# bacon205/Multimodal_eeg_fmri

Measured on AMD Instinct MI355X. Metric: pairs_per_sec_per_node, higher is better.
Workload: dtype bf16

## Files before the change

### include/mmeeg_hip.h

```cpp
#ifndef MMEEG_HIP_H
#define MMEEG_HIP_H

#include <stdint.h>

#ifdef __cplusplus
extern "C" {
#endif

typedef struct ihipStream_t* hipStream_t;

#define MM_ABI_VERSION 5

const char* mm_last_error(void);
int mm_abi_version(void);

int mm_pack_nct_bf16(const float* x, void* y, int B, int C, int T, int Cp, hipStream_t stream);
int mm_unpack_ntc_f32(const void* g, float* dx, int B, int C, int T, int Cp, hipStream_t stream);
int mm_prep_conv_weight(const float* w, void* w_fwd, void* w_dgrad, int Cout, int Cin, int k,
                        int Cinp, int Coutp, hipStream_t stream);

int mm_conv1d_fwd(const void* x, const void* w, int B, int T, int Cin, int Cout, int taps, int pad,
                  const float* scale, const float* shift, int act, const float* residual,
                  const float* pe, int pool, float* stats, float* out_f32, void* out_bf16,
                  void* out_pre, float drop_p, uint32_t drop_seed, const uint32_t* seed_epoch,
// ... 108 lines not shown
int mm_bn_act_bwd_apply_bcast(const float* y, const float* out4, const float* dout_rows, float scale, const float* sums,
                              void* dy, int R, int S, int N, int act, float drop_p, uint32_t seed,
                              const uint32_t* seed_epoch, int train, int sums_nrep, hipStream_t stream);

int mm_pooled_head_bwd_rows(const float* dout, const void* z_pre_bf16, const float* W, void* dz_bf16, float* rows_out,
                            void* dx_bf16, int B, int L, int D, int N, int act, float drop_p, uint32_t seed,
                            float emit_drop_p, uint32_t emit_seed, const uint32_t* seed_epoch, hipStream_t stream);

int mm_attn_fwd(const void* qkv, void* out, float* lse, int B, int L, int H, int head_dim,
                float scale, float drop_p, uint32_t seed, const uint32_t* seed_epoch,
                const float* attn_mask, int attn_mask_per_head, hipStream_t stream);
int mm_attn_bwd(const void* qkv, const void* out, const void* dout, const float* lse, void* dqkv,
                float* delta_ws, int B, int L, int H, int head_dim, float scale, float drop_p,
                uint32_t seed, const uint32_t* seed_epoch, const float* attn_mask, int attn_mask_per_head,
                hipStream_t stream);
int mm_attn_fwd_hd(const void* qkv, void* out, float* lse, int B, int L, int H, int head_dim,
                   float scale, float drop_p, uint32_t seed, const uint32_t* seed_epoch,
                   const float* attn_mask, int attn_mask_per_head, hipStream_t stream);
int mm_attn_bwd_hd(const void* qkv, const void* out, const void* dout, const float* lse, void* dqkv,
                   float* delta_ws, int B, int L, int H, int head_dim, float scale, float drop_p,
                   uint32_t seed, const uint32_t* seed_epoch, const float* attn_mask, int attn_mask_per_head,
                   hipStream_t stream);

int mm_colsum(const void* a_bf16, const float* a_f32, float* out, int M, int N, hipStream_t stream);
int mm_meanpool_fwd(const float* x, float* out_f32, void* out_bf16, int B, int L, int D, hipStream_t stream);
int mm_meanpool_bwd(const float* g, float* dx, int B, int L, int D, hipStream_t stream);
int mm_stage_inputs(const float* eeg, void* eeg_packed_bf16, float* eeg_copy, int B, int C, int T, int Cp,
                    float* fmri_dst, const float* fmri_src, int64_t fmri_n, hipStream_t stream);
int mm_act_bwd(const float* g_f32, const void* g_bf16, const void* z, void* out, int64_t n, int act,
               float drop_p, uint32_t seed, const uint32_t* seed_epoch, hipStream_t stream);

int mm_pack_volume_bf16(const float* x, void* y, int64_t nvox, int Cp, hipStream_t stream);
int mm_conv3d_fwd(const void* x, const void* w, int B, int D, int H, int W, int Cin, int Cout,
                  const float* shift, float* stats, float* out_f32, void* out_bf16, hipStream_t stream);
int mm_conv3d_wgrad(const void* dy, const void* x, float* dw, float* dbias, int B, int D, int H, int W,
                    int Cin, int Cout, int Cin_real, int64_t sn, int64_t sc, int64_t stap, int nrep,
                    int64_t rep_stride, int slot_mode, hipStream_t stream);
int mm_conv3d_wgrad_slots(int B, int D, int H, int W, int Cin, int Cout, int* slots_host, hipStream_t stream);
int mm_pool3d_bn_act_fwd(const void* y, const float* out4, void* out_bf16, void* ysel, void* arg, int B, int D,
                         int H, int W, int N, int act, float drop_p, uint32_t seed, const uint32_t* seed_epoch,
                         hipStream_t stream);
int mm_pool3d_bn_act_bwd_reduce(const void* ysel, const float* out4, const void* dout_bf16, float* sums_out,
                                int B, int D, int H, int W, int N, int act, float drop_p, uint32_t seed,
                                const uint32_t* seed_epoch, hipStream_t stream);
int mm_pool3d_bn_act_bwd_apply(const void* y, const void* arg, const float* out4, const void* dout_bf16,
                               const float* sums, void* dy, int B, int D, int H, int W, int N, int act,
                               float drop_p, uint32_t seed, const uint32_t* seed_epoch, int train, int sums_nrep,
                               hipStream_t stream);

int mm_conv3d_l1(int mode, const float* x, const void* wimg, const float* bias, const float* out4,
                 const void* dout, const float* sums, float* stats, void* out, float* dw_tapmajor,
                 float* dbias, int B, int D, int H, int W, int train, float drop_p, uint32_t seed,
                 const uint32_t* seed_epoch, hipStream_t stream);
int mm_conv3d_l1_fwd_winners(const float* x, const void* wimg, const float* bias, const float* out4, void* out,
                             void* arg, int B, int D, int H, int W, int train, float drop_p, uint32_t seed,
                             const uint32_t* seed_epoch, hipStream_t stream);
int mm_conv3d_l1_gram(const float* x, const void* wimg, const float* bias, float* gram, float* stats, int B, int D,
                      int H, int W, hipStream_t stream);
int mm_conv3d_l1_bwd(const float* x, const void* wimg, const float* bias, const float* out4, const void* dout,
                     float* sums_out, float* a1, const float* gram, float* dw, float* dbias, int B, int D,
                     int H, int W, int train, float drop_p, uint32_t seed, const uint32_t* seed_epoch,
                     hipStream_t stream);

int mm_small_linear_fwd(const float* x, const float* W, const float* bias, const float* scale,
                        const float* shift, float* y, float* pre, int B, int K, int N, int act,
                        float drop_p, uint32_t seed, const uint32_t* seed_epoch, hipStream_t stream);
int mm_small_linear_bwd(const float* dy, const float* x, const float* W, float* dx, float* dW, float* db,
                        int B, int K, int N, hipStream_t stream);
int mm_act_f32(const float* z, float* y, int64_t n, int act, float drop_p, uint32_t seed, const uint32_t* seed_epoch, hipStream_t stream);
int mm_act_bwd_f32(const float* g, const float* z, float* out, int64_t n, int act, float drop_p,
                   uint32_t seed, const uint32_t* seed_epoch, hipStream_t stream);
int mm_colstats(const float* x, float* stats, int B, int N, hipStream_t stream);
int mm_proj_heads_fwd(const float* x_e, const float* W_e, const float* b_e, const float* g_e, const float* be_e,
                      int K_e, const float* x_f, const float* W_f, const float* b_f, const float* g_f,
                      const float* be_f, int K_f, float* z1, float* hn, float* stat, float* z, float* nrm, int B,
                      int N, float eps, float drop_p, uint32_t seed_e, uint32_t seed_f,
                      const uint32_t* seed_epoch, hipStream_t stream);
int mm_proj_heads_bwd(const float* dz, const float* z, const float* nrm, const float* hn, const float* z1,
                      const float* stat, const float* x_e, const float* W_e, const float* g_e, int K_e,
                      const float* x_f, const float* W_f, const float* g_f, int K_f, float* dx_e, float* dW_e,
                      float* db_e, float* dg_e, float* dbe_e, float* dx_f, float* dW_f, float* db_f, float* dg_f,
                      float* dbe_f, int B, int N, float drop_p, uint32_t seed_e, uint32_t seed_f,
                      const uint32_t* seed_epoch, hipStream_t stream);
int mm_clip_loss_own_rows(const float* z_all, const float* logit_scale, float* scal4, float* dz_local, float* ws,
                          int B, int Bg, int N, int row0, hipStream_t stream);
int mm_clip_loss_ws_floats(int B, int Bg, int* floats_host, hipStream_t stream);
int mm_clip_loss_own_rows_grouped(const float* z_all, const int* gid_all, const float* logit_scale, float* scal4,
                                  float* dz_local, float* ws, int B, int Bg, int N, int row0, hipStream_t stream);
int mm_clip_loss_grouped_ws_floats(int B, int Bg, int* floats_host, hipStream_t stream);

#define MM_RETRIEVAL_KMAX 16
#define MM_RETRIEVAL_NMAX (1 << 20)
int mm_retrieval(const float* Q, const float* G, const int* pos, int* ranks, int* topk_idx, float* topk_score,
                 float* ws, int Nq, int Ng, int D, int k, hipStream_t stream);
int mm_retrieval_ws_floats(int Nq, int Ng, int D, int k, int* floats_host, hipStream_t stream);
int mm_retrieval_grouped(const float* Q, const float* G, const int* qgid, const int* ggid, int* ranks, float* ws,
                         int Nq, int Ng, int D, hipStream_t stream);
int mm_retrieval_grouped_ws_floats(int Nq, int Ng, int D, int* floats_host, hipStream_t stream);

typedef struct {
    float* w[3]; float* b[3]; float* gamma[3]; float* beta[3]; float* run_mean[3]; float* run_var[3];
    void* batches_tracked[3];
    float* W; float* B; float* Gamma; float* Beta; float* Run_mean; float* Run_var;
    int cin; int k[3]; int cinp; int reserved;
} mm_power_merge_t;
int mm_power_merge(const void* desc_host, int mode, hipStream_t stream);

int mm_softmax2_concat(const float* a, const float* c, const float* pa, const float* pc, float* out, int B,
                       int Ha, int Hc, hipStream_t stream);
int mm_learned_fusion(const float* f0, const float* f1, const float* f2, const float* dyn,
                      const float* logits, const float* temperature, float* fused, float* weights, int B,
                      int H, int M, hipStream_t stream);
int mm_attn_1xk(const float* p0, const float* p1, const float* p2, const float* p3, int K, const float* dctx,
                float* ctx, float* attw, float* dp0, float* dp1, float* dp2, float* dp3, int B, int E,
                int nhead, float drop_p, uint32_t seed, const uint32_t* seed_epoch, int backward,
                hipStream_t stream);
int mm_add_f32(const float* a, const float* b, float* out, int64_t n, hipStream_t stream);
int mm_attn_1x2(const float* proj_e, const float* proj_f, float* ctx, float* attw, int B, int E, int nhead,
                hipStream_t stream);
int mm_attn_1x2_train(const float* proj_e, const float* proj_f, const float* dctx, float* ctx, float* attw,
                      float* dproj_e, float* dproj_f, int B, int E, int nhead, float drop_p, uint32_t seed,
                      const uint32_t* seed_epoch, int backward, hipStream_t stream);
int mm_learned_fusion_bwd(const float* f0, const float* f1, const float* f2, const float* dyn,
                          const float* logits, const float* temperature, const float* dfused, float* df0,
                          float* df1, float* df2, float* ddyn, float* dlogits, float* dtemp, int B, int H,
                          int M, hipStream_t stream);
int mm_softmax2_concat_bwd(const float* dout, const float* a, const float* c, const float* pa,
                           const float* pc, float* da, float* dc, float* dpa, float* dpc, int B, int Ha,
                           int Hc, hipStream_t stream);
int mm_weighted_ce(const float* logits, const void* target_i64, const float* class_weight, float* loss_out,
                   float* dlogits, int B, int C, hipStream_t stream);
int mm_focal_loss(const float* logits, const void* target_i64, float* loss_out, float* per_sample,
                  float* dlogits, int B, int C, float alpha, float gamma, float scale, hipStream_t stream);
int mm_gate2_mix(const float* g, const float* erp, const float* pw, const float* conn, float* comb,
                 float* gate, int B, int H, float boost, hipStream_t stream);
int mm_gate2_mix_bwd(const float* dcomb, const float* g, const float* erp, const float* pw, float* derp,
                     float* dpw, float* dconn, float* dg, int B, int H, float boost, hipStream_t stream);
int mm_smoothed_ce(const float* logits, const void* target_i64, float* loss_out, float* dlogits, int B,
                   int C, float smoothing, hipStream_t stream);
int mm_stft_power(const float* x, void* out_bf16, float* out_f32, int B, int C, int T, int nfft, int hop,
                  int ch_off, int ch_total, hipStream_t stream);
#define MM_ZSCORE_WS_DOUBLES 64
int mm_sample_zscore_bf16(const float* x, void* out_bf16, double* ws, int B, int rows, int ch_valid, int ch_total,
                          float eps, hipStream_t stream);
int mm_sample_zscore_bwd(const float* x, const void* g_bf16, float* dx, int B, int rows, int ch_valid, int ch_total,
                         float eps, hipStream_t stream);
int mm_stft_power_bwd(const float* x, const float* g_power, float* dx, int B, int C, int T, int nfft, int hop,
                      int ch_off, int ch_total, hipStream_t stream);
int mm_mul_f32(const float* a, const float* b, float* out, int64_t n, hipStream_t stream);
int mm_linear_fwd_meanpool(const void* x, const void* w, int M, int K, const float* bias, const float* residual,
                           float* out_f32, float drop_p, uint32_t seed, const uint32_t* seed_epoch, float* pool_out,
                           int rows_per_group, hipStream_t stream);
int mm_linear_fwd_ln(const void* x, const void* w, int M, int K, const float* bias, const float* residual,
                     float* out_f32, float drop_p, uint32_t seed, const uint32_t* seed_epoch, const float* ln_gamma,
                     const float* ln_beta, float ln_eps, void* ln_out_bf16, float* ln_stat, hipStream_t stream);
int mm_pooled_head_fwd(const float* pooled, const float* pooled_acc, const float* W, const float* bias, float* out, void* z_pre_bf16,
                       void* pooled_bf16, int B, int D, int N, int act, float drop_p, uint32_t seed,
                       const uint32_t* seed_epoch, hipStream_t stream);
int mm_pooled_head_bwd(const float* dout, const void* z_pre_bf16, const float* W, void* dz_bf16, float* dx,
                       void* dx_bf16, int B, int L, int D, int N, int act, float drop_p, uint32_t seed,
                       float emit_drop_p, uint32_t emit_seed, const uint32_t* seed_epoch, hipStream_t stream);
int mm_drop_path(const float* x, float* out, int64_t B, int64_t inner, float drop_p, uint32_t seed,
                 const uint32_t* seed_epoch, hipStream_t stream);
int mm_meanpool_bf16(const void* x, float* out, int R, int S, int N, hipStream_t stream);

#define MM_OPT_STATE_FLOATS 1032
int mm_sumsq(const float* g, float* state, int64_t n, hipStream_t stream);
int mm_adamw_clip(float* p, float* g, float* m, float* v, float* state, int64_t n, float beta1,
                  float beta2, float eps, float weight_decay, float max_norm, float grad_scale,
                  int zero_grad, uint32_t* seed_epoch, hipStream_t stream);

int mm_xai_interp(const float* x, const float* base, int base_rows, float* out, int n_steps, int s0, int steps,
// ... 36 lines not shown
```

### multimodal_eeg_fmri_amd/autograd.py

```python
from __future__ import annotations

import os
from typing import Dict, List, Optional

import torch

from . import _hip
from . import ops
from .ops import ACT, AREPL, REPL, WREP, _BF, _F32, _empty, _zeros


_BAG = {"cur": None}


def _reduce_into(dst, src, K, stride, offset=0, nrep=REPL):
    if dst is None:
        return
    if nrep not in (1, REPL):
        raise ValueError("_reduce_into: nrep is 1 (fp32 vector) or REPL (accumulator workspace)")
    bag = _BAG["cur"]
    ptr = src.data_ptr() + (8 if nrep == REPL else 4) * offset
    if bag is not None:
        bag.defer(ptr, dst, K, AREPL if nrep == REPL else 1, stride, keep=src)
    elif nrep == REPL:
# ... 617 lines not shown
    end = ops.kernel_timer.bracket(f"conv3d_dgrad_c{N}")
    _hip.call("mm_conv3d_fwd", dy, wd, B, D, H, W, N, cinp, None, None, None, dx)
    if end is not None:
        end.record()
    return dx


def conv3d_l1_bwd(bag: GradBag, s: dict, dout: torch.Tensor):
    conv, bn, x = s["conv"], s["bn"], s["x"]
    B, _, D, H, W = x.shape
    train = 1 if s.get("train", True) else 0
    sums = _zeros((REPL, 2, 32), x)
    dw = bag.target(conv.weight)
    if dw is None:
        _hip.call("mm_conv3d_l1", 2, x, s["wimg"], conv.bias, s["out4"], dout, None, sums, None, None, None,
                  B, D, H, W, train, float(s["drop_p"]), int(s["seed"]), ops.EP())
    else:
        a1 = _zeros((REPL, 27, 32), x)
        _hip.call("mm_conv3d_l1_bwd", x, s["wimg"], conv.bias, s["out4"], dout, sums, a1, s.get("gramc") if train else None,
                  dw, bag.target(conv.bias), B, D, H, W, train, float(s["drop_p"]), int(s["seed"]), ops.EP())
    _bn_param_grads(bag, bn, sums, 32, nrep=REPL)


def volume_encoder_bwd(bag: GradBag, sv: dict, dout: torch.Tensor):
    last = sv["convs"][2]
    d = pooled_head_bwd(bag, sv["head"], dout, rows_only=not last["pool"])
    g = conv3d_bn_act_bwd(bag, last, d)
    g = conv3d_bn_act_bwd(bag, sv["convs"][1], g)
    if sv["convs"][0].get("l1"):
        conv3d_l1_bwd(bag, sv["convs"][0], g)
        return None
    need_dx = bool(sv.get("need_dx"))
    dxp = conv3d_bn_act_bwd(bag, sv["convs"][0], g, need_dx=need_dx)
    if not need_dx:
        return None
    Bx, C, D, H, W = sv["x_shape"]
    return dxp[..., :C].permute(0, 4, 1, 2, 3).float().contiguous()


class VolumeEncoderFn(_ModuleFn):

    @staticmethod
    def run(m, x):
        return VolumeEncoderFn.apply(m, x, *_module_params(m))

    @staticmethod
    def forward(ctx, m, x, *params):
        ctx.need_dx = bool(x.requires_grad)
        out, saved = ops._vol_forward_impl(m, x.float(), m.training, True, save=True, need_dx=ctx.need_dx)
        ctx.saved, ctx.params = saved, params
        return out

    @staticmethod
    def backward(ctx, dout):
        bag = GradBag()
        with deferred(bag, dout.device):
            dx = volume_encoder_bwd(bag, ctx.saved, dout)
        return _ModuleFn._finish(ctx, bag, ctx.params, dx)


def proj_head_bwd(bag: GradBag, s: dict, da: torch.Tensor, need_dx=True):
    lin, ln = s["seq"][0], s["seq"][1]
    B, N = da.shape
    K = lin.weight.shape[1]
    dhn = _empty((B, N), _F32, da)
    _hip.call("mm_act_bwd_f32", da, s["hn"], dhn, B * N, ACT["gelu"], float(s["p"]), int(s["seed"]), ops.EP())
    dz1 = _empty((B, N), _F32, da)
    dgb = _zeros((REPL, 2, N), da)
    _hip.call("mm_layernorm_bwd", None, dhn, s["z1"], s["stat"], ln.weight, None, dz1, None, dgb, B, N, 0.0, 0, None)
    _ln_param_grads(bag, ln, dgb, N)
    dx = _empty((B, K), _F32, da) if need_dx else None
    _hip.call("mm_small_linear_bwd", dz1, s["x"], lin.weight, dx, bag.target(lin.weight), bag.target(lin.bias), B, K, N)
    return dx


def contrastive_embed_bwd(bag: GradBag, s: dict, dz: torch.Tensor, need=(True, True)):
    B, N = s["B"], s["N"]
    br = s["bridge"]
    (le, lne), (lf, lnf) = br.eeg_proj[:2], br.fmri_proj[:2]
    xe, xf = s["xe"], s["xf"]
    dxe = _empty(xe.shape, _F32, dz) if need[0] else None
    dxf = _empty(xf.shape, _F32, dz) if need[1] else None
    t = bag.target
    _hip.call("mm_proj_heads_bwd", dz.contiguous(), s["z"], s["nrm"], s["hn"], s["z1"], s["stat"],
              xe, le.weight, lne.weight, xe.shape[1], xf, lf.weight, lnf.weight, xf.shape[1],
              dxe, t(le.weight), t(le.bias), t(lne.weight), t(lne.bias),
              dxf, t(lf.weight), t(lf.bias), t(lnf.weight), t(lnf.bias),
              B, N, float(s["p"]), int(s["seeds"][0]), int(s["seeds"][1]), ops.EP())
    return dxe, dxf


class ContrastiveEmbedFn(torch.autograd.Function):
    @staticmethod
    def run(bridge, eeg, fmri):
        ps = list(bridge.eeg_proj.parameters()) + list(bridge.fmri_proj.parameters())
        return ContrastiveEmbedFn.apply(bridge, eeg, fmri, *ps)

    @staticmethod
    def forward(ctx, bridge, eeg, fmri, *params):
        z, saved = ops.contrastive_embed_impl(bridge, eeg, fmri, bridge.training)
        ctx.saved, ctx.params = saved, params
        ctx.need = (eeg.requires_grad, fmri.requires_grad)
        return z

    @staticmethod
    def backward(ctx, dz):
        bag = GradBag()
        with deferred(bag, dz.device):
            dxe, dxf = contrastive_embed_bwd(bag, ctx.saved, dz.contiguous(), ctx.need)
        return (None, dxe, dxf) + tuple(bag.result(p) for p in ctx.params)


class ClipLossFn(torch.autograd.Function):

    @staticmethod
    def forward(ctx, z, logit_scale, group, gid=None):
        from . import dp
        z = z.contiguous().float()
        B, N2 = z.shape
        rank = dp.rank(group)
        z_all = dp.gather_embeddings(z, group)
        need_grad = z.requires_grad or logit_scale.requires_grad
        scal = _empty((4,), _F32, z)
        dz = _empty((B, N2), _F32, z) if need_grad else None
        ls = logit_scale.detach().reshape(1).float().contiguous()
        gid_all = None if gid is None else dp.gather_embeddings(gid.view(B, 1), group).view(-1)
        ops.clip_loss_own_rows(z_all, gid_all, ls, scal, dz, B, rank * B)
        if need_grad:
            ctx.save_for_backward(dz, scal)
        return scal[0].clone(), scal[1].clone(), scal[2].clone()

    @staticmethod
    def backward(ctx, g_loss, g_a, g_b):
        dz, scal = ctx.saved_tensors
        return dz * g_loss, (scal[3] * g_loss).reshape(()), None, None
```

### multimodal_eeg_fmri_amd/bridge_trainer.py

```python
from __future__ import annotations

import os
from typing import Dict, Optional

import torch
import torch.nn as nn

from . import _hip, dp, ops
from .autograd import GradBag, contrastive_embed_bwd, deferred, erp_encoder_bwd, power_encoder_bwd, volume_encoder_bwd
from .bridge_checkpoint import TrainerCheckpointMixin
from .bridge_utils import EEGfMRIContrastiveBridge, retrieval_metrics
from .enhanced_models_v4 import EnhancedERPEncoder
from .fmri_utils import fMRIVolumeEncoder3D
from .optim import FlatBucket


class BridgeTrainer(TrainerCheckpointMixin, nn.Module):
    def __init__(self, eeg_channels: int = 64, hidden_dim: int = 128, fmri_dim: int = 64,
                 bridge_dim: int = 128, dropout: float = 0.3, lr: float = 1e-4,
                 weight_decay: float = 1e-4, grad_clip: float = 1.0, betas=(0.9, 0.999),
                 eps: float = 1e-8, group=None, device="cuda", mode: str = "graph", eeg_encoder: Optional[nn.Module] = None,
                 num_heads: int = 4, num_layers: int = 2):
        super().__init__()
        self.eeg_encoder = (EnhancedERPEncoder(eeg_channels, hidden_dim, num_layers, num_heads, dropout)
# ... 50 lines not shown
        assert off == self.bucket.n
        self.fmri_lo = self.groups[-1][2]
        self._works = []
        self.capture_mode = None
        self.bucket.state[2] = lr
        self._scal = torch.zeros(4, device=device)
        ops.weights_changed()

    @property
    def _side(self):
        if self._side_stream is None:
            self._side_stream = torch.cuda.Stream()
        return self._side_stream

    @property
    def world(self):
        import torch.distributed as dist
        return dist.get_world_size(self.group) if self.group is not None else 1

    def set_lr(self, lr: float):
        self.lr = lr
        self.bucket.state[2] = lr

    def forward(self, eeg: torch.Tensor, fmri: torch.Tensor, groups: Optional[torch.Tensor] = None):
        gid = ops.group_ids(groups, eeg.shape[0], eeg.device, "BridgeTrainer")
        if not self.two_streams:
            return self.head(self.eeg_encoder(eeg), self.fmri_encoder(fmri), self.group, gid)
        main = torch.cuda.current_stream()
        self._side.wait_stream(main)
        with torch.cuda.stream(self._side):
            ff = self.fmri_encoder(fmri)
        fe = self.eeg_encoder(eeg)
        main.wait_stream(self._side)
        ff.record_stream(main)
        return self.head(fe, ff, self.group, gid)

    def train_step(self, eeg: torch.Tensor, fmri: torch.Tensor, groups: Optional[torch.Tensor] = None) -> Dict[str, torch.Tensor]:
        ops.check_volume_shape(fmri.shape)
        gid = ops.group_ids(groups, eeg.shape[0], None if self.mode == "graph" else eeg.device, "train_step")
        if self.mode == "autograd":
            return self._step_autograd(eeg, fmri, gid)
        if self.mode == "manual":
            with torch.no_grad():
                return self._step_manual(eeg, fmri, gid)
        return self._step_graph(eeg, fmri, gid)

    def _step_autograd(self, eeg, fmri, gid=None):
        b = self.bucket
        b.zero_grad()
        loss, acc_e, acc_f = self.forward(eeg, fmri, gid)
        loss.backward()
        b.absorb_autograd_grads()
        self._seg_optimizer()
        return {"loss": loss.detach(), "top1_e2f": acc_e, "top1_f2e": acc_f}

    STAMP_NAMES = ("step start", "weights prepared", "EEG fwd done", "fMRI fwd start", "fMRI fwd done",
                   "heads fwd done", "loss done", "heads bwd done", "EEG bwd done", "fMRI bwd start",
                   "fMRI bwd done", "grad reductions done", "AdamW done", "side stream done")

    def _stamp(self, i):
        if self.stamps is not None:
            _hip.call("mm_debug_stamp", self.stamps, i)

    def _seg_forward(self, eeg, fmri, xb=None):
        self._stamp(0)
        if self._weight_list is not None:
            ops.arena.begin(eeg.device, clear=self._arena_need, defer_zero=True)
            ops.weights.prepare_all(self._weight_list, zero=ops.arena.zero_range())
        else:
            ops.arena.begin(eeg.device, clear=self._arena_need)
        self._stamp(1)
        main = torch.cuda.current_stream()
        self._side.wait_stream(main)
        self._fmri_longer = self._fmri_is_longer(fmri)

        def fmri_branch():
            with torch.cuda.stream(self._side):
                self._stamp(3)
                out = ops._vol_forward_impl(self.fmri_encoder, fmri, True, True)
                self._stamp(4)
            return out
        if self._fmri_longer:
            ff, sv_f = fmri_branch()
        fe, sv_e = self._eeg_forward(eeg, xb)
        self._stamp(2)
        if not self._fmri_longer:
            ff, sv_f = fmri_branch()
        main.wait_stream(self._side)
        z, sv_h = ops.contrastive_embed_impl(self.head.bridge, fe, ff, True)
        self._stamp(5)
        return z, (sv_e, sv_f, sv_h)

    @staticmethod
    def _fmri_is_longer(fmri) -> bool:
        env = os.environ.get("MM_FMRI_LONGER")
        if env is not None:
            return env == "1"
        return fmri[0].numel() >= 4 * 32 ** 3

    def _eeg_forward(self, eeg, xb):
        enc = self.eeg_encoder
        if self._eeg_kind == "erp":
            return ops._erp_forward_impl(enc, eeg, True, True, xb=xb)
        if self._eeg_kind == "power":
            return ops._power_forward_impl(enc, xb if xb is not None else ops.pack_nct(eeg), True, False)
        spec = ops.stft_front_end(eeg, enc.n_ffts, enc.hop, enc.normalize)
        return ops._power_forward_impl(enc.encoder, spec, True, False)

    def _seg_loss(self, z_all, scal, dz, gid_all=None):
        ls = self.head.logit_scale.detach().reshape(1)
        ops.clip_loss_own_rows(z_all, gid_all, ls, scal, dz, dz.shape[0], dp.rank(self.group) * dz.shape[0])
        self._stamp(6)

    def _reduce_group(self, ready: str):
        for name, rdy, lo, hi in self.groups:
            if rdy == ready and hi > lo:
                self._works.append(dp.allreduce_sum_(self.bucket.g[lo:hi], self.group, async_op=True))

    def _seg_backward(self, saved, dz, scal, reduce: bool = False):
        sv_e, sv_f, sv_h = saved
        self._works = []
        bag = GradBag()
        with deferred(bag, dz.device):
            bag.defer(scal.data_ptr() + 12, self.head.logit_scale._mm_grad.view(1), 1, 1, 1, keep=scal)
            dfe, dff = contrastive_embed_bwd(bag, sv_h, dz)
            self._stamp(7)
            main = torch.cuda.current_stream()
            self._side.wait_stream(main)
            hand = not getattr(self, "_fmri_longer", False)
            handed = []

            def split():
                if not hand:
                    return
                ev = torch.cuda.Event()
                handed.append((bag.hand_over(), ev))
                ev.record()
            def split_convs():
                split()
                bag.defer_conv_wgrads = False
            handed_convs = int(os.environ.get("MM_CONV_WGRADS_HANDED", "1")) if hand else 0
            bag.defer_conv_wgrads = handed_convs >= 2

            def conv3_done():
                bag.defer_conv_wgrads = handed_convs >= 1

            def fmri_branch():
                with torch.cuda.stream(self._side):
                    self._stamp(9)
                    bag_f = GradBag()
                    with deferred(bag_f, dz.device):
                        volume_encoder_bwd(bag_f, sv_f, dff)
                    self._stamp(10)
                    if reduce and hand:
                        self._reduce_group("fmri")
                    for i, (hb, ev) in enumerate(handed):
                        self._side.wait_event(ev)
                        hb.flush(dz.device)
                        if reduce:
                            self._reduce_group(f"handed{i}")
                    self._stamp(13)
                return bag_f
            if not hand:
                bag_f = fmri_branch()
            finish = None
            if self._eeg_kind == "erp":
                erp_encoder_bwd(bag, sv_e, dfe, after_blocks=split, after_conv2=split_convs, after_conv3=conv3_done)
            else:
                _, finish = power_encoder_bwd(bag, sv_e, dfe)
            bag.flush(dz.device)
            if finish is not None:
                finish()
            self._stamp(8)
            if hand:
                bag_f = fmri_branch()
            if reduce:
                if not hand:
                    self._reduce_group("handed0")
                    self._reduce_group("handed1")
                self._reduce_group("main")
                if not hand:
                    with torch.cuda.stream(self._side):
                        self._reduce_group("fmri")
            main.wait_stream(self._side)
        self._stamp(11)
        self._bags = getattr(self, "_bags", [])[-12:] + [bag, bag_f] + [hb for hb, _ in handed]

    def _seg_optimizer(self, reduced: bool = False):
        if reduced:
            for w in self._works:
                dp.wait(w)
            self._works = []
        else:
            dp.allreduce_sum_(self.bucket.g, self.group)
        self._seg_adamw()

    def _seg_adamw(self):
        b = self.bucket
        _hip.call("mm_sumsq", b.g, b.state, b.n)
        _hip.call("mm_adamw_clip", b.p, b.g, b.m, b.v, b.state, b.n, self.betas[0], self.betas[1],
                  self.eps, self.weight_decay, self.grad_clip, 1.0 / self.world, 1, ops.EP())
        ops.weights_changed()
        if self._arena_need is None:
            self._arena_need = (ops.arena.high * 5 // 4 + 4095) // 4096 * 4096
        ops.arena.end()
        self._stamp(12)

    def _step_manual(self, eeg, fmri, gid=None):
        recording = self._weight_list is None
        if recording:
            ops.weights.start_recording()
        try:
            return self._step_manual_body(eeg, fmri, gid)
        finally:
            if recording:
                self._weight_list = ops.weights.stop_recording()

    def _step_manual_body(self, eeg, fmri, gid=None):
        gid_all = None if gid is None else dp.gather_embeddings(gid.view(-1, 1), self.group).view(-1)
        z, saved = self._seg_forward(eeg, fmri)
        z_all = dp.gather_embeddings(z, self.group)
        scal, dz = self._scal, ops._empty(tuple(z.shape), torch.float32, z)
        self._seg_loss(z_all, scal, dz, gid_all)
        early = dp.active(self.group)
        self._seg_backward(saved, dz, scal, reduce=early)
        self._seg_optimizer(reduced=early)
        return {"loss": scal[0], "top1_e2f": scal[1], "top1_f2e": scal[2]}

    def _capture(self, eeg, fmri, gid=None):
        dev = eeg.device
        world = self.world
        c = {"epoch": torch.zeros(1, dtype=torch.int32, device=dev)}
        stft = self._eeg_kind == "stft"
        Bx, Cx, Tx = eeg.shape
        n_e = eeg.numel() * 4 if stft else Bx * Tx * ops.cpad(Cx) * 2
        n_f = fmri.numel() * 4
        c["grouped"] = gid is not None
        c["in"] = torch.empty(n_e + n_f + (Bx * 4 if c["grouped"] else 0), dtype=torch.uint8, device=dev)
        c["fmri"] = c["in"][n_e:n_e + n_f].view(torch.float32).view(fmri.shape)
        c["fmri"].copy_(fmri)
        c["gid"] = c["gid_all"] = None
        if c["grouped"]:
            c["gid"] = c["in"][n_e + n_f:].view(torch.int32)
            c["gid"].copy_(gid)
        if stft:
            c["eeg"], c["xb"] = c["in"][:n_e].view(torch.float32).view(eeg.shape), None
            c["eeg"].copy_(eeg)
        else:
            c["eeg"] = eeg.clone()
            c["xb"] = c["in"][:n_e].view(torch.bfloat16).view(Bx, Tx, ops.cpad(Cx))
            _hip.call("mm_pack_nct_bf16", c["eeg"], c["xb"], Bx, Cx, Tx, c["xb"].shape[2])
        ops.set_seed_epoch(c["epoch"])
        b = self.bucket
        snap = [t.clone() for t in (b.p, b.m, b.v, b.state)]
        bufs = [t for t in self.buffers() if t is not None]
        snap_bufs = [t.clone() for t in bufs]
        side = torch.cuda.Stream()
        side.wait_stream(torch.cuda.current_stream())
        with torch.cuda.stream(side), torch.no_grad():
            for _ in range(2):
                self._step_manual(c["eeg"], c["fmri"], c["gid"])
        torch.cuda.current_stream().wait_stream(side)
        torch.cuda.synchronize()
        with torch.no_grad():
            for t, sv in zip((b.p, b.m, b.v, b.state), snap):
                t.copy_(sv)
            for t, sv in zip(bufs, snap_bufs):
                t.copy_(sv)
        ops.weights_changed()
        c["pool"] = torch.cuda.graph_pool_handle()
        graphs = []

        dist_alive = torch.distributed.is_available() and torch.distributed.is_initialized()

        def record(fn, mode=None):
            mode = mode or ("thread_local" if dist_alive else "global")
            g = torch.cuda.CUDAGraph()
            with torch.cuda.graph(g, pool=c["pool"], capture_error_mode=mode), torch.no_grad():
                fn()
            graphs.append(g)

        B = eeg.shape[0]
        N2 = 2 * self.head.bridge.bridge_dim
        c["scal"] = self._scal
        import os
        dist_step = not (world == 1 and not (self.force_segments and self.group is not None))
        c["gid_gather"] = c["grouped"] and dist_step and dp.active(self.group)
        if c["grouped"]:
            c["gid_all"] = torch.empty(world * B, dtype=torch.int32, device=dev) if c["gid_gather"] else c["gid"]
        if not dist_step:
            def whole():
                z, saved = self._seg_forward(c["eeg"], c["fmri"], xb=c["xb"])
                c["z"] = z
                c["dz"] = ops._empty(tuple(z.shape), torch.float32, z)
                self._seg_loss(z, c["scal"], c["dz"], c["gid_all"])
                self._seg_backward(saved, c["dz"], c["scal"])
                self._grad_probe()
                self._seg_adamw()
            record(whole)
            self.capture_mode = "one graph"
        elif dp.CAPTURABLE and os.environ.get("MM_DP_CAPTURE", "1") != "0" and self._capture_with_collectives(c, record, graphs, B, N2, world, dev):
            self.capture_mode = "one graph + captured RCCL collectives"
        else:
            self.capture_mode = "3 segments + 2 eager collectives"
            def seg1():
                c["z"], c["saved"] = self._seg_forward(c["eeg"], c["fmri"], xb=c["xb"])
                c["dz"] = ops._empty((B, N2), torch.float32, c["z"])
            record(seg1)
            c["z_all"] = torch.empty(world * B, N2, device=dev)

            def seg2():
                self._seg_loss(c["z_all"], c["scal"], c["dz"], c["gid_all"])
                self._seg_backward(c["saved"], c["dz"], c["scal"])
            record(seg2)

            def seg3():
                self._grad_probe()
                self._seg_adamw()
            record(seg3)
        c["graphs"] = graphs
        self._cap = c

    def _grad_probe(self):
        probe = getattr(self, "grad_probe", None)
        if probe is not None:
            probe.copy_(self.bucket.g)

    def _capture_with_collectives(self, c, record, graphs, B, N2, world, dev) -> bool:
        c["z_all"] = torch.empty(world * B, N2, device=dev)
        dp.all_gather_into(c["z_all"], torch.zeros(B, N2, device=dev), self.group)
        dp.wait(dp.allreduce_sum_(torch.zeros(8, device=dev), self.group, async_op=True))
        torch.cuda.synchronize()

        def whole_dp():
            self._gather_group_ids(c)
            z, saved = self._seg_forward(c["eeg"], c["fmri"], xb=c["xb"])
            c["z"] = z
            c["dz"] = ops._empty((B, N2), torch.float32, z)
            dp.all_gather_into(c["z_all"], z, self.group)
            self._seg_loss(c["z_all"], c["scal"], c["dz"], c["gid_all"])
            self._seg_backward(saved, c["dz"], c["scal"], reduce=True)
            for w in self._works:
                dp.wait(w)
            self._works = []
            self._grad_probe()
            self._seg_adamw()
        issued0 = dp.issued
        err = None
        try:
            record(whole_dp, mode="thread_local")
        except Exception as e:
            err = f"{type(e).__name__}: {e}"
            e.__traceback__ = None
            del e
        verdict = dp.agree_on_capture(err is None, dp.issued - issued0, self.group)
        if verdict == "captured":
            return True
        import gc
        import warnings
        warnings.warn(f"collectives not captured into the step's hipGraph on every rank (this rank: "
                      f"{'captured' if err is None else err}; group verdict {verdict}); "
                      "all ranks use three graph segments around two eager collectives")
        if err is None:
            graphs.pop()
        c.pop("z", None), c.pop("dz", None)
        gc.collect()
        torch.cuda.synchronize()
        c["pool"] = torch.cuda.graph_pool_handle()
        self._works = []
        if verdict == "segments-after-abort":
            dp.check_communicator(self.group, dev)
        ops.arena.end()
        ops.weights_changed()
        return False

    def _gather_group_ids(self, c):
        if not c["gid_gather"]:
            return
# ... 299 lines not shown
```

### multimodal_eeg_fmri_amd/csrc/heads.hip

```cpp
#include "common.h"

namespace {

__global__ void small_linear_fwd_kernel(const float* __restrict__ x, const float* __restrict__ W,
                                        const float* __restrict__ bias, const float* __restrict__ scale,
                                        const float* __restrict__ shift, float* __restrict__ y,
                                        float* __restrict__ pre, int B, int K, int N, int act,
                                        uint32_t thresh, uint32_t seed, float inv_keep, const uint32_t* epoch) {
    seed = mm_eff_seed(seed, epoch);
    extern __shared__ float xs[];
    const int b = blockIdx.x;
    for (int k = threadIdx.x; k < K; k += blockDim.x) xs[k] = x[(size_t)b * K + k];
    __syncthreads();
    const int lane = threadIdx.x & 63, wave = threadIdx.x >> 6, nw = blockDim.x >> 6;
    for (int n = blockIdx.y * nw + wave; n < N; n += gridDim.y * nw) {
        float s = 0.f;
        for (int k = lane; k < K; k += 64) s += xs[k] * W[(size_t)n * K + k];
        s = wave_sum(s);
        if (lane == 0) {
            s += bias ? bias[n] : 0.f;
            if (scale) s = s * scale[n] + shift[n];
            const size_t idx = (size_t)b * N + n;
            if (pre) pre[idx] = s;
            s = apply_act(s, act);
// ... 5 lines not shown

__global__ void small_linear_dx_kernel(const float* __restrict__ dy, const float* __restrict__ W,
                                       float* __restrict__ dx, int B, int K, int N) {
    extern __shared__ float ds[];
    const int b = blockIdx.x;
    for (int n = threadIdx.x; n < N; n += blockDim.x) ds[n] = dy[(size_t)b * N + n];
    __syncthreads();
    for (int k = threadIdx.x; k < K; k += blockDim.x) {
        float s = 0.f;
        for (int n = 0; n < N; ++n) s += ds[n] * W[(size_t)n * K + k];
        dx[(size_t)b * K + k] = s;
    }
}

__global__ void small_linear_dw_kernel(const float* __restrict__ dy, const float* __restrict__ x,
                                       float* __restrict__ dW, float* __restrict__ db, int B, int K, int N) {
    const int n = blockIdx.x;
    for (int k = threadIdx.x; k < K; k += blockDim.x) {
        float s = 0.f;
        for (int b = 0; b < B; ++b) s += dy[(size_t)b * N + n] * x[(size_t)b * K + k];
        dW[(size_t)n * K + k] += s;
    }
    if (db && threadIdx.x == 0) {
        float s = 0.f;
        for (int b = 0; b < B; ++b) s += dy[(size_t)b * N + n];
        db[n] += s;
    }
}

__global__ void act_f32_kernel(const float* __restrict__ z, float* __restrict__ y, size_t n, int act,
                               uint32_t thresh, uint32_t seed, float inv_keep, const uint32_t* epoch) {
    seed = mm_eff_seed(seed, epoch);
    for (size_t i = (size_t)blockIdx.x * blockDim.x + threadIdx.x; i < n; i += (size_t)gridDim.x * blockDim.x) {
        float v = apply_act(z[i], act);
        if (thresh) v *= dropout_scale(seed, (uint32_t)i, thresh, inv_keep);
        y[i] = v;
    }
}
__global__ void act_bwd_f32_kernel(const float* __restrict__ g, const float* __restrict__ z, float* __restrict__ out,
                                   size_t n, int act, uint32_t thresh, uint32_t seed, float inv_keep,
                                   const uint32_t* epoch) {
    seed = mm_eff_seed(seed, epoch);
    for (size_t i = (size_t)blockIdx.x * blockDim.x + threadIdx.x; i < n; i += (size_t)gridDim.x * blockDim.x) {
        float v = g[i];
        if (thresh) v *= dropout_scale(seed, (uint32_t)i, thresh, inv_keep);
        if (z) v *= act_grad(z[i], act);
        out[i] = v;
    }
}

__global__ void colstats_kernel(const float* __restrict__ x, float* __restrict__ stats, int B, int N) {
    const int n = blockIdx.x * blockDim.x + threadIdx.x;
    if (n >= N) return;
    float s = 0.f, q = 0.f;
    for (int b = 0; b < B; ++b) { const float v = x[(size_t)b * N + n]; s += v; q += v * v; }
    mm_acc_t* acc = reinterpret_cast<mm_acc_t*>(stats);
    acc[n] = acc_encode<MM_ACC_STAT>(s);
    acc[N + n] = acc_encode<MM_ACC_STAT>(q);
}


struct HeadSide {
    const float* x; const float* W; const float* bias; const float* gamma; const float* beta;
    float* dx; float* dW; float* dbias; float* dgamma; float* dbeta;
    int K; uint32_t seed;
};
struct HeadsArgs {
    HeadSide s[2];
    float* z1; float* hn; float* stat;
    float* z; float* nrm;
    const float* dz;
    int B, N; float eps; uint32_t thresh; float inv_keep; const uint32_t* epoch;
};
constexpr int HEAD_MAXK = 1024, HEAD_MAXN = 256;

__device__ __forceinline__ float block_sum256(float v, float* red ) {
    v = wave_sum(v);
    __syncthreads();
    if ((threadIdx.x & 63) == 0) red[threadIdx.x >> 6] = v;
    __syncthreads();
    return (red[0] + red[1]) + (red[2] + red[3]);
}

__global__ __launch_bounds__(256) void proj_heads_fwd_kernel(HeadsArgs a) {
    __shared__ float xs[HEAD_MAXK], v[HEAD_MAXN], red[4];
    const int b = blockIdx.x, m = blockIdx.y, tid = threadIdx.x, lane = tid & 63, wave = tid >> 6;
    const HeadSide s = a.s[m];
    const int N = a.N, K = s.K;
    for (int k = tid; k < K; k += 256) xs[k] = s.x[(size_t)b * K + k];
    __syncthreads();
    const int T = N <= 64 ? 4 : (N <= 128 ? 2 : 1);
    {
        const int n = tid / T, part = tid % T;
        float acc = 0.f;
        if (n < N) {
            const float* wr = s.W + (size_t)n * K;
            if ((K & 3) == 0) {
#pragma unroll 8
                for (int k = part * 4; k < K; k += 4 * T) {
                    const float4 w4 = *reinterpret_cast<const float4*>(wr + k);
                    acc += w4.x * xs[k] + w4.y * xs[k + 1] + w4.z * xs[k + 2] + w4.w * xs[k + 3];
                }
            } else {
                for (int k = part; k < K; k += T) acc += wr[k] * xs[k];
            }
        }
        if (T >= 2) acc += __shfl_xor(acc, 1, 64);
        if (T >= 4) acc += __shfl_xor(acc, 2, 64);
        if (n < N && part == 0) v[n] = acc + (s.bias ? s.bias[n] : 0.f);
    }
    (void)lane; (void)wave;
    __syncthreads();
    const bool on = tid < N;
    const float x1 = on ? v[tid] : 0.f;
    const float mean = block_sum256(x1, red) / N;
    const float dlt = on ? x1 - mean : 0.f;
    const float rstd = rsqrtf(block_sum256(dlt * dlt, red) / N + a.eps);
    float act = 0.f, hn = 0.f;
    const size_t o = ((size_t)m * a.B + b) * N + tid;
    if (on) {
        hn = dlt * rstd * s.gamma[tid] + s.beta[tid];
        act = gelu_erf(hn);
        if (a.thresh) act *= dropout_scale(mm_eff_seed(s.seed, a.epoch), (uint32_t)(b * N + tid), a.thresh, a.inv_keep);
        if (a.z1) { a.z1[o] = x1; a.hn[o] = hn; }
    }
    const float nr = fmaxf(sqrtf(block_sum256(act * act, red)), 1e-12f);
    if (on) a.z[(size_t)b * 2 * N + m * N + tid] = act / nr;
    if (tid == 0) {
        a.nrm[m * a.B + b] = nr;
        if (a.stat) { a.stat[((size_t)m * a.B + b) * 2] = mean; a.stat[((size_t)m * a.B + b) * 2 + 1] = rstd; }
    }
}

constexpr int HB_RC = 32;
template <int NE>
__global__ __launch_bounds__(1024) void proj_heads_bwd_kernel(HeadsArgs a) {
    __shared__ float d1[HB_RC][HEAD_MAXN];
    __shared__ float px[1024];
    const int j = blockIdx.x, m = blockIdx.y, tid = threadIdx.x, lane = tid & 63, wave = tid >> 6;
    const HeadSide s = a.s[m];
    const int N = a.N, K = s.K, B = a.B, G = gridDim.x;
    const int NK = N * K, S = (NK + G - 1) / G;
    const uint32_t seed = mm_eff_seed(s.seed, a.epoch);
    float ag[NE], ab[NE], gam[NE];
#pragma unroll
    for (int e = 0; e < NE; ++e) {
        ag[e] = 0.f; ab[e] = 0.f;
        gam[e] = lane + 64 * e < N ? s.gamma[lane + 64 * e] : 0.f;
    }
    for (int b0 = 0; b0 < B; b0 += HB_RC) {
        const int nb = B - b0 < HB_RC ? B - b0 : HB_RC;
        __syncthreads();
        float dzv[2][NE], zv[2][NE], hnv[2][NE], z1v[2][NE], mean[2], rstd[2], nr[2];
#pragma unroll
        for (int q = 0; q < 2; ++q) {
            const int r = wave + 16 * q;
            const bool row_on = r < nb;
            const int b = row_on ? b0 + r : b0;
            const size_t o = ((size_t)m * B + b) * N, oz = (size_t)b * 2 * N + m * N;
            mean[q] = a.stat[((size_t)m * B + b) * 2]; rstd[q] = a.stat[((size_t)m * B + b) * 2 + 1];
            nr[q] = a.nrm[m * B + b];
#pragma unroll
            for (int e = 0; e < NE; ++e) {
                const int n = lane + 64 * e;
                const bool on = row_on && n < N;
                dzv[q][e] = on ? a.dz[oz + n] : 0.f;
                zv[q][e] = on ? a.z[oz + n] : 0.f;
                hnv[q][e] = on ? a.hn[o + n] : 0.f;
                z1v[q][e] = on ? a.z1[o + n] : 0.f;
            }
        }
#pragma unroll
        for (int q = 0; q < 2; ++q) {
            const int r = wave + 16 * q;
            if (r >= nb) continue;
            const int b = b0 + r;
            float dot = 0.f;
#pragma unroll
            for (int e = 0; e < NE; ++e) dot += dzv[q][e] * zv[q][e];
            dot = wave_sum(dot);
            float gd[NE], xh[NE], s1 = 0.f, s2 = 0.f;
#pragma unroll
            for (int e = 0; e < NE; ++e) {
                const int n = lane + 64 * e;
                gd[e] = 0.f; xh[e] = 0.f;
                if (n < N) {
                    float g = (dzv[q][e] - zv[q][e] * dot) / nr[q];
                    if (a.thresh) g *= dropout_scale(seed, (uint32_t)(b * N + n), a.thresh, a.inv_keep);
                    const float dh = g * gelu_erf_grad(hnv[q][e]);
                    xh[e] = (z1v[q][e] - mean[q]) * rstd[q];
                    gd[e] = dh * gam[e];
                    ag[e] += dh * xh[e];
                    ab[e] += dh;
                }
                s1 += gd[e]; s2 += gd[e] * xh[e];
            }
            const float m1 = wave_sum(s1) / N, m2 = wave_sum(s2) / N;
#pragma unroll
            for (int e = 0; e < NE; ++e) {
                const int n = lane + 64 * e;
                if (n < N) d1[r][n] = rstd[q] * (gd[e] - m1 - xh[e] * m2);
            }
        }
        __syncthreads();
        if (s.dx) {
            const int nparts = 1024 / K > 0 ? 1024 / K : 1;
            for (int b = j; b < b0 + nb; b += G) {
                if (b < b0) continue;
                const int k = tid % K, part = tid / K;
                if (part < nparts) {
                    float acc = 0.f;
#pragma unroll 4
                    for (int n = part; n < N; n += nparts) acc += d1[b - b0][n] * s.W[(size_t)n * K + k];
                    px[part * K + k] = acc;
                }
                __syncthreads();
                if (tid < K) {
                    float acc = 0.f;
                    for (int q = 0; q < nparts; ++q) acc += px[q * K + tid];
                    s.dx[(size_t)b * K + tid] = acc;
                }
                __syncthreads();
            }
        }
        if (s.dW) {
            const int hi = (j + 1) * S < NK ? (j + 1) * S : NK;
            for (int i = j * S + tid; i < hi; i += 1024) {
                const int n = i / K, k = i % K;
                const float* xc = s.x + (size_t)b0 * K + k;
                float acc = 0.f;
#pragma unroll 8
                for (int r = 0; r < nb; ++r) acc += d1[r][n] * xc[(size_t)r * K];
                s.dW[i] += acc;
            }
        }
        if (j == 0 && s.dbias && tid < N) {
            float acc = 0.f;
            for (int r = 0; r < nb; ++r) acc += d1[r][tid];
            s.dbias[tid] += acc;
        }
    }
    if (j == 0 && (s.dgamma || s.dbeta)) {
        __syncthreads();
        float (*pg)[2][HEAD_MAXN] = reinterpret_cast<float (*)[2][HEAD_MAXN]>(&d1[0][0]);
#pragma unroll
        for (int e = 0; e < NE; ++e) {
            const int n = lane + 64 * e;
            if (n < N) { pg[wave][0][n] = ag[e]; pg[wave][1][n] = ab[e]; }
        }
        __syncthreads();
        if (tid < 2 * N) {
            const int which = tid / N, n = tid % N;
            float acc = 0.f;
            for (int w = 0; w < 16; ++w) acc += pg[w][which][n];
            float* dst = which ? s.dbeta : s.dgamma;
            if (dst) dst[n] += acc;
        }
    }
}

struct ClipShared {
    float *qe, *qf, *cr, *cc, *red;
};
__device__ __forceinline__ ClipShared clip_shared(float* sm, int N, int Bg) {
    ClipShared s;
    s.qe = sm; s.qf = sm + N; s.cr = s.qf + N; s.cc = s.cr + Bg; s.red = s.cc + Bg;
    return s;
}
__device__ __forceinline__ void clip_cosines(const float* __restrict__ z_all, int r, int Bg, int N, const ClipShared& sh,
                                             float& mxr, float& mxc) {
    const int LD = 2 * N, tid = threadIdx.x, lane = tid & 63, wave = tid >> 6;
    for (int n = tid; n < N; n += 256) { sh.qe[n] = z_all[(size_t)r * LD + n]; sh.qf[n] = z_all[(size_t)r * LD + N + n]; }
    __syncthreads();
    float a_mx = -INFINITY, c_mx = -INFINITY;
    const int sub = tid & 7, n32 = N & ~31;
    for (int j = tid >> 3; j < Bg; j += 32) {
        float a = 0.f, c = 0.f;
        const float* re = z_all + (size_t)j * LD;
        const float* rf = re + N;
        for (int n = sub * 4; n < n32; n += 32) {
            const float4 vf = *reinterpret_cast<const float4*>(rf + n);
            const float4 ve = *reinterpret_cast<const float4*>(re + n);
            a += sh.qe[n] * vf.x + sh.qe[n + 1] * vf.y + sh.qe[n + 2] * vf.z + sh.qe[n + 3] * vf.w;
            c += sh.qf[n] * ve.x + sh.qf[n + 1] * ve.y + sh.qf[n + 2] * ve.z + sh.qf[n + 3] * ve.w;
        }
        for (int n = n32 + sub; n < N; n += 8) { a += sh.qe[n] * rf[n]; c += sh.qf[n] * re[n]; }
#pragma unroll
        for (int o = 4; o > 0; o >>= 1) { a += __shfl_xor(a, o, 64); c += __shfl_xor(c, o, 64); }
        if (sub == 0) { sh.cr[j] = a; sh.cc[j] = c; }
        a_mx = fmaxf(a_mx, a); c_mx = fmaxf(c_mx, c);
    }
    a_mx = wave_max(a_mx); c_mx = wave_max(c_mx);
    if (lane == 0) { sh.red[wave] = a_mx; sh.red[4 + wave] = c_mx; }
    __syncthreads();
    mxr = fmaxf(fmaxf(sh.red[0], sh.red[1]), fmaxf(sh.red[2], sh.red[3]));
    mxc = fmaxf(fmaxf(sh.red[4], sh.red[5]), fmaxf(sh.red[6], sh.red[7]));
    __syncthreads();
}
__device__ __forceinline__ void clip_sum2(float& a, float& c, float* red) {
    const int lane = threadIdx.x & 63, wave = threadIdx.x >> 6;
    a = wave_sum(a); c = wave_sum(c);
    if (lane == 0) { red[wave] = a; red[4 + wave] = c; }
    __syncthreads();
    a = (red[0] + red[1]) + (red[2] + red[3]);
    c = (red[4] + red[5]) + (red[6] + red[7]);
    __syncthreads();
}
__device__ __forceinline__ void clip_max2(float& a, float& c, float* red) {
    const int lane = threadIdx.x & 63, wave = threadIdx.x >> 6;
    a = wave_max(a); c = wave_max(c);
    if (lane == 0) { red[wave] = a; red[4 + wave] = c; }
    __syncthreads();
    a = fmaxf(fmaxf(red[0], red[1]), fmaxf(red[2], red[3]));
    c = fmaxf(fmaxf(red[4], red[5]), fmaxf(red[6], red[7]));
    __syncthreads();
}

template <bool GROUPED>
__global__ __launch_bounds__(256) void clip_lse_kernel(const float* __restrict__ z_all, const float* __restrict__ logit_scale,
                                                       float* __restrict__ ws, int Bg, int N, const int* __restrict__ gid) {
    extern __shared__ float sm[];
    const ClipShared sh = clip_shared(sm, N, Bg);
    const int r = blockIdx.x, tid = threadIdx.x;
    const float s = __expf(logit_scale[0]);
    int gr = 0;
    if constexpr (GROUPED) gr = gid[r];
    float mxr, mxc;
    clip_cosines(z_all, r, Bg, N, sh, mxr, mxc);
    float pmr = -INFINITY, pmc = -INFINITY;
    if constexpr (GROUPED) {
        for (int j = tid; j < Bg; j += 256)
            if (gid[j] == gr) { pmr = fmaxf(pmr, sh.cr[j]); pmc = fmaxf(pmc, sh.cc[j]); }
        clip_max2(pmr, pmc, sh.red);
    }
    float se = 0.f, sf = 0.f, ee = 0.f, ef = 0.f;
    float qe = 0.f, qf = 0.f, qee = 0.f, qef = 0.f;
    for (int j = tid; j < Bg; j += 256) {
        const float a = sh.cr[j], c = sh.cc[j];
        const float pa = __expf(s * (a - mxr)), pc = __expf(s * (c - mxc));
        se += pa; sf += pc; ee += pa * a; ef += pc * c;
        if constexpr (GROUPED) {
            if (gid[j] == gr) {
                const float qa = __expf(s * (a - pmr)), qc = __expf(s * (c - pmc));
                qe += qa; qf += qc; qee += qa * a; qef += qc * c;
            }
        }
    }
    clip_sum2(se, sf, sh.red);
    clip_sum2(ee, ef, sh.red);
    if constexpr (GROUPED) {
        clip_sum2(qe, qf, sh.red);
        clip_sum2(qee, qef, sh.red);
    }
    if (tid == 0) {
        if constexpr (GROUPED) {
            const float lse_r = s * mxr + __logf(se), lse_c = s * mxc + __logf(sf);
            const float lsp_r = s * pmr + __logf(qe), lsp_c = s * pmc + __logf(qf);
            ws[r] = lse_r;
            ws[Bg + r] = lse_c;
            ws[2 * Bg + r] = 0.5f * ((lse_r - lsp_r) + (lse_c - lsp_c));
            ws[3 * Bg + r] = pmr >= mxr ? 1.f : 0.f;
            ws[4 * Bg + r] = pmc >= mxc ? 1.f : 0.f;
            ws[5 * Bg + r] = s * 0.5f * ((ee / se - qee / qe) + (ef / sf - qef / qf));
            ws[6 * Bg + r] = lsp_r;
            ws[7 * Bg + r] = lsp_c;
        } else {
            const float diag = sh.cr[r];
            const float lse_r = s * mxr + __logf(se), lse_c = s * mxc + __logf(sf);
            ws[r] = lse_r;
            ws[Bg + r] = lse_c;
            ws[2 * Bg + r] = 0.5f * ((lse_r - s * diag) + (lse_c - s * sh.cc[r]));
            ws[3 * Bg + r] = diag >= mxr ? 1.f : 0.f;
            ws[4 * Bg + r] = sh.cc[r] >= mxc ? 1.f : 0.f;
            ws[5 * Bg + r] = s * 0.5f * ((ee / se - diag) + (ef / sf - sh.cc[r]));
        }
    }
}

template <bool GROUPED>
__global__ __launch_bounds__(256) void clip_rows_kernel(const float* __restrict__ z_all, const float* __restrict__ logit_scale,
                                                        const float* __restrict__ ws, float* __restrict__ scal,
                                                        float* __restrict__ dz, int B, int Bg, int N, int row0,
                                                        const int* __restrict__ gid) {
    extern __shared__ float sm[];
    const ClipShared sh = clip_shared(sm, N, Bg);
    const int i = blockIdx.x, gi = row0 + i, tid = threadIdx.x, LD = 2 * N;
    const float s = __expf(logit_scale[0]);
    const float invB = 1.f / (float)B;
    if (i == 0 && tid < 64) {
        float acc[4] = {0.f, 0.f, 0.f, 0.f};
        for (int r0 = 0; r0 < B; r0 += 64) {
            float v[4];
#pragma unroll
            for (int q = 0; q < 4; ++q) v[q] = (r0 + tid < B) ? ws[(size_t)(2 + q) * Bg + row0 + r0 + tid] : 0.f;
#pragma unroll
            for (int q = 0; q < 4; ++q) acc[q] += wave_sum(v[q]);
        }
        if (tid < 4) scal[tid] = (tid == 0 ? acc[0] : tid == 1 ? acc[1] : tid == 2 ? acc[2] : acc[3]) * invB;
    }
    if (!dz) return;
    float mxr, mxc;
    clip_cosines(z_all, gi, Bg, N, sh, mxr, mxc);
    const float lse_rg = ws[gi], lse_cg = ws[Bg + gi];
    float lsp_rg = 0.f, lsp_cg = 0.f;
    int gg = 0;
    if constexpr (GROUPED) { lsp_rg = ws[6 * Bg + gi]; lsp_cg = ws[7 * Bg + gi]; gg = gid[gi]; }
    const float k = 0.5f * invB * s;
    for (int j = tid; j < Bg; j += 256) {
        const float a = s * sh.cr[j], c = s * sh.cc[j];
        float ga = __expf(a - lse_rg) + __expf(a - ws[Bg + j]);
        float gc = __expf(c - ws[j]) + __expf(c - lse_cg);
        if constexpr (GROUPED) {
            if (gid[j] == gg) {
                ga -= __expf(a - lsp_rg) + __expf(a - ws[7 * Bg + j]);
                gc -= __expf(c - ws[6 * Bg + j]) + __expf(c - lsp_cg);
            }
        } else {
            if (j == gi) { ga -= 2.f; gc -= 2.f; }
        }
        sh.cr[j] = k * ga; sh.cc[j] = k * gc;
    }
    __syncthreads();
    float* orow = dz + (size_t)i * LD;
    for (int n = tid; n < 2 * N; n += 256) {
        const bool first = n < N;
        const float* g = first ? sh.cr : sh.cc;
        const float* col = z_all + (first ? N + n : n - N);
        float acc = 0.f;
        int j = 0;
        for (; j + 8 <= Bg; j += 8) {
            float v[8];
#pragma unroll
            for (int q = 0; q < 8; ++q) v[q] = col[(size_t)(j + q) * LD];
#pragma unroll
            for (int q = 0; q < 8; ++q) acc += g[j + q] * v[q];
        }
        for (; j < Bg; ++j) acc += g[j] * col[(size_t)j * LD];
        orow[n] = acc;
    }
}

constexpr int SUMSQ_SLOTS = 1024;

__global__ void sumsq_kernel(const float* __restrict__ g, float* __restrict__ state, size_t n) {
    float s = 0.f;
    for (size_t i = (size_t)blockIdx.x * blockDim.x + threadIdx.x; i < n; i += (size_t)gridDim.x * blockDim.x) s += g[i] * g[i];
    s = wave_sum(s);
    __shared__ float red[4];
    if ((threadIdx.x & 63) == 0) red[threadIdx.x >> 6] = s;
    __syncthreads();
    if (threadIdx.x == 0) state[8 + blockIdx.x] = (red[0] + red[1]) + (red[2] + red[3]);
    if (blockIdx.x == 0)
        for (int i = gridDim.x + threadIdx.x; i < SUMSQ_SLOTS; i += blockDim.x) state[8 + i] = 0.f;
}

__device__ inline float sumsq_total(const float* __restrict__ state) {
    __shared__ float tot[4];
    const int t = threadIdx.x;
    float s = (state[8 + t] + state[8 + 256 + t]) + (state[8 + 512 + t] + state[8 + 768 + t]);
    s = wave_sum(s);
    if ((t & 63) == 0) tot[t >> 6] = s;
    __syncthreads();
    return (tot[0] + tot[1]) + (tot[2] + tot[3]);
}

__global__ void adamw_kernel(float* __restrict__ p, float* __restrict__ g, float* __restrict__ m,
                             float* __restrict__ v, const float* __restrict__ state, size_t n, float beta1,
                             float beta2, float eps, float wd, float max_norm, float grad_scale, int zero_grad) {
    const float step = state[0] + 1.f;
    const float lr = state[2];
    const float gn = sqrtf(sumsq_total(state)) * grad_scale;
    const float clip = (max_norm > 0.f) ? fminf(1.f, max_norm / (gn + 1e-6f)) : 1.f;
    const float gs = grad_scale * clip;
    const float bc1 = 1.f - powf(beta1, step), bc2 = 1.f - powf(beta2, step);
    const float step_size = lr / bc1, inv_sqrt_bc2 = rsqrtf(bc2);
    for (size_t i = (size_t)blockIdx.x * blockDim.x + threadIdx.x; i < n; i += (size_t)gridDim.x * blockDim.x) {
        const float gi = g[i] * gs;
        float pi = p[i] * (1.f - lr * wd);
        const float mi = beta1 * m[i] + (1.f - beta1) * gi;
        const float vi = beta2 * v[i] + (1.f - beta2) * gi * gi;
        pi -= step_size * mi / (sqrtf(vi) * inv_sqrt_bc2 + eps);
        p[i] = pi; m[i] = mi; v[i] = vi;
        if (zero_grad) g[i] = 0.f;
    }
}

__global__ void adamw_finish_kernel(float* __restrict__ state, float max_norm, float grad_scale, uint32_t* epoch) {
    const float ss = sumsq_total(state);
    if (threadIdx.x != 0) return;
    if (epoch) epoch[0] += 1;
    const float gn = sqrtf(ss) * grad_scale;
    state[3] = (max_norm > 0.f) ? fminf(1.f, max_norm / (gn + 1e-6f)) : 1.f;
    state[4] = gn;
    state[0] += 1.f;
    state[1] = ss;
}


struct PowerMergeArgs {
    float* w[3]; float* b[3]; float* gamma[3]; float* beta[3]; float* run_mean[3]; float* run_var[3];
    long long* tracked[3];
    float* W; float* B; float* Gamma; float* Beta; float* Run_mean; float* Run_var;
    int cin, k[3], cinp, reserved;
};

template <int MODE>
__global__ void power_merge_kernel(PowerMergeArgs a) {
    const size_t per_o = (size_t)a.cin * 7, total = 192 * per_o;
    const size_t gid = (size_t)blockIdx.x * blockDim.x + threadIdx.x;
    if (gid < 192) {
        const int i = (int)gid / 64, j = (int)gid % 64;
        if (MODE == 0 || MODE == 3) {
            a.B[gid] = a.b[i][j]; a.Gamma[gid] = a.gamma[i][j]; a.Beta[gid] = a.beta[i][j];
            a.Run_mean[gid] = a.run_mean[i][j]; a.Run_var[gid] = a.run_var[i][j];
        } else if (MODE == 1) {
            a.run_mean[i][j] = a.Run_mean[gid]; a.run_var[i][j] = a.Run_var[gid];
            if (j == 0 && a.tracked[i]) a.tracked[i][0] += 1;
        } else {
            if (a.b[i] && a.B) a.b[i][j] += a.B[gid];
            if (a.gamma[i] && a.Gamma) a.gamma[i][j] += a.Gamma[gid];
            if (a.beta[i] && a.Beta) a.beta[i][j] += a.Beta[gid];
        }
// ... 694 lines not shown
    const int F = nfft / 2 + 1;
    float* tw_c = sm;
    float* tw_s = tw_c + nfft;
    float* win = tw_s + nfft;
    float* fr = win + nfft;
    float* cr = fr + 8 * nfft;
    float* ci = cr + 8 * F;
    float* acc = ci + 8 * F;
    const int b = blockIdx.y, c = blockIdx.x, tid = threadIdx.x;
    for (int n = tid; n < nfft; n += 256) {
        float s, co;
        __sincosf(6.283185307179586f * (float)n / (float)nfft, &s, &co);
        tw_c[n] = co; tw_s[n] = s;
        win[n] = 0.5f - 0.5f * __cosf(6.283185307179586f * (float)n / (float)nfft);
    }
    for (int t = tid; t < T; t += 256) acc[t] = 0.f;
    const float* xr = x + ((size_t)b * C + c) * T;
    __syncthreads();
    for (int f0 = 0; f0 < frames; f0 += 8) {
        for (int i = tid; i < 8 * nfft; i += 256) {
            const int fi = i / nfft, n = i % nfft, frame = f0 + fi;
            float v = 0.f;
            if (frame < frames) {
                int t = frame * hop + n - nfft / 2;
                if (t < 0) t = -t;
                if (t >= T) t = 2 * (T - 1) - t;
                v = xr[t] * win[n];
            }
            fr[i] = v;
        }
        __syncthreads();
        for (int i = tid; i < 8 * F; i += 256) {
            const int fi = i / F, f = i % F, frame = f0 + fi;
            float re = 0.f, im = 0.f;
            if (frame < frames) {
                const float* fv = fr + fi * nfft;
                for (int n = 0; n < nfft; ++n) {
                    const int k = (f * n) & (nfft - 1);
                    re += fv[n] * tw_c[k];
                    im -= fv[n] * tw_s[k];
                }
                const float g2 = 2.f * gP[((size_t)b * frames + frame) * ch_total + ch_off + (size_t)c * F + f];
                re *= g2; im *= g2;
            }
            cr[i] = re; ci[i] = im;
        }
        __syncthreads();
        for (int i = tid; i < 8 * nfft; i += 256) {
            const int fi = i / nfft, n = i % nfft;
            float dv = 0.f;
            const float *pr = cr + fi * F, *pi = ci + fi * F;
            for (int f = 0; f < F; ++f) {
                const int k = (f * n) & (nfft - 1);
                dv += pr[f] * tw_c[k] - pi[f] * tw_s[k];
            }
            fr[i] = dv * win[n];
        }
        __syncthreads();
        for (int t0 = tid; t0 < T; t0 += 256) {
            float a = acc[t0];
            for (int fi = 0; fi < 8; ++fi) {
                const int frame = f0 + fi;
                if (frame >= frames) break;
                const int base = nfft / 2 - frame * hop;
                int n = t0 + base;
                if (n >= 0 && n < nfft) a += fr[fi * nfft + n];
                n = -t0 + base;
                if (t0 > 0 && n >= 0 && n < nfft) a += fr[fi * nfft + n];
                n = 2 * (T - 1) - t0 + base;
                if (t0 < T - 1 && n >= 0 && n < nfft) a += fr[fi * nfft + n];
            }
            acc[t0] = a;
        }
        __syncthreads();
    }
    float* dr = dx + ((size_t)b * C + c) * T;
    for (int t = tid; t < T; t += 256) dr[t] += acc[t];
}

__global__ void mul_f32_kernel(const float* __restrict__ a, const float* __restrict__ b, float* __restrict__ o, size_t n) {
    for (size_t i = (size_t)blockIdx.x * blockDim.x + threadIdx.x; i < n; i += (size_t)gridDim.x * blockDim.x) o[i] = a[i] * b[i];
}

__global__ __launch_bounds__(256) void pooled_head_fwd_kernel(const float* __restrict__ pooled, const mm_acc_t* __restrict__ pooled_acc,
                                                             const float* __restrict__ W,
                                                             const float* __restrict__ bias, float* __restrict__ out,
                                                             bf16* __restrict__ z_pre, bf16* __restrict__ pooled_bf16,
                                                             int D, int N, int act, uint32_t thresh, float inv_keep,
                                                             uint32_t seed, const uint32_t* __restrict__ epoch) {
    __shared__ float xs[1024];
    const int b = blockIdx.x;
    for (int k = threadIdx.x; k < D; k += 256) {
        const float v = pooled ? pooled[(size_t)b * D + k] : acc_val<MM_ACC_GRAD>(pooled_acc[(size_t)b * D + k]);
        xs[k] = v;
        if (pooled_bf16) pooled_bf16[(size_t)b * D + k] = (bf16)v;
    }
    __syncthreads();
    seed = mm_eff_seed(seed, epoch);
    for (int n = threadIdx.x; n < N; n += 256) {
        const float* wr = W + (size_t)n * D;
        float acc[4] = {0.f, 0.f, 0.f, 0.f};
        int k = 0;
        for (; k + 64 <= D; k += 64) {
            float4 w4[16];
#pragma unroll
            for (int q = 0; q < 16; ++q) w4[q] = *reinterpret_cast<const float4*>(wr + k + q * 4);
#pragma unroll
            for (int q = 0; q < 16; ++q)
                acc[q & 3] += w4[q].x * xs[k + q * 4] + w4[q].y * xs[k + q * 4 + 1] + w4[q].z * xs[k + q * 4 + 2] +
                              w4[q].w * xs[k + q * 4 + 3];
        }
        for (; k < D; k += 16) {
            float4 w4[4];
#pragma unroll
            for (int q = 0; q < 4; ++q) w4[q] = *reinterpret_cast<const float4*>(wr + k + q * 4);
#pragma unroll
            for (int q = 0; q < 4; ++q)
                acc[q] += w4[q].x * xs[k + q * 4] + w4[q].y * xs[k + q * 4 + 1] + w4[q].z * xs[k + q * 4 + 2] +
                          w4[q].w * xs[k + q * 4 + 3];
        }
        const float z = (acc[0] + acc[1]) + (acc[2] + acc[3]) + (bias ? bias[n] : 0.f);
        const size_t idx = (size_t)b * N + n;
        if (z_pre) z_pre[idx] = (bf16)z;
        float v = apply_act(z, act);
        if (thresh) v *= dropout_scale(seed, (uint32_t)idx, thresh, inv_keep);
        out[idx] = v;
    }
}

__global__ __launch_bounds__(256) void pooled_head_bwd_kernel(const float* __restrict__ dout, const bf16* __restrict__ z_pre,
                                                             const float* __restrict__ W, bf16* __restrict__ dz_bf16,
                                                             float* __restrict__ dx, bf16* __restrict__ dx_bf16, int L, int D,
                                                             int N, int rows_per_wg, int act, uint32_t thresh, float inv_keep,
                                                             uint32_t seed, uint32_t thresh2, float inv_keep2, uint32_t seed2,
                                                             const uint32_t* __restrict__ epoch, float* __restrict__ rows_out) {
    __shared__ float dz[1024];
    __shared__ __attribute__((aligned(16))) float dp[1024];
    const int b = blockIdx.x, l0 = blockIdx.y * rows_per_wg;
    seed = mm_eff_seed(seed, epoch);
    seed2 = mm_eff_seed(seed2, epoch);
    for (int n = threadIdx.x; n < N; n += 256) {
        const size_t idx = (size_t)b * N + n;
        float g = dout[idx] * act_grad((float)z_pre[idx], act);
        if (thresh) g *= dropout_scale(seed, (uint32_t)idx, thresh, inv_keep);
        dz[n] = g;
        if (blockIdx.y == 0 && dz_bf16) dz_bf16[idx] = (bf16)g;
    }
    __syncthreads();
    const float invL = 1.f / (float)L;
    for (int k = threadIdx.x; k < D; k += 256) {
        float acc[4] = {0.f, 0.f, 0.f, 0.f};
        int n = 0;
        for (; n + 16 <= N; n += 16) {
            float w[16];
#pragma unroll
            for (int q = 0; q < 16; ++q) w[q] = W[(size_t)(n + q) * D + k];
#pragma unroll
            for (int q = 0; q < 16; ++q) acc[q & 3] += dz[n + q] * w[q];
        }
        for (; n < N; n += 4) {
#pragma unroll
            for (int q = 0; q < 4; ++q) acc[q] += dz[n + q] * W[(size_t)(n + q) * D + k];
        }
        dp[k] = ((acc[0] + acc[1]) + (acc[2] + acc[3])) * invL;
        if (rows_out && blockIdx.y == 0) rows_out[(size_t)b * D + k] = dp[k];
    }
    __syncthreads();
    const int vec = D / 4;
    const int lend = min(L, l0 + rows_per_wg);
    for (int i = threadIdx.x; i < (lend - l0) * vec; i += 256) {
        const int l = l0 + i / vec, k4 = (i % vec) * 4;
        const float4 v = *reinterpret_cast<const float4*>(dp + k4);
        const size_t base = ((size_t)b * L + l) * D + k4;
        if (dx) *reinterpret_cast<float4*>(dx + base) = v;
        if (dx_bf16) {
            const float vs[4] = {v.x, v.y, v.z, v.w};
            bf16x4 o;
#pragma unroll
            for (int c = 0; c < 4; ++c)
                o[c] = (bf16)(thresh2 ? vs[c] * dropout_scale(seed2, (uint32_t)(base + c), thresh2, inv_keep2) : vs[c]);
            *reinterpret_cast<bf16x4*>(dx_bf16 + base) = o;
        }
    }
}

__global__ void drop_path_kernel(const float* __restrict__ x, float* __restrict__ o, size_t n, size_t inner,
                                 uint32_t thresh, float inv_keep, uint32_t base, const uint32_t* __restrict__ epoch) {
    const uint32_t seed = mm_eff_seed(base, epoch);
    for (size_t i = (size_t)blockIdx.x * blockDim.x + threadIdx.x; i < n; i += (size_t)gridDim.x * blockDim.x)
        o[i] = x[i] * dropout_scale(seed, (uint32_t)(i / inner), thresh, inv_keep);
}

__global__ void meanpool_bf16_kernel(const bf16* __restrict__ x, float* __restrict__ out, int S, int N) {
    const int r = blockIdx.x;
    for (int n = threadIdx.x; n < N; n += blockDim.x) {
        float s = 0.f;
        for (int t = 0; t < S; ++t) s += (float)x[((size_t)r * S + t) * N + n];
        out[(size_t)r * N + n] = s / (float)S;
    }
}

inline uint32_t thresh_h(float p) { return p > 0.f ? (uint32_t)((double)p * 4294967296.0) : 0u; }
inline int grid_h(size_t n, int cap = 2048) { size_t g = (n + 255) / 256; return (int)(g < (size_t)cap ? (g ? g : 1) : cap); }

}

extern "C" {

int mm_small_linear_fwd(const float* x, const float* W, const float* bias, const float* scale, const float* shift,
                        float* y, float* pre, int B, int K, int N, int act, float drop_p, uint32_t seed,
                        const uint32_t* seed_epoch, hipStream_t st) {
    MM_REQUIRE(x && W && y && B > 0 && K > 0 && N > 0, "small_linear_fwd: null/invalid");
    MM_REQUIRE((scale == nullptr) == (shift == nullptr), "small_linear_fwd: scale/shift come in pairs");
    MM_REQUIRE((size_t)K * 4 <= 64 * 1024, "small_linear_fwd: K=%d too large", K);
    const int gy = ceil_div(N, 4) < 64 ? ceil_div(N, 4) : 64;
    hipLaunchKernelGGL(small_linear_fwd_kernel, dim3(B, gy), dim3(256), K * sizeof(float), st, x, W, bias, scale, shift,
                       y, pre, B, K, N, act, thresh_h(drop_p), seed, drop_p > 0.f ? 1.f / (1.f - drop_p) : 1.f, seed_epoch);
    return mm_check_launch("small_linear_fwd");
}

int mm_small_linear_bwd(const float* dy, const float* x, const float* W, float* dx, float* dW, float* db, int B, int K,
                        int N, hipStream_t st) {
    MM_REQUIRE(dy && x && W && B > 0 && K > 0 && N > 0, "small_linear_bwd: null/invalid");
    MM_REQUIRE((size_t)N * 4 <= 64 * 1024, "small_linear_bwd: N=%d too large", N);
    if (dx) hipLaunchKernelGGL(small_linear_dx_kernel, dim3(B), dim3(256), N * sizeof(float), st, dy, W, dx, B, K, N);
    if (dW) hipLaunchKernelGGL(small_linear_dw_kernel, dim3(N), dim3(128), 0, st, dy, x, dW, db, B, K, N);
    return mm_check_launch("small_linear_bwd");
}

int mm_act_f32(const float* z, float* y, int64_t n, int act, float drop_p, uint32_t seed, const uint32_t* seed_epoch,
               hipStream_t st) {
    MM_REQUIRE(z && y && n > 0, "act_f32: null");
    hipLaunchKernelGGL(act_f32_kernel, dim3(grid_h((size_t)n)), dim3(256), 0, st, z, y, (size_t)n, act, thresh_h(drop_p),
                       seed, drop_p > 0.f ? 1.f / (1.f - drop_p) : 1.f, seed_epoch);
    return mm_check_launch("act_f32");
}

int mm_act_bwd_f32(const float* g, const float* z, float* out, int64_t n, int act, float drop_p, uint32_t seed,
                   const uint32_t* seed_epoch, hipStream_t st) {
    MM_REQUIRE(g && out && n > 0, "act_bwd_f32: null");
    hipLaunchKernelGGL(act_bwd_f32_kernel, dim3(grid_h((size_t)n)), dim3(256), 0, st, g, z, out, (size_t)n, act,
                       thresh_h(drop_p), seed, drop_p > 0.f ? 1.f / (1.f - drop_p) : 1.f, seed_epoch);
    return mm_check_launch("act_bwd_f32");
}

int mm_colstats(const float* x, float* stats, int B, int N, hipStream_t st) {
    MM_REQUIRE(x && stats && B > 0 && N > 0, "colstats: null");
    hipLaunchKernelGGL(colstats_kernel, dim3(ceil_div(N, 64)), dim3(64), 0, st, x, stats, B, N);
    return mm_check_launch("colstats");
}

int mm_proj_heads_fwd(const float* x_e, const float* W_e, const float* b_e, const float* g_e, const float* be_e, int K_e,
                      const float* x_f, const float* W_f, const float* b_f, const float* g_f, const float* be_f, int K_f,
                      float* z1, float* hn, float* stat, float* z, float* nrm, int B, int N, float eps, float drop_p,
                      uint32_t seed_e, uint32_t seed_f, const uint32_t* seed_epoch, hipStream_t st) {
    MM_REQUIRE(x_e && W_e && g_e && be_e && x_f && W_f && g_f && be_f && z && nrm, "proj_heads_fwd: null");
    MM_REQUIRE((!z1 && !hn && !stat) || (z1 && hn && stat), "proj_heads_fwd: z1/hn/stat go together");
    MM_REQUIRE(B > 0 && N > 0 && N <= HEAD_MAXN && K_e > 0 && K_e <= HEAD_MAXK && K_f > 0 && K_f <= HEAD_MAXK,
               "proj_heads_fwd: B=%d N=%d K=%d/%d", B, N, K_e, K_f);
    HeadsArgs a{};
    a.s[0].x = x_e; a.s[0].W = W_e; a.s[0].bias = b_e; a.s[0].gamma = g_e; a.s[0].beta = be_e; a.s[0].K = K_e; a.s[0].seed = seed_e;
    a.s[1].x = x_f; a.s[1].W = W_f; a.s[1].bias = b_f; a.s[1].gamma = g_f; a.s[1].beta = be_f; a.s[1].K = K_f; a.s[1].seed = seed_f;
    a.z1 = z1; a.hn = hn; a.stat = stat; a.z = z; a.nrm = nrm; a.B = B; a.N = N; a.eps = eps;
    a.thresh = thresh_h(drop_p); a.inv_keep = drop_p > 0.f ? 1.f / (1.f - drop_p) : 1.f; a.epoch = seed_epoch;
    hipLaunchKernelGGL(proj_heads_fwd_kernel, dim3(B, 2), dim3(256), 0, st, a);
    return mm_check_launch("proj_heads_fwd");
}

int mm_proj_heads_bwd(const float* dz, const float* z, const float* nrm, const float* hn, const float* z1,
                      const float* stat, const float* x_e, const float* W_e, const float* g_e, int K_e,
                      const float* x_f, const float* W_f, const float* g_f, int K_f, float* dx_e, float* dW_e,
                      float* db_e, float* dg_e, float* dbe_e, float* dx_f, float* dW_f, float* db_f, float* dg_f,
                      float* dbe_f, int B, int N, float drop_p, uint32_t seed_e, uint32_t seed_f,
                      const uint32_t* seed_epoch, hipStream_t st) {
    MM_REQUIRE(dz && z && nrm && hn && z1 && stat && x_e && W_e && g_e && x_f && W_f && g_f, "proj_heads_bwd: null");
    MM_REQUIRE(B > 0 && N > 0 && N <= HEAD_MAXN && K_e > 0 && K_e <= HEAD_MAXK && K_f > 0 && K_f <= HEAD_MAXK,
               "proj_heads_bwd: B=%d N=%d K=%d/%d", B, N, K_e, K_f);
    HeadsArgs a{};
    a.s[0].x = x_e; a.s[0].W = W_e; a.s[0].gamma = g_e; a.s[0].K = K_e; a.s[0].seed = seed_e;
    a.s[0].dx = dx_e; a.s[0].dW = dW_e; a.s[0].dbias = db_e; a.s[0].dgamma = dg_e; a.s[0].dbeta = dbe_e;
    a.s[1].x = x_f; a.s[1].W = W_f; a.s[1].gamma = g_f; a.s[1].K = K_f; a.s[1].seed = seed_f;
    a.s[1].dx = dx_f; a.s[1].dW = dW_f; a.s[1].dbias = db_f; a.s[1].dgamma = dg_f; a.s[1].dbeta = dbe_f;
    a.z1 = const_cast<float*>(z1); a.hn = const_cast<float*>(hn); a.stat = const_cast<float*>(stat);
    a.z = const_cast<float*>(z); a.nrm = const_cast<float*>(nrm); a.dz = dz; a.B = B; a.N = N;
    a.thresh = thresh_h(drop_p); a.inv_keep = drop_p > 0.f ? 1.f / (1.f - drop_p) : 1.f; a.epoch = seed_epoch;
    switch (ceil_div(N, 64)) {
        case 1: hipLaunchKernelGGL(proj_heads_bwd_kernel<1>, dim3(B, 2), dim3(1024), 0, st, a); break;
        case 2: hipLaunchKernelGGL(proj_heads_bwd_kernel<2>, dim3(B, 2), dim3(1024), 0, st, a); break;
        case 3: hipLaunchKernelGGL(proj_heads_bwd_kernel<3>, dim3(B, 2), dim3(1024), 0, st, a); break;
        default: hipLaunchKernelGGL(proj_heads_bwd_kernel<4>, dim3(B, 2), dim3(1024), 0, st, a); break;
    }
    return mm_check_launch("proj_heads_bwd");
}

static int clip_ws_rows(bool grouped) { return grouped ? 8 : 6; }

static int clip_loss_launch(const char* who, const float* z_all, const int* gid, const float* logit_scale, float* scal4,
                            float* dz_local, float* ws, int B, int Bg, int N, int row0, hipStream_t st) {
    MM_REQUIRE(B > 0 && Bg >= B && row0 >= 0 && row0 + B <= Bg && N > 0, "%s: B=%d Bg=%d row0=%d", who, B, Bg, row0);
    MM_REQUIRE(N % 4 == 0, "%s: N=%d must be a multiple of 4 (16-byte row loads)", who, N);
    const size_t lds = (size_t)(2 * N + 2 * Bg + 32) * sizeof(float);
    MM_REQUIRE(lds <= 64 * 1024, "%s: N/Bg too large for LDS", who);
    const auto lse = gid ? clip_lse_kernel<true> : clip_lse_kernel<false>;
    const auto rows = gid ? clip_rows_kernel<true> : clip_rows_kernel<false>;
    hipLaunchKernelGGL(lse, dim3(Bg), dim3(256), lds, st, z_all, logit_scale, ws, Bg, N, gid);
    char what[64];
    snprintf(what, sizeof what, "%s(lse)", who);
    int rc = mm_check_launch(what);
    if (rc) return rc;
    hipLaunchKernelGGL(rows, dim3(B), dim3(256), lds, st, z_all, logit_scale, ws, scal4, dz_local, B, Bg, N, row0, gid);
    snprintf(what, sizeof what, "%s(rows)", who);
    return mm_check_launch(what);
}

int mm_clip_loss_ws_floats(int B, int Bg, int* floats_host, hipStream_t) {
    MM_REQUIRE(floats_host && B > 0 && Bg >= B, "clip_loss_ws_floats: bad args");
    *floats_host = clip_ws_rows(false) * Bg;
    return 0;
}

int mm_clip_loss_own_rows(const float* z_all, const float* logit_scale, float* scal4, float* dz_local, float* ws, int B,
                          int Bg, int N, int row0, hipStream_t st) {
    MM_REQUIRE(z_all && logit_scale && scal4 && ws, "clip_loss_own_rows: null");
    return clip_loss_launch("clip_loss_own_rows", z_all, nullptr, logit_scale, scal4, dz_local, ws, B, Bg, N, row0, st);
}

int mm_clip_loss_grouped_ws_floats(int B, int Bg, int* floats_host, hipStream_t) {
    MM_REQUIRE(floats_host && B > 0 && Bg >= B, "clip_loss_grouped_ws_floats: bad args");
    *floats_host = clip_ws_rows(true) * Bg;
    return 0;
}

int mm_clip_loss_own_rows_grouped(const float* z_all, const int* gid_all, const float* logit_scale, float* scal4, float* dz_local,
                                  float* ws, int B, int Bg, int N, int row0, hipStream_t st) {
    MM_REQUIRE(z_all && gid_all && logit_scale && scal4 && ws, "clip_loss_own_rows_grouped: null");
    return clip_loss_launch("clip_loss_own_rows_grouped", z_all, gid_all, logit_scale, scal4, dz_local, ws, B, Bg, N, row0, st);
}

int mm_sumsq(const float* g, float* state, int64_t n, hipStream_t st) {
    MM_REQUIRE(g && state && n > 0, "sumsq: null");
    hipLaunchKernelGGL(sumsq_kernel, dim3(grid_h((size_t)n, 1024)), dim3(256), 0, st, g, state, (size_t)n);
    return mm_check_launch("sumsq");
}

int mm_adamw_clip(float* p, float* g, float* m, float* v, float* state, int64_t n, float beta1, float beta2,
                  float eps, float weight_decay, float max_norm, float grad_scale, int zero_grad, uint32_t* seed_epoch,
                  hipStream_t st) {
    MM_REQUIRE(p && g && m && v && state && n > 0, "adamw_clip: null");
    hipLaunchKernelGGL(adamw_kernel, dim3(grid_h((size_t)n)), dim3(256), 0, st, p, g, m, v, state, (size_t)n, beta1,
                       beta2, eps, weight_decay, max_norm, grad_scale, zero_grad);
    hipLaunchKernelGGL(adamw_finish_kernel, dim3(1), dim3(256), 0, st, state, max_norm, grad_scale, seed_epoch);
    return mm_check_launch("adamw_clip");
}

int mm_power_merge(const void* desc_host, int mode, hipStream_t st) {
    MM_REQUIRE(desc_host && mode >= 0 && mode <= 3, "power_merge: null / mode");
    const PowerMergeArgs a = *static_cast<const PowerMergeArgs*>(desc_host);
    MM_REQUIRE(a.cin > 0, "power_merge: cin");
    for (int i = 0; i < 3; ++i) MM_REQUIRE(a.k[i] == 3 || a.k[i] == 5 || a.k[i] == 7, "power_merge: kernel sizes must be 3, 5 or 7");
    if (mode == 0 || mode == 3) {
        for (int i = 0; i < 3; ++i)
            MM_REQUIRE(a.w[i] && a.b[i] && a.gamma[i] && a.beta[i] && a.run_mean[i] && a.run_var[i], "power_merge(0): null part");
        MM_REQUIRE(a.W && a.B && a.Gamma && a.Beta && a.Run_mean && a.Run_var, "power_merge(0): null merged tensor");
        MM_REQUIRE(mode == 0 || (a.cinp >= a.cin && a.cinp % 16 == 0), "power_merge(3): cinp=%d", a.cinp);
    } else if (mode == 1) {
        for (int i = 0; i < 3; ++i) MM_REQUIRE(a.run_mean[i] && a.run_var[i], "power_merge(1): null part");
        MM_REQUIRE(a.Run_mean && a.Run_var, "power_merge(1): null merged statistics");
    }
    const size_t total = (size_t)192 * a.cin * 7;
    const int grid = mode == 1 ? 1 : grid_h(total, 2048);
    if (mode == 3) hipLaunchKernelGGL(power_merge_kernel<3>, dim3(grid), dim3(256), 0, st, a);
    else if (mode == 0) hipLaunchKernelGGL(power_merge_kernel<0>, dim3(grid), dim3(256), 0, st, a);
    else if (mode == 1) hipLaunchKernelGGL(power_merge_kernel<1>, dim3(grid), dim3(256), 0, st, a);
    else hipLaunchKernelGGL(power_merge_kernel<2>, dim3(grid), dim3(256), 0, st, a);
    return mm_check_launch("power_merge");
}

int mm_softmax2_concat(const float* a, const float* c, const float* pa, const float* pc, float* out, int B, int Ha,
                       int Hc, hipStream_t st) {
    MM_REQUIRE(a && c && pa && pc && out && B > 0 && Ha > 0 && Hc > 0, "softmax2_concat: null");
    hipLaunchKernelGGL(softmax2_concat_kernel, dim3(grid_h((size_t)B * (Ha + Hc))), dim3(256), 0, st, a, c, pa, pc, out, B, Ha, Hc);
    return mm_check_launch("softmax2_concat");
}

int mm_learned_fusion(const float* f0, const float* f1, const float* f2, const float* dyn, const float* logits,
                      const float* temperature, float* fused, float* weights, int B, int H, int M, hipStream_t st) {
    MM_REQUIRE(f0 && f1 && dyn && logits && temperature && fused && B > 0 && H > 0, "learned_fusion: null");
    MM_REQUIRE(M >= 2 && M <= 3 && (M == 2 || f2), "learned_fusion: M=%d (2 or 3)", M);
    hipLaunchKernelGGL(learned_fusion_kernel, dim3(ceil_div(B, 4)), dim3(256), 0, st, f0, f1, f2, dyn, logits,
                       temperature, fused, weights, B, H, M);
    return mm_check_launch("learned_fusion");
}

int mm_attn_1x2(const float* proj_e, const float* proj_f, float* ctx, float* attw, int B, int E, int nhead,
                hipStream_t st) {
    MM_REQUIRE(proj_e && proj_f && ctx && attw && B > 0 && nhead > 0 && nhead <= 16 && E % nhead == 0, "attn_1x2: bad args");
    hipLaunchKernelGGL(attn_1x2_fused_kernel, dim3(B), dim3(256), 0, st, proj_e, proj_f, nullptr, ctx, attw, nullptr, nullptr,
                       B, E, nhead, 0u, 0u, 1.f, nullptr, 0);
    return mm_check_launch("attn_1x2");
}

int mm_attn_1x2_train(const float* proj_e, const float* proj_f, const float* dctx, float* ctx, float* attw,
                      float* dproj_e, float* dproj_f, int B, int E, int nhead, float drop_p, uint32_t seed,
                      const uint32_t* seed_epoch, int backward, hipStream_t st) {
    MM_REQUIRE(proj_e && proj_f && B > 0 && nhead > 0 && nhead <= 16 && E % nhead == 0, "attn_1x2_train: bad args");
    MM_REQUIRE(backward ? (dctx && dproj_e && dproj_f) : (ctx != nullptr), "attn_1x2_train: outputs");
    hipLaunchKernelGGL(attn_1x2_fused_kernel, dim3(B), dim3(256), 0, st, proj_e, proj_f, dctx, ctx, attw, dproj_e,
                       dproj_f, B, E, nhead, thresh_h(drop_p), seed, drop_p > 0.f ? 1.f / (1.f - drop_p) : 1.f,
                       seed_epoch, backward);
    return mm_check_launch("attn_1x2_train");
}

int mm_learned_fusion_bwd(const float* f0, const float* f1, const float* f2, const float* dyn, const float* logits,
                          const float* temperature, const float* dfused, float* df0, float* df1, float* df2,
                          float* ddyn, float* dlogits, float* dtemp, int B, int H, int M, hipStream_t st) {
    MM_REQUIRE(f0 && f1 && dyn && logits && temperature && dfused && df0 && df1 && ddyn && dlogits && dtemp,
               "learned_fusion_bwd: null");
    MM_REQUIRE(M >= 2 && M <= 3 && (M == 2 || (f2 && df2)), "learned_fusion_bwd: M=%d", M);
    hipLaunchKernelGGL(learned_fusion_bwd_kernel, dim3(1), dim3(1024), 0, st, f0, f1, f2, dyn, logits,
                       temperature, dfused, df0, df1, df2, ddyn, dlogits, dtemp, B, H, M);
    return mm_check_launch("learned_fusion_bwd");
// ... 65 lines not shown
    }
    const size_t lds = (size_t)(3 * nfft + 8 * nfft) * sizeof(float);
    const int fblocks = ceil_div(frames, 8);
    const int gx = (long)B * C >= 1024 ? 1 : (fblocks < 8 ? fblocks : 8);
    hipLaunchKernelGGL(stft_power_kernel, dim3(gx, C, B), dim3(256), lds, st, x, (bf16*)out_bf16, out_f32,
                       C, T, nfft, hop, frames, ch_off, ch_total);
    return mm_check_launch("stft_power");
}

int mm_sample_zscore_bf16(const float* x, void* out_bf16, double* ws, int B, int rows, int ch_valid, int ch_total, float eps,
                          hipStream_t st) {
    MM_REQUIRE(x && out_bf16 && B > 0 && rows > 0 && ch_valid > 0 && ch_valid <= ch_total, "sample_zscore: null/invalid");
    const size_t n = (size_t)rows * ch_total;
    if (ws && ch_valid == ch_total && (n & 3) == 0 && n < (1ull << 31) && n >= (1u << 16)) {
        MM_REQUIRE(((uintptr_t)ws & 7) == 0, "sample_zscore: workspace alignment");
        hipLaunchKernelGGL(zscore_partial_kernel, dim3(ZS_CHUNKS, B), dim3(256), 0, st, x, ws, (unsigned)(n >> 2));
        hipLaunchKernelGGL(zscore_apply_kernel, dim3(ZS_CHUNKS, B), dim3(256), 0, st, x, (const double*)ws, (bf16*)out_bf16,
                           (unsigned)(n >> 2), (float)rows * (float)ch_valid, eps);
        return mm_check_launch("sample_zscore(chunked)");
    }
    hipLaunchKernelGGL(sample_zscore_kernel, dim3(B), dim3(1024), 0, st, x, (bf16*)out_bf16, rows, ch_valid, ch_total, eps);
    return mm_check_launch("sample_zscore");
}

int mm_stft_power_bwd(const float* x, const float* g_power, float* dx, int B, int C, int T, int nfft, int hop, int ch_off,
                      int ch_total, hipStream_t st) {
    MM_REQUIRE(x && g_power && dx && B > 0 && C > 0 && T > 0, "stft_power_bwd: null/invalid");
    MM_REQUIRE(nfft >= 8 && nfft <= 1024 && (nfft & (nfft - 1)) == 0 && hop > 0 && T > nfft / 2, "stft_power_bwd: nfft=%d hop=%d", nfft, hop);
    const int frames = T / hop + 1;
    const int F = nfft / 2 + 1;
    MM_REQUIRE(ch_off >= 0 && ch_off + C * F <= ch_total, "stft_power_bwd: channel window");
    const size_t lds = (size_t)(3 * nfft + 8 * nfft + 16 * F + T) * sizeof(float);
    if (lds > 160 * 1024) return mm_fail(MM_ERR_UNSUPPORTED, "stft_power_bwd: T=%d nfft=%d needs %zu bytes of LDS", T, nfft, lds);
    auto kern = stft_power_bwd_kernel;
    if (lds > 64 * 1024) (void)hipFuncSetAttribute(reinterpret_cast<const void*>(kern), hipFuncAttributeMaxDynamicSharedMemorySize, (int)lds);
    hipLaunchKernelGGL(kern, dim3(C, B), dim3(256), lds, st, x, g_power, dx, C, T, nfft, hop, frames, ch_off, ch_total);
    return mm_check_launch("stft_power_bwd");
}

int mm_sample_zscore_bwd(const float* x, const void* g_bf16, float* dx, int B, int rows, int ch_valid, int ch_total, float eps,
                         hipStream_t st) {
    MM_REQUIRE(x && g_bf16 && dx && B > 0 && rows > 0 && ch_valid > 0 && ch_valid <= ch_total, "sample_zscore_bwd: null/invalid");
    hipLaunchKernelGGL(sample_zscore_bwd_kernel, dim3(B), dim3(1024), 0, st, x, (const bf16*)g_bf16, dx, rows, ch_valid, ch_total, eps);
    return mm_check_launch("sample_zscore_bwd");
}

int mm_attn_1xk(const float* p0, const float* p1, const float* p2, const float* p3, int K, const float* dctx,
                float* ctx, float* attw, float* dp0, float* dp1, float* dp2, float* dp3, int B, int E, int nhead,
                float drop_p, uint32_t seed, const uint32_t* seed_epoch, int backward, hipStream_t st) {
    MM_REQUIRE(K >= 1 && K <= 4 && B > 0 && nhead > 0 && nhead <= 16 && E % nhead == 0, "attn_1xk: K=%d nhead=%d E=%d", K, nhead, E);
    Attn1xKArgs a{};
    const float* p[4] = {p0, p1, p2, p3};
    float* dp[4] = {dp0, dp1, dp2, dp3};
    for (int j = 0; j < K; ++j) {
        MM_REQUIRE(p[j] && (!backward || dp[j]), "attn_1xk: null token %d", j);
        a.p[j] = p[j]; a.dp[j] = dp[j];
    }
    MM_REQUIRE(backward ? dctx != nullptr : ctx != nullptr, "attn_1xk: outputs");
    a.dctx = dctx; a.ctx = ctx; a.attw = attw; a.B = B; a.E = E; a.nhead = nhead; a.K = K;
    a.thresh = thresh_h(drop_p); a.seed = seed; a.inv_keep = drop_p > 0.f ? 1.f / (1.f - drop_p) : 1.f;
    a.epoch = seed_epoch; a.backward = backward;
    hipLaunchKernelGGL(attn_1xk_kernel, dim3(B), dim3(256), 0, st, a);
    return mm_check_launch("attn_1xk");
}

int mm_add_f32(const float* a, const float* b, float* out, int64_t n, hipStream_t st) {
    MM_REQUIRE(a && b && out && n > 0, "add_f32: null");
    hipLaunchKernelGGL(add_f32_kernel, dim3(grid_h((size_t)n)), dim3(256), 0, st, a, b, out, (size_t)n);
    return mm_check_launch("add_f32");
}

int mm_mul_f32(const float* a, const float* b, float* out, int64_t n, hipStream_t st) {
    MM_REQUIRE(a && b && out && n > 0, "mul_f32: null");
    hipLaunchKernelGGL(mul_f32_kernel, dim3(grid_h((size_t)n)), dim3(256), 0, st, a, b, out, (size_t)n);
    return mm_check_launch("mul_f32");
}

int mm_pooled_head_fwd(const float* pooled, const float* pooled_acc, const float* W, const float* bias, float* out, void* z_pre_bf16,
                       void* pooled_bf16, int B, int D, int N, int act, float drop_p, uint32_t seed,
                       const uint32_t* seed_epoch, hipStream_t st) {
    MM_REQUIRE((pooled != nullptr) != (pooled_acc != nullptr) && W && out && B > 0, "pooled_head_fwd: null (exactly one of pooled / pooled_acc)");
    MM_REQUIRE(D > 0 && D <= 1024 && D % 16 == 0 && N > 0, "pooled_head_fwd: D=%d (multiple of 16, <= 1024)", D);
    MM_REQUIRE(drop_p >= 0.f && drop_p < 1.f, "pooled_head_fwd: drop_p");
    const uint32_t thresh = drop_p > 0.f ? (uint32_t)((double)drop_p * 4294967296.0) : 0u;
    hipLaunchKernelGGL(pooled_head_fwd_kernel, dim3(B), dim3(256), 0, st, pooled, reinterpret_cast<const mm_acc_t*>(pooled_acc), W, bias, out, (bf16*)z_pre_bf16,
                       (bf16*)pooled_bf16, D, N, act, thresh, drop_p > 0.f ? 1.f / (1.f - drop_p) : 1.f, seed, seed_epoch);
    return mm_check_launch("pooled_head_fwd");
}

static int pooled_head_bwd_common(const float* dout, const void* z_pre_bf16, const float* W, void* dz_bf16, float* dx,
                                  void* dx_bf16, float* rows_out, int B, int L, int D, int N, int act, float drop_p,
                                  uint32_t seed, float emit_drop_p, uint32_t emit_seed, const uint32_t* seed_epoch,
                                  hipStream_t st) {
    MM_REQUIRE(dout && z_pre_bf16 && W && (dx || dx_bf16) && B > 0 && L > 0, "pooled_head_bwd: null");
    MM_REQUIRE(D > 0 && D <= 1024 && D % 4 == 0 && N > 0 && N <= 1024 && N % 4 == 0, "pooled_head_bwd: D=%d N=%d", D, N);
    MM_REQUIRE(drop_p >= 0.f && drop_p < 1.f && emit_drop_p >= 0.f && emit_drop_p < 1.f, "pooled_head_bwd: drop_p");
    const int rows = 32;
    const uint32_t t1 = drop_p > 0.f ? (uint32_t)((double)drop_p * 4294967296.0) : 0u;
    const uint32_t t2 = emit_drop_p > 0.f ? (uint32_t)((double)emit_drop_p * 4294967296.0) : 0u;
    hipLaunchKernelGGL(pooled_head_bwd_kernel, dim3(B, (L + rows - 1) / rows), dim3(256), 0, st, dout, (const bf16*)z_pre_bf16, W,
                       (bf16*)dz_bf16, dx, (bf16*)dx_bf16, L, D, N, rows, act, t1, drop_p > 0.f ? 1.f / (1.f - drop_p) : 1.f, seed,
                       t2, emit_drop_p > 0.f ? 1.f / (1.f - emit_drop_p) : 1.f, emit_seed, seed_epoch, rows_out);
    return mm_check_launch("pooled_head_bwd");
}

int mm_pooled_head_bwd(const float* dout, const void* z_pre_bf16, const float* W, void* dz_bf16, float* dx, void* dx_bf16,
                       int B, int L, int D, int N, int act, float drop_p, uint32_t seed, float emit_drop_p,
                       uint32_t emit_seed, const uint32_t* seed_epoch, hipStream_t st) {
    return pooled_head_bwd_common(dout, z_pre_bf16, W, dz_bf16, dx, dx_bf16, nullptr, B, L, D, N, act, drop_p, seed, emit_drop_p,
                                  emit_seed, seed_epoch, st);
}

int mm_pooled_head_bwd_rows(const float* dout, const void* z_pre_bf16, const float* W, void* dz_bf16, float* rows_out,
                            void* dx_bf16, int B, int L, int D, int N, int act, float drop_p, uint32_t seed,
                            float emit_drop_p, uint32_t emit_seed, const uint32_t* seed_epoch, hipStream_t st) {
    MM_REQUIRE(rows_out && dx_bf16, "pooled_head_bwd_rows: null");
    return pooled_head_bwd_common(dout, z_pre_bf16, W, dz_bf16, nullptr, dx_bf16, rows_out, B, L, D, N, act, drop_p, seed,
                                  emit_drop_p, emit_seed, seed_epoch, st);
}

int mm_drop_path(const float* x, float* out, int64_t B, int64_t inner, float drop_p, uint32_t seed,
                 const uint32_t* seed_epoch, hipStream_t st) {
    MM_REQUIRE(x && out && B > 0 && inner > 0 && drop_p >= 0.f && drop_p < 1.f, "drop_path: bad args");
    const uint32_t thresh = (uint32_t)fminf(drop_p * 4294967296.f, 4294967295.f);
    hipLaunchKernelGGL(drop_path_kernel, dim3(grid_h((size_t)(B * inner))), dim3(256), 0, st, x, out, (size_t)(B * inner),
                       (size_t)inner, thresh, 1.f / (1.f - drop_p), seed, seed_epoch);
    return mm_check_launch("drop_path");
}

int mm_meanpool_bf16(const void* x, float* out, int R, int S, int N, hipStream_t st) {
    MM_REQUIRE(x && out && R > 0 && S > 0 && N > 0, "meanpool_bf16: null");
    hipLaunchKernelGGL(meanpool_bf16_kernel, dim3(R), dim3(128), 0, st, (const bf16*)x, out, S, N);
    return mm_check_launch("meanpool_bf16");
}

}
```

### multimodal_eeg_fmri_amd/ops.py

```python
from __future__ import annotations

import functools
import math
import os
import weakref
from typing import Dict, List, Optional

import torch

from . import _hip

ACT = {"none": 0, "gelu": 1, "relu": 2, "tanh": 3, "sigmoid": 4}
_BF = torch.bfloat16
_F32 = torch.float32


def _need_gpu(*tensors):
    for t in tensors:
        if t is not None and not t.is_cuda:
            raise _hip.HipLibraryError(
                "multimodal_eeg_fmri_amd runs on the MI355X HIP path only: got a CPU tensor "
                "(no CPU / eager-PyTorch fallback is provided)")
    _hip.load()

# ... 193 lines not shown
    def seed(self, w: torch.Tensor, wf: torch.Tensor, wd, cinp: int, coutp: int):
        self._store[id(w)] = ((w.data_ptr(), w._version, self._gen, tuple(w.shape)), wf, wd, cinp, coutp, weakref.ref(w))

    def get(self, w: torch.Tensor, need_dgrad: bool, key=None):
        owner = w if key is None else key
        if self._rec is not None and not getattr(owner, "_mm_transient", False):
            self._rec.append((owner, None if key is None else tuple(w.shape), bool(need_dgrad)))
        k = id(owner)
        ver = (owner.data_ptr(), owner._version, self._gen, tuple(w.shape))
        hit = self._store.get(k)
        if (hit is not None and hit[5]() is owner and hit[0] == ver
                and (hit[2] is not None or not need_dgrad)):
            return hit[1], hit[2], hit[3], hit[4]
        wd3 = self._as3d(w)
        cout, cin, k3 = wd3.shape
        cinp, coutp = cpad(cin), cpad(cout)
        wf = _empty((cout, k3, cinp), _BF, w)
        wd = _empty((cinp, k3, coutp), _BF, w) if need_dgrad else None
        _hip.call("mm_prep_conv_weight", wd3, wf, wd, cout, cin, k3, cinp, coutp if need_dgrad else 0)
        if len(self._store) > 4096:
            self._store = {i: e for i, e in self._store.items() if e[5]() is not None}
        self._store[k] = (ver, wf, wd, cinp, coutp, weakref.ref(owner))
        return wf, wd, cinp, coutp


weights = _WeightCache()


def weights_changed():
    weights.invalidate()


def pack_nct(x: torch.Tensor) -> torch.Tensor:
    B, C, T = x.shape
    cp = cpad(C)
    y = _empty((B, T, cp), _BF, x)
    _hip.call("mm_pack_nct_bf16", x.contiguous(), y, B, C, T, cp)
    return y


def igemm(x: torch.Tensor, wf: torch.Tensor, taps: int, pad: int, cout: int, *,
          scale=None, shift=None, act="none", residual=None, pe=None, pool=1, stats=None,
          out_f32=False, out_bf16=True, out_pre=False, drop_p=0.0, seed=0, gradz=None, gradz_act="none"):
    B, T, cin = x.shape
    res = {}
    of = _empty((B, T // pool, cout), _F32, x) if out_f32 else None
    ob = _empty((B, T // pool, cout), _BF, x) if out_bf16 else None
    op = _empty((B, T, cout), _BF, x) if out_pre else None
    args = (x, wf, B, T, cin, cout, taps, pad, scale, shift, ACT[act], residual, pe,
            pool, stats, of, ob, op, float(drop_p), int(seed), EP(), gradz, ACT[gradz_act])
    nsplit, ws_floats = _splitk_plan(B, T, cin, cout, taps)
    if nsplit > 1:
        _hip.call("mm_conv1d_fwd_splitk", *args, _empty((ws_floats,), _F32, x), nsplit)
    else:
        _hip.call("mm_conv1d_fwd", *args)
    res["f32"], res["bf16"], res["pre"] = of, ob, op
    return res


_SPLITK_PLANS: Dict[tuple, tuple] = {}


def _splitk_plan(B: int, T: int, cin: int, cout: int, taps: int):
    if taps == 1:
        return 1, 0
    key = (B, T, cin, cout, taps)
    plan = _SPLITK_PLANS.get(key)
    if plan is None:
        import ctypes
        n, ws = ctypes.c_int(0), ctypes.c_int64(0)
        _hip.call("mm_conv1d_fwd_splitk_plan", B, T, cin, cout, taps, ctypes.addressof(n), ctypes.addressof(ws))
        plan = _SPLITK_PLANS[key] = (n.value, ws.value)
    return plan


def clip_loss_ws_floats(B: int, Bg: int, grouped: bool = False) -> int:
    return _hip.host_int("mm_clip_loss_grouped_ws_floats" if grouped else "mm_clip_loss_ws_floats", B, Bg)


def clip_loss_grouped_ws_floats(B: int, Bg: int) -> int:
    return clip_loss_ws_floats(B, Bg, grouped=True)


def clip_loss_own_rows(z_all, gid_all, logit_scale1, scal, dz, B: int, row0: int):
    Bg, N2 = z_all.shape
    ws = _empty((clip_loss_ws_floats(B, Bg, gid_all is not None),), _F32, z_all)
    if gid_all is None:
        _hip.call("mm_clip_loss_own_rows", z_all, logit_scale1, scal, dz, ws, B, Bg, N2 // 2, row0)
    else:
        _hip.call("mm_clip_loss_own_rows_grouped", z_all, gid_all, logit_scale1, scal, dz, ws, B, Bg, N2 // 2, row0)


def group_ids(groups, n: int, device=None, who: str = "groups") -> Optional[torch.Tensor]:
    if groups is None:
        return None
    if not isinstance(groups, torch.Tensor):
        raise ValueError(f"{who}: group ids must be a torch.Tensor (got {type(groups).__name__})")
    if groups.dim() != 1 or groups.shape[0] != n:
        raise ValueError(f"{who}: group ids must have shape ({n},) (got {tuple(groups.shape)})")
    if groups.dtype.is_floating_point or groups.dtype.is_complex or groups.dtype == torch.bool:
        raise ValueError(f"{who}: group ids must be an integer tensor (got {groups.dtype})")
    if groups.is_cuda:
        if groups.dtype != torch.int32:
            raise ValueError(f"{who}: group ids on the device must be int32 (got {groups.dtype}); host tensors of any integer "
                             "dtype are converted")
        if device is not None and groups.device != torch.device(device):
            raise ValueError(f"{who}: group ids are on {groups.device}, the batch on {device}")
        return groups.contiguous()
    if n and groups.dtype != torch.int32:
        g64 = groups.long()
        if bool((g64 < -2 ** 31).any()) or bool((g64 >= 2 ** 31).any()):
            raise ValueError(f"{who}: group ids must fit in int32")
    g32 = groups.to(torch.int32).contiguous()
    return g32 if device is None else g32.to(device)


def linear_rows(x2d: torch.Tensor, weight: torch.Tensor, bias, *, act="none", residual=None,
                out_f32=False, out_bf16=True, out_pre=False, drop_p=0.0, seed=0, need_dgrad=False):
    M, K = x2d.shape
    wf, _, cinp, _ = weights.get(weight, need_dgrad)
    if cinp != K:
        raise _hip.HipLibraryError(f"linear: activation width {K} != padded weight width {cinp}")
    r = igemm(x2d.view(1, M, K), wf, 1, 0, weight.shape[0], shift=bias, act=act,
              residual=residual, out_f32=out_f32, out_bf16=out_bf16, out_pre=out_pre,
              drop_p=drop_p, seed=seed)
    return {k: (v.view(-1, v.shape[-1]) if v is not None else None) for k, v in r.items()}


def bn_fold_eval(bn, conv_bias) -> torch.Tensor:
    n = bn.num_features
    out4 = _empty((4, n), _F32, bn.weight)
    _hip.call("mm_bn_finalize", None, bn.weight, bn.bias, bn.running_mean, bn.running_var,
              conv_bias, out4, n, 1.0, 0.0, float(bn.eps), 1, None)
    return out4


def bn_finalize_train(bn, stats, count) -> torch.Tensor:
    n = bn.num_features
    out4 = _empty((4, n), _F32, bn.weight)
    mom = 0.1 if bn.momentum is None else float(bn.momentum)
    _hip.call("mm_bn_finalize", stats, bn.weight, bn.bias, bn.running_mean, bn.running_var,
              None, out4, n, float(count), mom, float(bn.eps), 0, bn.num_batches_tracked)
    return out4


def bn_fin_desc(bn, stats, count):
    import ctypes
    import struct
    n = bn.num_features
    out4 = _empty((4, n), _F32, bn.weight)
    mom = 0.1 if bn.momentum is None else float(bn.momentum)
    nb = bn.num_batches_tracked
    raw = struct.pack("<QQQQQQQfffi", stats.data_ptr(), bn.weight.data_ptr(), bn.bias.data_ptr(), bn.running_mean.data_ptr(),
                      bn.running_var.data_ptr(), out4.data_ptr(), nb.data_ptr() if nb is not None else 0,
                      float(count), mom, float(bn.eps), 0)
    buf = ctypes.create_string_buffer(raw, len(raw))
    return buf, out4


def layernorm(x2d: torch.Tensor, ln, want_stat: bool):
    M, D = x2d.shape
    out = _empty((M, D), _BF, x2d)
    stat = _empty((M, 2), _F32, x2d) if want_stat else None
    _hip.call("mm_layernorm_fwd", x2d, ln.weight, ln.bias, out, None, stat, M, D, float(ln.eps))
    return out, stat


def attn_effective_dropout(p: float) -> float:
    return round(256.0 * float(p)) / 256.0


def attention(qkv: torch.Tensor, nhead: int, want_lse: bool, drop_p: float = 0.0, seed: int = 0, mask=None):
    if 0.0 < float(drop_p) < 1.0 / 512.0:
# ... 106 lines not shown
    x2 = x.view(M, D)
    fuse_ln = D == 128 and M % 32 == 0
    h1, st1 = prenorm[:2] if prenorm is not None else layernorm(x2, blk.norm1, save)
    if prenorm is not None and len(prenorm) > 2:
        qkv = prenorm[2]
    else:
        qkv = linear_rows(h1, blk.self_attn.in_proj_weight, blk.self_attn.in_proj_bias,
                          need_dgrad=need_dgrad)["bf16"]
    pa = float(blk.self_attn.dropout) if training else 0.0
    sa = _next_seed() if pa > 0 else 0
    o, lse = attention(qkv.view(B, L, 3 * D), blk.nhead, save, pa, sa, mask)
    s1 = _next_seed() if p > 0 else 0
    f1 = None
    s2 = None
    if fuse_ln:
        wf, _, cinp, _ = weights.get(blk.self_attn.out_proj.weight, need_dgrad)
        x1 = _empty((M, D), _F32, x)
        h2 = _empty((M, D), _BF, x)
        st2 = _empty((M, 2), _F32, x) if save else None
        w1, _, c1, _ = weights.get(blk.linear1.weight, need_dgrad)
        n1 = blk.linear1.weight.shape[0]
        if c1 == 128 and n1 % 128 == 0 and M * n1 < (1 << 32) and not _NO_FFN1_FUSE:
            s2 = _next_seed() if p > 0 else 0
            g1 = _empty((M, n1), _BF, x)
            z1 = _empty((M, n1), _BF, x) if save else None
            _hip.call("mm_linear_fwd_ln_gemm2_act", o.view(M, D), wf, M, cinp, blk.self_attn.out_proj.bias, x2, x1, float(p),
                      int(s1), EP(), blk.norm2.weight, blk.norm2.bias, float(blk.norm2.eps), h2, st2, w1, blk.linear1.bias,
                      n1, g1, z1, ACT[blk._act], float(p), int(s2))
            f1 = {"bf16": g1, "pre": z1, "f32": None}
        else:
            _hip.call("mm_linear_fwd_ln", o.view(M, D), wf, M, cinp, blk.self_attn.out_proj.bias, x2, x1, float(p), int(s1),
                      EP(), blk.norm2.weight, blk.norm2.bias, float(blk.norm2.eps), h2, st2)
    else:
        x1 = linear_rows(o.view(M, D), blk.self_attn.out_proj.weight, blk.self_attn.out_proj.bias,
                         residual=x2, out_f32=True, out_bf16=False, drop_p=p, seed=s1,
                         need_dgrad=need_dgrad)["f32"]
        h2, st2 = layernorm(x1, blk.norm2, save)
    if f1 is None:
        s2 = _next_seed() if p > 0 else 0
        f1 = linear_rows(h2, blk.linear1.weight, blk.linear1.bias, act=blk._act, out_pre=save,
                         drop_p=p, seed=s2, need_dgrad=need_dgrad)
    s3 = _next_seed() if p > 0 else 0
    nxt = None
    if pool_out is not None:
        wf, _, cinp, _ = weights.get(blk.linear2.weight, need_dgrad)
        x2o = _empty((M, D), _F32, x)
        _hip.call("mm_linear_fwd_meanpool", f1["bf16"], wf, M, cinp, blk.linear2.bias, x1, x2o, float(p), int(s3),
                  EP(), pool_out, L)
    elif next_norm is not None and fuse_ln:
        wf, _, cinp, _ = weights.get(blk.linear2.weight, need_dgrad)
        x2o = _empty((M, D), _F32, x)
        hn = _empty((M, D), _BF, x)
        stn = _empty((M, 2), _F32, x) if save else None
        wq = None
        if next_blk is not None and not _NO_QKV_FUSE:
            wq, _, cq, _ = weights.get(next_blk.self_attn.in_proj_weight, need_dgrad)
            if cq != 128 or next_blk.self_attn.in_proj_weight.shape[0] % 128:
                wq = None
        if wq is not None:
            nq = next_blk.self_attn.in_proj_weight.shape[0]
            qn = _empty((M, nq), _BF, x)
            _hip.call("mm_linear_fwd_ln_gemm2", f1["bf16"], wf, M, cinp, blk.linear2.bias, x1, x2o, float(p), int(s3), EP(),
                      next_norm.weight, next_norm.bias, float(next_norm.eps), hn, stn, wq, next_blk.self_attn.in_proj_bias,
                      nq, qn)
            nxt = (hn, stn, qn)
        else:
            _hip.call("mm_linear_fwd_ln", f1["bf16"], wf, M, cinp, blk.linear2.bias, x1, x2o, float(p), int(s3), EP(),
                      next_norm.weight, next_norm.bias, float(next_norm.eps), hn, stn)
            nxt = (hn, stn)
    else:
        x2o = linear_rows(f1["bf16"], blk.linear2.weight, blk.linear2.bias, residual=x1, out_f32=True,
                          out_bf16=False, drop_p=p, seed=s3, need_dgrad=need_dgrad)["f32"]
    saved = None
    if save:
        saved = dict(x=x2, h1=h1, st1=st1, qkv=qkv, o=o, lse=lse, x1=x1, h2=h2, st2=st2,
                     z=f1["pre"], g=f1["bf16"], p=p, seeds=(s1, s2, s3), attn_drop=(pa, sa), B=B, L=L, blk=blk,
                     mask=mask)
    if next_norm is not None:
        return x2o.view(B, L, D), saved, nxt
    return x2o.view(B, L, D), saved


def pooled_head_fwd(x: torch.Tensor, lin, *, act="gelu", training=False, drop_p=0.0,
                    need_dgrad=False, save=None, pooled_f32=None):
    B, L, D = x.shape
    pooled_acc = pooled_f32 is not None
    save = training if save is None else save
    p = drop_p if training else 0.0
    seed = _next_seed() if p > 0 else 0
    if D % 16 == 0 and D <= 1024:
        if pooled_f32 is None:
            pooled_f32 = _empty((B, D), _F32, x)
            _hip.call("mm_meanpool_fwd", x, pooled_f32, None, B, L, D)
        N = lin.weight.shape[0]
        out = _empty((B, N), _F32, x)
        z = _empty((B, N), _BF, x) if save else None
        pooled = _empty((B, D), _BF, x) if save else None
        _hip.call("mm_pooled_head_fwd", None if pooled_acc else pooled_f32, pooled_f32 if pooled_acc else None,
                  lin.weight, lin.bias, out, z, pooled, B, D, N, ACT[act], float(p), int(seed), EP())
        saved = dict(pooled=pooled, z=z, seed=seed, drop_p=p, B=B, L=L, D=D, lin=lin, act=act, fused=True) if save else None
        return out, saved
    pooled = _empty((B, D), _BF, x)
    _hip.call("mm_meanpool_fwd", x, None, pooled, B, L, D)
    r = linear_rows(pooled, lin.weight, lin.bias, act=act, out_f32=True, out_bf16=False,
                    out_pre=save, drop_p=p, seed=seed, need_dgrad=need_dgrad)
    saved = dict(pooled=pooled, z=r["pre"], seed=seed, drop_p=p, B=B, L=L, D=D, lin=lin,
                 act=act) if save else None
    return r["f32"], saved


def pe_table(pos_encoder, L: int) -> torch.Tensor:
    pe = pos_encoder.pe
    if L > pe.shape[0]:
        raise ValueError(f"sequence length {L} exceeds PositionalEncoding max_len {pe.shape[0]}")
    return pe[:L, 0, :].contiguous()


def _encoder_tail_impl(m, h, training: bool, need_dgrad: bool, save: bool, prenorm=None, stages=None):
    blocks = []
    B, L, D = h.shape
    nblk = len(m.transformer_layers)
    pooled = _zeros((B, 2 * D), h) if nblk and L % 32 == 0 and D == 128 else None
    layers = list(m.transformer_layers)
    for i, blk in enumerate(layers):
        if i < nblk - 1:
            h, s, prenorm = transformer_block_fwd(h, blk, training, need_dgrad, save=save, prenorm=prenorm,
                                                  next_norm=layers[i + 1].norm1, next_blk=layers[i + 1])
        else:
            h, s = transformer_block_fwd(h, blk, training, need_dgrad, save=save, pool_out=pooled, prenorm=prenorm)
        blocks.append(s)
        if stages is not None:
            stages[f"block{i}"] = h.clone()
    out, s = pooled_head_fwd(h, m.output_proj[2], training=training, drop_p=m.drop_p, need_dgrad=need_dgrad,
                             save=save, pooled_f32=pooled)
    return out, blocks, s, h


def _erp_forward_impl(m, x: torch.Tensor, training: bool, need_dgrad: bool, save=None, xb=None, stages=None):
    cl = m.conv_layers
    save = training if save is None else save
    p = m.drop_p if training else 0.0
    if xb is None:
        xb = pack_nct(x)
    saved = []
    saved_in = []
    r, s = conv_bn_act(xb, cl[0], cl[1], training=training, drop_p=p, need_dgrad=need_dgrad, save=save)
    saved.append(s)
    saved_in.append(r["bf16"])
    r, s = conv_bn_act(r["bf16"], cl[4], cl[5], pool=2, training=training, drop_p=p,
                       drop_first=False, need_dgrad=need_dgrad, save=save)
    saved.append(s)
    saved_in.append(r["bf16"])
    L = r["bf16"].shape[1]
    r, s = conv_bn_act(r["bf16"], cl[9], cl[10], training=training, drop_p=p,
                       pe=pe_table(m.pos_encoder, L), pe_drop_p=(m.pos_encoder.dropout.p if training else 0.0),
                       want_f32=True, want_bf16=False, need_dgrad=need_dgrad, save=save,
                       next_norm=m.transformer_layers[0].norm1 if len(m.transformer_layers) else None)
    saved.append(s)
    if stages is not None:
        stages["conv1"], stages["conv2"] = saved_in[0].clone(), saved_in[1].clone()
        stages["pos"] = r["f32"].clone()
        if not save:
            wf3 = weights.get(cl[9].weight, need_dgrad)[0]
            o4 = bn_fold_eval(cl[10], cl[9].bias)
            stages["conv3"] = igemm(saved_in[1], wf3, cl[9].kernel_size[0], cl[9].padding[0], cl[9].out_channels,
                                    scale=o4[0], shift=o4[1], act="gelu", out_f32=True, out_bf16=False)["f32"]
    out, blocks, s, h = _encoder_tail_impl(m, r["f32"], training, need_dgrad, save, prenorm=r.get("prenorm"), stages=stages)
    return out, dict(convs=saved, blocks=blocks, head=s, x_shape=tuple(x.shape), tokens=h)


def erp_encoder_forward(m, x: torch.Tensor) -> torch.Tensor:
    _need_gpu(x)
    if m.training or _wants_grad(m, x):
        from .autograd import ErpEncoderFn
        return ErpEncoderFn.run(m, x)
    with torch.no_grad():
        return _erp_forward_impl(m, x.float(), False, False)[0]


def _wants_grad(m, x) -> bool:
    return torch.is_grad_enabled() and (x.requires_grad or any(p.requires_grad for p in m.parameters()))


def add_positional(x, pe, drop_p, training):
    _need_gpu(x)
    if x.dim() != 3:
        raise ValueError("PositionalEncoding: expected a 3-D input (batch, seq, d_model) or (seq, 1, d_model)")
    L = x.size(1) if x.size(1) != 1 else x.size(0)
    if L > pe.shape[0]:
        raise ValueError(f"sequence length {L} exceeds PositionalEncoding max_len {pe.shape[0]}")
    from .autograd import AddPositionalFn
    return AddPositionalFn.apply(x, pe, float(drop_p) if training else 0.0)


def add_positional_impl(x, pe, p: float, seed: int, backward: bool = False):
    shape = x.shape
    if x.size(1) != 1:
        B, L, D = shape
    else:
        L, B, D = shape[0], 1, shape[2]
    xf = x.float().contiguous()
    tab = None if backward else pe[:L, 0, :].contiguous()
    out = _empty(tuple(shape), _F32, xf)
    _hip.call("mm_add_pe", xf, tab, out, None, B, L, D, float(p), int(seed), EP())
    return out


def transformer_block(x, blk, training, mask=None):
    _need_gpu(x)
    mask = additive_attn_mask(mask, x.shape[1], x)
    if training or (torch.is_grad_enabled() and x.requires_grad):
        from .autograd import TransformerBlockFn
        return TransformerBlockFn.run(blk, x, mask)
    with torch.no_grad():
        return transformer_block_fwd(x.float().contiguous(), blk, False, mask=mask)[0]


def pack_volume(x: torch.Tensor) -> torch.Tensor:
    B, C, D, H, W = x.shape
    if C != 1:
        raise _hip.HipLibraryError("fMRIVolumeEncoder3D: single-channel volumes only")
    y = _empty((B, D, H, W, 16), _BF, x)
    _hip.call("mm_pack_volume_bf16", x.contiguous(), y, B * D * H * W, 16)
    return y


def conv3d_bn_act(xv: torch.Tensor, conv, bn, *, pool: bool, training: bool, drop_p: float,
                  need_dgrad: bool, save=None):
    save = training if save is None else save
    B, D, H, W, cinp = xv.shape
    cout = conv.out_channels
    wf, _, cp, _ = weights.get(conv.weight, need_dgrad)
    assert cp == cinp, (cp, cinp)
    y = _empty((B, D, H, W, cout), _BF if pool else _F32, xv)
    yf, yb = (None, y) if pool else (y, None)
    fin = None
    if training:
        stats = _zeros((REPL, 2, cout), xv)
        cal = kernel_timer.bracket(f"event_pair_c{cinp}")
        if cal is not None:
            cal.record()
        end = kernel_timer.bracket(f"conv3d_fwd_c{cinp}")
        _hip.call("mm_conv3d_fwd", xv, wf, B, D, H, W, cinp, cout, conv.bias, stats, yf, yb)
        if end is not None:
            end.record()
        if cout <= 256:
            fin, out4 = bn_fin_desc(bn, stats, B * D * H * W)
        else:
            out4 = bn_finalize_train(bn, stats, B * D * H * W)
    elif save:
# ... 63 lines not shown
        winners.append(arg)
    else:
        _hip.call("mm_conv3d_l1", 1, x, wimg, bias, out4, None, None, None, out, None, None,
                  B, D, H, W, 1 if training else 0, float(p), seed, EP())
    saved = dict(l1=True, x=x, wimg=wimg, out4=out4, drop_p=p, seed=seed, conv=conv, bn=bn, train=training, gramc=gramc) if save else None
    return out, saved


def check_volume_shape(shape):
    if len(shape) != 5:
        raise ValueError(f"fMRIVolumeEncoder3D: expected a (B, C, D, H, W) volume batch, got shape {tuple(shape)}")
    if min(shape[2:]) < 4:
        raise ValueError(f"fMRIVolumeEncoder3D: every spatial extent must be >= 4 (two MaxPool3d(2) layers), "
                         f"got D, H, W = {tuple(shape[2:])}")


def _vol_forward_impl(m, x: torch.Tensor, training: bool, need_dgrad: bool, save=None, need_dx: bool = False, winners=None):
    save = training if save is None else save
    cl = m.conv_layers
    p = m.drop_p
    saved = []
    B, C, D, H, W = x.shape
    check_volume_shape(x.shape)
    x = x.contiguous()
    if C == 1 and cl[0].out_channels == 32 and not need_dx:
        h, s = conv3d_l1_bn_act(x, cl[0], cl[1], training=training, drop_p=p, save=save, winners=winners)
    else:
        h, s = conv3d_bn_act(pack_volume(x), cl[0], cl[1], pool=True, training=training, drop_p=p,
                             need_dgrad=need_dgrad or need_dx, save=save)
    saved.append(s)
    h, s = conv3d_bn_act(h, cl[5], cl[6], pool=True, training=training, drop_p=p, need_dgrad=need_dgrad, save=save)
    saved.append(s)
    if winners is not None:
        if len(winners) == 0:
            winners.append(saved[0]["arg"])
        winners.append(s["arg"])
    h, s = conv3d_bn_act(h, cl[10], cl[11], pool=False, training=training, drop_p=p, need_dgrad=need_dgrad, save=save)
    saved.append(s)
    out, hs = pooled_head_fwd(h, m.output_proj[2], training=training, drop_p=p, need_dgrad=need_dgrad, save=save)
    return out, dict(convs=saved, head=hs, x_shape=tuple(x.shape), need_dx=need_dx)


def volume_encoder_forward(m, x: torch.Tensor) -> torch.Tensor:
    check_volume_shape(x.shape)
    _need_gpu(x)
    if m.training or _wants_grad(m, x):
        from .autograd import VolumeEncoderFn
        return VolumeEncoderFn.run(m, x)
    with torch.no_grad():
        return _vol_forward_impl(m, x.float(), False, False)[0]


def small_linear(x: torch.Tensor, lin, *, act="none", drop_p=0.0, seed=0, want_pre=False, bn=None,
                 weight=None, bias=None):
    W = lin.weight if weight is None else weight
    bvec = (lin.bias if lin is not None else None) if bias is None else bias
    B, K = x.shape
    N = W.shape[0]
    y = _empty((B, N), _F32, x)
    pre = _empty((B, N), _F32, x) if want_pre else None
    sc = sh = None
    if bn is not None:
        out4 = bn_fold_eval(bn, None)
        sc, sh = out4[0], out4[1]
    _hip.call("mm_small_linear_fwd", x, W, bvec, sc, sh, y, pre, B, K, N, ACT[act], float(drop_p), int(seed), EP())
    return y, pre


def proj_head_fwd(seq, x: torch.Tensor, training: bool, drop_p: float):
    lin, ln = seq[0], seq[1]
    B = x.shape[0]
    N = lin.weight.shape[0]
    z1, _ = small_linear(x, lin)
    hn = _empty((B, N), _F32, x)
    stat = _empty((B, 2), _F32, x)
    _hip.call("mm_layernorm_fwd", z1, ln.weight, ln.bias, None, hn, stat, B, N, float(ln.eps))
    p = drop_p if training else 0.0
    seed = _next_seed() if p > 0 else 0
    a = _empty((B, N), _F32, x)
    _hip.call("mm_act_f32", hn, a, B * N, ACT["gelu"], float(p), seed, EP())
    return a, dict(x=x, z1=z1, hn=hn, stat=stat, p=p, seed=seed, seq=seq)


def contrastive_embed_impl(bridge, eeg: torch.Tensor, fmri: torch.Tensor, training: bool):
    B = eeg.shape[0]
    N = bridge.bridge_dim
    xe, xf = eeg.float().contiguous(), fmri.float().contiguous()
    (le, lne), (lf, lnf) = bridge.eeg_proj[:2], bridge.fmri_proj[:2]
    assert lne.eps == lnf.eps
    p = float(bridge.drop_p) if training else 0.0
    se, sf = (_next_seed(), _next_seed()) if p > 0 else (0, 0)
    z = _empty((B, 2 * N), _F32, eeg)
    nrm = _empty((2, B), _F32, eeg)
    z1 = _empty((2, B, N), _F32, eeg)
    hn = _empty((2, B, N), _F32, eeg)
    stat = _empty((2, B, 2), _F32, eeg)
    _hip.call("mm_proj_heads_fwd", xe, le.weight, le.bias, lne.weight, lne.bias, xe.shape[1],
              xf, lf.weight, lf.bias, lnf.weight, lnf.bias, xf.shape[1],
              z1, hn, stat, z, nrm, B, N, float(lne.eps), p, se, sf, EP())
    return z, dict(xe=xe, xf=xf, z1=z1, hn=hn, stat=stat, z=z, nrm=nrm, B=B, N=N, p=p, seeds=(se, sf), bridge=bridge)


def proj_embed_one(bridge, x: torch.Tensor, modality: str) -> torch.Tensor:
    _need_gpu(x)
    if modality not in ("eeg", "fmri"):
        raise ValueError(f"proj_embed_one: modality must be 'eeg' or 'fmri', got {modality!r}")
    B = x.shape[0]
    N = bridge.bridge_dim
    xc = x.detach().float().contiguous()
    lin, ln = (bridge.eeg_proj if modality == "eeg" else bridge.fmri_proj)[:2]
    z = _empty((B, 2 * N), _F32, x)
    nrm = _empty((2, B), _F32, x)
    z1 = _empty((2, B, N), _F32, x)
    hn = _empty((2, B, N), _F32, x)
    stat = _empty((2, B, 2), _F32, x)
    _hip.call("mm_proj_heads_fwd", xc, lin.weight, lin.bias, ln.weight, ln.bias, xc.shape[1],
              xc, lin.weight, lin.bias, ln.weight, ln.bias, xc.shape[1],
              z1, hn, stat, z, nrm, B, N, float(ln.eps), 0.0, 0, 0, EP())
    return z[:, :N].contiguous()


def retrieval_ws_floats(nq: int, ng: int, d: int, k: int) -> int:
    return _hip.host_int("mm_retrieval_ws_floats", nq, ng, d, k)


@functools.lru_cache(maxsize=None)
def retrieval_kmax() -> int:
    import re
    m = re.search(r"^#define\s+MM_RETRIEVAL_KMAX\s+(\d+)", open(_hip.header_path()).read(), flags=re.M)
    return int(m.group(1))


def retrieval_grouped_ws_floats(nq: int, ng: int, d: int) -> int:
    return _hip.host_int("mm_retrieval_grouped_ws_floats", nq, ng, d)


def retrieval(q: torch.Tensor, g: torch.Tensor, positives: Optional[torch.Tensor] = None, k: int = 0,
              ranks: bool = True, q_groups: Optional[torch.Tensor] = None, g_groups: Optional[torch.Tensor] = None):
    grouped = q_groups is not None or g_groups is not None
    if grouped:
        if q_groups is None or g_groups is None:
            raise ValueError("retrieval: give both q_groups and g_groups, or neither")
        if positives is not None:
            raise ValueError("retrieval: positives and group ids are exclusive")
        if not ranks or int(k) != 0:
            raise ValueError("retrieval: with group ids only ranks are computed (ranks=True, k = 0; top-k does not depend on groups)")
    for name, t in (("q", q), ("g", g)):
        if not isinstance(t, torch.Tensor) or t.dim() != 2:
            raise ValueError(f"retrieval: {name} must be a 2-D tensor")
        if not t.is_cuda:
            raise _hip.HipLibraryError(f"retrieval: {name} is a CPU tensor; the HIP path has no CPU fallback")
        if t.dtype != torch.float32:
            raise ValueError(f"retrieval: {name} must be float32 (got {t.dtype})")
        if not t.is_contiguous():
            raise ValueError(f"retrieval: {name} must be contiguous")
    _hip.load()
    nq, d = q.shape
    ng = g.shape[0]
    if g.shape[1] != d:
        raise ValueError(f"retrieval: q has D = {d}, g has D = {g.shape[1]}")
    if q.device != g.device:
        raise ValueError("retrieval: q and g are on different devices")
    if grouped:
        qg = group_ids(q_groups, nq, q.device, "retrieval: q_groups")
        gg = group_ids(g_groups, ng, q.device, "retrieval: g_groups")
        ws = torch.empty(retrieval_grouped_ws_floats(nq, ng, d), dtype=_F32, device=q.device)
        r32 = torch.empty(nq, dtype=torch.int32, device=q.device)
        with torch.cuda.device(q.device):
            _hip.call("mm_retrieval_grouped", q, g, qg, gg, r32, ws, nq, ng, d)
        return r32.long(), None, None
    k = int(k)
    if not 0 <= k <= min(retrieval_kmax(), ng):
        raise ValueError(f"retrieval: k must be in [0, min({retrieval_kmax()}, Ng = {ng})] (got {k})")
    if not ranks and k == 0:
        raise ValueError("retrieval: nothing to compute (ranks=False and k = 0)")
    pos = None
    if ranks:
        if positives is None:
            if nq > ng:
                raise ValueError(f"retrieval: without positives query i pairs with gallery row i, so Nq ({nq}) <= Ng ({ng})")
        else:
            if positives.shape != (nq,):
# ... 526 lines not shown
        out = _empty((B, frames, cp), _BF, x)
    else:
        spec = None
        out = torch.zeros((B, frames, cp), dtype=_BF, device=x.device) if cp != total else _empty((B, frames, cp), _BF, x)
    off = 0
    for n, wdt in zip(n_ffts, widths):
        _hip.call("mm_stft_power", xc, None if normalize else out, spec, B, C, T, int(n), int(hop), off, cp)
        off += wdt
    if normalize:
        _hip.call("mm_sample_zscore_bf16", spec, out, _empty((64 * B,), torch.float64, x), B, frames, total, cp, 1e-8)
    return (out, spec) if keep_spec else out


def stft_power_encoder_forward(m, x):
    _need_gpu(x)
    enc = m.encoder
    if enc.training or _wants_grad(enc, x):
        from .autograd import PowerEncoderFn, StftFrontEndFn
        if x.requires_grad and torch.is_grad_enabled():
            spec = StftFrontEndFn.apply(x, m.n_ffts, m.hop, m.normalize)
        else:
            with torch.no_grad():
                spec = stft_front_end(x, m.n_ffts, m.hop, m.normalize)
        return PowerEncoderFn.run(enc, spec, packed=True)
    with torch.no_grad():
        return _power_forward_ntc(enc, stft_front_end(x, m.n_ffts, m.hop, m.normalize))


def power_encoder_forward(m, x):
    _need_gpu(x)
    if m.training or _wants_grad(m, x):
        from .autograd import PowerEncoderFn
        return PowerEncoderFn.run(m, x)
    with torch.no_grad():
        return _power_forward_ntc(m, pack_nct(x.float()))


class _Merged:

    def __init__(self, **kw):
        self.__dict__.update(kw)


def power_merge_call(mode: int, parts, merged, tracked=(None, None, None), cin: int = 0, ks=(3, 5, 7), cinp: int = 0):
    import ctypes
    import struct
    ptr = lambda t: 0 if t is None else t.data_ptr()
    flat = [ptr(t) for trip in parts for t in trip] + [ptr(t) for t in tracked] + [ptr(t) for t in merged]
    buf = struct.pack("<27Q6i", *flat, int(cin), *[int(k) for k in ks], int(cinp), 0)
    host = ctypes.create_string_buffer(buf, len(buf))
    _hip.call("mm_power_merge", ctypes.addressof(host), int(mode))


def _power_merged_train(m, need_dgrad: bool = True):
    seqs = (m.conv_scale1, m.conv_scale2, m.conv_scale3)
    ref = seqs[0][0].weight
    cin = seqs[0][0].in_channels
    ks = tuple(s[0].kernel_size[0] for s in seqs)
    assert all(s[0].out_channels == 64 and s[0].in_channels == cin and s[0].weight.dtype == _F32 for s in seqs), "three 64-channel branches"
    w = _empty((192, cin, 7), _F32, ref)
    vec = [_empty((192,), _F32, ref) for _ in range(5)]
    parts = ([s[0].weight.detach() for s in seqs], [s[0].bias.detach() for s in seqs], [s[1].weight.detach() for s in seqs],
             [s[1].bias.detach() for s in seqs], [s[1].running_mean for s in seqs], [s[1].running_var for s in seqs])
    if need_dgrad:
        power_merge_call(0, parts, [w] + vec, cin=cin, ks=ks)
    else:
        cinp = cpad(cin)
        wf = _empty((192, 7, cinp), _BF, ref)
        power_merge_call(3, parts, [wf] + vec, cin=cin, ks=ks, cinp=cinp)
        weights.seed(w, wf, None, cinp, cpad(192))
    w._mm_transient = True
    conv = _Merged(weight=w.requires_grad_(any(s[0].weight.requires_grad for s in seqs)),
                   bias=vec[0].requires_grad_(any(s[0].bias.requires_grad for s in seqs)),
                   kernel_size=(7,), padding=(3,), in_channels=cin, out_channels=192,
                   parts=[(s[0].weight, 64 * i) for i, s in enumerate(seqs)])
    bn = _Merged(weight=vec[1].requires_grad_(any(s[1].weight.requires_grad for s in seqs)),
                 bias=vec[2].requires_grad_(any(s[1].bias.requires_grad for s in seqs)),
                 running_mean=vec[3], running_var=vec[4],
                 num_batches_tracked=None, num_features=192, eps=seqs[0][1].eps, momentum=seqs[0][1].momentum)
    assert all(s[1].eps == bn.eps and s[1].momentum == bn.momentum for s in seqs)
    return conv, bn, seqs


def _power_forward_impl(m, xb: torch.Tensor, training: bool, need_dgrad: bool, save=None):
    save = training if save is None else save
    conv, bn, seqs = _power_merged_train(m, need_dgrad)
    r, s0 = conv_bn_act(xb, conv, bn, training=training, need_dgrad=need_dgrad, save=save)
    if training:
        none3 = [None] * 3
        power_merge_call(1, (none3, none3, none3, none3, [sq[1].running_mean for sq in seqs], [sq[1].running_var for sq in seqs]),
                         [None, None, None, None, bn.running_mean, bn.running_var],
                         tracked=[sq[1].num_batches_tracked for sq in seqs], cin=conv.in_channels,
                         ks=[sq[0].kernel_size[0] for sq in seqs])
    T = xb.shape[1]
    p = m.drop_p if training else 0.0
    r, s1 = conv_bn_act(r["bf16"], m.fusion[0], m.fusion[1], training=training, drop_p=p,
                        pe=pe_table(m.pos_encoder, T), pe_drop_p=(m.pos_encoder.dropout.p if training else 0.0),
                        want_f32=True, want_bf16=False, need_dgrad=True, save=save)
    out, blocks, sh, h = _encoder_tail_impl(m, r["f32"], training, True, save)
    return out, dict(convs=[s0, s1], blocks=blocks, head=sh, merged=(conv, bn, seqs), tokens=h)


def _power_forward_ntc(m, xb):
    B, T, cp = xb.shape
    w192, o4 = _power_merged(m, xb.device)
    wf = _empty((192, 7, cp), _BF, xb)
    _hip.call("mm_prep_conv_weight", w192, wf, None, 192, w192.shape[1], 7, cp, 0)
    h = igemm(xb, wf, 7, 3, 192, scale=o4[0], shift=o4[1], act="gelu")["bf16"]
    r, _ = conv_bn_act(h, m.fusion[0], m.fusion[1], training=False, pe=pe_table(m.pos_encoder, T),
                       want_f32=True, want_bf16=False)
    tok = r["f32"]
    for blk in m.transformer_layers:
        tok, _ = transformer_block_fwd(tok, blk, False)
    out, _ = pooled_head_fwd(tok, m.output_proj[2])
    return out


def weighted_cross_entropy(logits, target, weight=None):
    _need_gpu(logits, target)
    from . import small_autograd as sa
    w = weight.float().contiguous() if weight is not None else None
    return sa.WeightedCEFn.apply(logits, target, w)


def focal_loss(logits, target, alpha=0.25, gamma=2.0, reduction="mean"):
    _need_gpu(logits, target)
    from . import small_autograd as sa
    return sa.FocalLossFn.apply(logits, target, float(alpha), float(gamma), reduction)


def drop_path(x, drop_prob):
    _need_gpu(x)
    from . import small_autograd as sa
    return sa.DropPathFn.apply(x, float(drop_prob))


def smoothed_cross_entropy(pred, target, smoothing):
    _need_gpu(pred, target)
    from . import small_autograd as sa
    return sa.SmoothedCEFn.apply(pred, target, float(smoothing))


_ATTRIBUTION = {"depth": 0}


class attribution_mode:

    def __enter__(self):
        _ATTRIBUTION["depth"] += 1
        return self

    def __exit__(self, *exc):
        _ATTRIBUTION["depth"] -= 1
        return False


def attribution_active() -> bool:
    return _ATTRIBUTION["depth"] > 0


def xai_alphas(n_steps: int):
    import numpy as np
    if n_steps < 1:
        raise ValueError("xai_alphas: n_steps must be >= 1")
    if n_steps == 1:
        return np.zeros(1, dtype=np.float32)
    step = 1.0 / float(n_steps - 1)
    a = [float(s) * step for s in range(n_steps)]
    a[-1] = 1.0
    return np.asarray(a, dtype=np.float64).astype(np.float32)


XAI_BUDGET_BYTES = 2 << 30


def ig_chunk_steps(n_steps: int, step_bytes: int, budget_bytes: int = XAI_BUDGET_BYTES) -> int:
    if n_steps < 1 or step_bytes < 1 or budget_bytes < 1:
        raise ValueError("ig_chunk_steps: n_steps, step_bytes and budget_bytes must be positive")
    return max(1, min(int(n_steps), int(budget_bytes) // int(step_bytes)))


def ig_chunks(n_steps: int, chunk_steps: int, first_alone: bool = False):
# ... 128 lines not shown
```

Before: 41990.

## Fuse EEG pooled head into projection heads and CLIP loss into heads backward

Defers the EEG pooled-head launch so it runs inside a new fused kernel together with the contrastive projection heads forward. When the gathered batch is local (single rank), the CLIP loss can also be folded into a fused loss-plus-heads backward kernel. The goal is fewer small kernel launches and fewer global-memory round trips for tiny per-step tensors. Default MM_HEADS_FUSED=1 enables only the forward fusion; level 2 adds the backward fusion, which brings extra code paths and constraints (B==Bg, row0==0).

```diff
diff --git a/include/mmeeg_hip.h b/include/mmeeg_hip.h
--- a/include/mmeeg_hip.h
+++ b/include/mmeeg_hip.h
@@ -214,12 +214,25 @@
                       float* db_e, float* dg_e, float* dbe_e, float* dx_f, float* dW_f, float* db_f, float* dg_f,
                       float* dbe_f, int B, int N, float drop_p, uint32_t seed_e, uint32_t seed_f,
                       const uint32_t* seed_epoch, hipStream_t stream);
+int mm_heads_fwd_fused(const float* pooled, const float* pooled_acc, const float* W_p, const float* b_p, float* x_e,
+                       void* z_pre_bf16, void* pooled_bf16, int D, int act, float drop_p_p, uint32_t seed_p,
+                       const float* W_e, const float* b_e, const float* g_e, const float* be_e, int K_e, const float* x_f,
+                       const float* W_f, const float* b_f, const float* g_f, const float* be_f, int K_f, float* z1,
+                       float* hn, float* stat, float* z, float* nrm, int B, int N, float eps, float drop_p,
+                       uint32_t seed_e, uint32_t seed_f, const uint32_t* seed_epoch, hipStream_t stream);
 int mm_clip_loss_own_rows(const float* z_all, const float* logit_scale, float* scal4, float* dz_local, float* ws,
                           int B, int Bg, int N, int row0, hipStream_t stream);
 int mm_clip_loss_ws_floats(int B, int Bg, int* floats_host, hipStream_t stream);
 int mm_clip_loss_own_rows_grouped(const float* z_all, const int* gid_all, const float* logit_scale, float* scal4,
                                   float* dz_local, float* ws, int B, int Bg, int N, int row0, hipStream_t stream);
 int mm_clip_loss_grouped_ws_floats(int B, int Bg, int* floats_host, hipStream_t stream);
+int mm_clip_heads_bwd_fused(const float* z, const int* gid, const float* logit_scale, float* scal4, float* dz,
+                            const float* nrm, const float* hn, const float* z1, const float* stat, const float* x_e,
+                            const float* W_e, const float* g_e, int K_e, const float* x_f, const float* W_f,
+                            const float* g_f, int K_f, float* dx_e, float* dW_e, float* db_e, float* dg_e, float* dbe_e,
+                            float* dx_f, float* dW_f, float* db_f, float* dg_f, float* dbe_f, int B, int N, float drop_p,
+                            uint32_t seed_e, uint32_t seed_f, const uint32_t* seed_epoch, hipStream_t stream);
+int mm_clip_heads_bwd_fused_ok(int B, int N, int* ok_host, hipStream_t stream);
 
 #define MM_RETRIEVAL_KMAX 16
 #define MM_RETRIEVAL_NMAX (1 << 20)
diff --git a/multimodal_eeg_fmri_amd/autograd.py b/multimodal_eeg_fmri_amd/autograd.py
--- a/multimodal_eeg_fmri_amd/autograd.py
+++ b/multimodal_eeg_fmri_amd/autograd.py
@@ -723,6 +723,15 @@
     dxe = _empty(xe.shape, _F32, dz) if need[0] else None
     dxf = _empty(xf.shape, _F32, dz) if need[1] else None
     t = bag.target
+    loss = s.pop("loss", None)
+    if loss is not None:
+        gid, ls, scal = loss
+        _hip.call("mm_clip_heads_bwd_fused", s["z"], gid, ls, scal, dz, s["nrm"], s["hn"], s["z1"], s["stat"],
+                  xe, le.weight, lne.weight, xe.shape[1], xf, lf.weight, lnf.weight, xf.shape[1],
+                  dxe, t(le.weight), t(le.bias), t(lne.weight), t(lne.bias),
+                  dxf, t(lf.weight), t(lf.bias), t(lnf.weight), t(lnf.bias),
+                  B, N, float(s["p"]), int(s["seeds"][0]), int(s["seeds"][1]), ops.EP())
+        return dxe, dxf
     _hip.call("mm_proj_heads_bwd", dz.contiguous(), s["z"], s["nrm"], s["hn"], s["z1"], s["stat"],
               xe, le.weight, lne.weight, xe.shape[1], xf, lf.weight, lnf.weight, xf.shape[1],
               dxe, t(le.weight), t(le.bias), t(lne.weight), t(lne.bias),
diff --git a/multimodal_eeg_fmri_amd/bridge_trainer.py b/multimodal_eeg_fmri_amd/bridge_trainer.py
--- a/multimodal_eeg_fmri_amd/bridge_trainer.py
+++ b/multimodal_eeg_fmri_amd/bridge_trainer.py
@@ -156,12 +156,13 @@
             return out
         if self._fmri_longer:
             ff, sv_f = fmri_branch()
-        fe, sv_e = self._eeg_forward(eeg, xb)
+        defer = ops.heads_fused_level() >= 1
+        fe, sv_e = self._eeg_forward(eeg, xb, defer)
         self._stamp(2)
         if not self._fmri_longer:
             ff, sv_f = fmri_branch()
         main.wait_stream(self._side)
-        z, sv_h = ops.contrastive_embed_impl(self.head.bridge, fe, ff, True)
+        z, sv_h = ops.contrastive_embed_impl(self.head.bridge, fe, ff, True, eeg_head=sv_e["head"] if defer else None)
         self._stamp(5)
         return z, (sv_e, sv_f, sv_h)
 
@@ -172,19 +173,21 @@
             return env == "1"
         return fmri[0].numel() >= 4 * 32 ** 3
 
-    def _eeg_forward(self, eeg, xb):
+    def _eeg_forward(self, eeg, xb, defer_head=False):
         enc = self.eeg_encoder
         if self._eeg_kind == "erp":
-            return ops._erp_forward_impl(enc, eeg, True, True, xb=xb)
+            return ops._erp_forward_impl(enc, eeg, True, True, xb=xb, defer_head=defer_head)
         if self._eeg_kind == "power":
-            return ops._power_forward_impl(enc, xb if xb is not None else ops.pack_nct(eeg), True, False)
+            return ops._power_forward_impl(enc, xb if xb is not None else ops.pack_nct(eeg), True, False, defer_head=defer_head)
         spec = ops.stft_front_end(eeg, enc.n_ffts, enc.hop, enc.normalize)
-        return ops._power_forward_impl(enc.encoder, spec, True, False)
-
-    def _seg_loss(self, z_all, scal, dz, gid_all=None):
+        return ops._power_forward_impl(enc.encoder, spec, True, False, defer_head=defer_head)
+
+    def _seg_loss(self, z_all, scal, dz, gid_all=None, heads=None):
         ls = self.head.logit_scale.detach().reshape(1)
-        ops.clip_loss_own_rows(z_all, gid_all, ls, scal, dz, dz.shape[0], dp.rank(self.group) * dz.shape[0])
-        self._stamp(6)
+        self._loss_in_bwd = ops.clip_loss_own_rows(z_all, gid_all, ls, scal, dz, dz.shape[0], dp.rank(self.group) * dz.shape[0],
+                                                   heads=heads)
+        if not self._loss_in_bwd:
+            self._stamp(6)
 
     def _reduce_group(self, ready: str):
         for name, rdy, lo, hi in self.groups:
@@ -198,6 +201,9 @@
         with deferred(bag, dz.device):
             bag.defer(scal.data_ptr() + 12, self.head.logit_scale._mm_grad.view(1), 1, 1, 1, keep=scal)
             dfe, dff = contrastive_embed_bwd(bag, sv_h, dz)
+            if getattr(self, "_loss_in_bwd", False):
+                self._stamp(6)
+                self._loss_in_bwd = False
             self._stamp(7)
             main = torch.cuda.current_stream()
             self._side.wait_stream(main)
@@ -295,7 +301,7 @@
         z, saved = self._seg_forward(eeg, fmri)
         z_all = dp.gather_embeddings(z, self.group)
         scal, dz = self._scal, ops._empty(tuple(z.shape), torch.float32, z)
-        self._seg_loss(z_all, scal, dz, gid_all)
+        self._seg_loss(z_all, scal, dz, gid_all, heads=saved[2] if z_all is z else None)
         early = dp.active(self.group)
         self._seg_backward(saved, dz, scal, reduce=early)
         self._seg_optimizer(reduced=early)
@@ -367,7 +373,7 @@
                 z, saved = self._seg_forward(c["eeg"], c["fmri"], xb=c["xb"])
                 c["z"] = z
                 c["dz"] = ops._empty(tuple(z.shape), torch.float32, z)
-                self._seg_loss(z, c["scal"], c["dz"], c["gid_all"])
+                self._seg_loss(z, c["scal"], c["dz"], c["gid_all"], heads=saved[2])
                 self._seg_backward(saved, c["dz"], c["scal"])
                 self._grad_probe()
                 self._seg_adamw()
diff --git a/multimodal_eeg_fmri_amd/csrc/heads.hip b/multimodal_eeg_fmri_amd/csrc/heads.hip
--- a/multimodal_eeg_fmri_amd/csrc/heads.hip
+++ b/multimodal_eeg_fmri_amd/csrc/heads.hip
@@ -111,12 +111,13 @@
     return (red[0] + red[1]) + (red[2] + red[3]);
 }
 
-__global__ __launch_bounds__(256) void proj_heads_fwd_kernel(HeadsArgs a) {
-    __shared__ float xs[HEAD_MAXK], v[HEAD_MAXN], red[4];
-    const int b = blockIdx.x, m = blockIdx.y, tid = threadIdx.x, lane = tid & 63, wave = tid >> 6;
+__device__ __forceinline__ void proj_heads_fwd_row(const HeadsArgs& a, int b, int m, bool xs_ready, float* xs ,
+                                                   float* v , float* red ) {
+    const int tid = threadIdx.x, lane = tid & 63, wave = tid >> 6;
     const HeadSide s = a.s[m];
     const int N = a.N, K = s.K;
-    for (int k = tid; k < K; k += 256) xs[k] = s.x[(size_t)b * K + k];
+    if (!xs_ready)
+        for (int k = tid; k < K; k += 256) xs[k] = s.x[(size_t)b * K + k];
     __syncthreads();
     const int T = N <= 64 ? 4 : (N <= 128 ? 2 : 1);
     {
@@ -161,14 +162,18 @@
     }
 }
 
+__global__ __launch_bounds__(256) void proj_heads_fwd_kernel(HeadsArgs a) {
+    __shared__ float xs[HEAD_MAXK], v[HEAD_MAXN], red[4];
+    proj_heads_fwd_row(a, blockIdx.x, blockIdx.y, false, xs, v, red);
+}
+
 constexpr int HB_RC = 32;
 template <int NE>
-__global__ __launch_bounds__(1024) void proj_heads_bwd_kernel(HeadsArgs a) {
-    __shared__ float d1[HB_RC][HEAD_MAXN];
-    __shared__ float px[1024];
-    const int j = blockIdx.x, m = blockIdx.y, tid = threadIdx.x, lane = tid & 63, wave = tid >> 6;
+__device__ __forceinline__ void proj_heads_bwd_block(const HeadsArgs& a, const float* dz, int dz_ld, int dz_off, int j, int m, int G,
+                                                     float (*d1)[HEAD_MAXN], float* px ) {
+    const int tid = threadIdx.x, lane = tid & 63, wave = tid >> 6;
     const HeadSide s = a.s[m];
-    const int N = a.N, K = s.K, B = a.B, G = gridDim.x;
+    const int N = a.N, K = s.K, B = a.B;
     const int NK = N * K, S = (NK + G - 1) / G;
     const uint32_t seed = mm_eff_seed(s.seed, a.epoch);
     float ag[NE], ab[NE], gam[NE];
@@ -193,7 +198,7 @@
             for (int e = 0; e < NE; ++e) {
                 const int n = lane + 64 * e;
                 const bool on = row_on && n < N;
-                dzv[q][e] = on ? a.dz[oz + n] : 0.f;
+                dzv[q][e] = on ? dz[(size_t)b * dz_ld + dz_off + n] : 0.f;
                 zv[q][e] = on ? a.z[oz + n] : 0.f;
                 hnv[q][e] = on ? a.hn[o + n] : 0.f;
                 z1v[q][e] = on ? a.z1[o + n] : 0.f;
@@ -288,6 +293,13 @@
     }
 }
 
+template <int NE>
+__global__ __launch_bounds__(1024) void proj_heads_bwd_kernel(HeadsArgs a) {
+    __shared__ float d1[HB_RC][HEAD_MAXN];
+    __shared__ float px[1024];
+    proj_heads_bwd_block<NE>(a, a.dz, 2 * a.N, blockIdx.y * a.N, blockIdx.x, blockIdx.y, gridDim.x, d1, px);
+}
+
 struct ClipShared {
     float *qe, *qf, *cr, *cc, *red;
 };
@@ -296,9 +308,10 @@
     s.qe = sm; s.qf = sm + N; s.cr = s.qf + N; s.cc = s.cr + Bg; s.red = s.cc + Bg;
     return s;
 }
+__device__ __forceinline__ int clip_tid() { return threadIdx.x & 255; }
 __device__ __forceinline__ void clip_cosines(const float* __restrict__ z_all, int r, int Bg, int N, const ClipShared& sh,
                                              float& mxr, float& mxc) {
-    const int LD = 2 * N, tid = threadIdx.x, lane = tid & 63, wave = tid >> 6;
+    const int LD = 2 * N, tid = clip_tid(), lane = tid & 63, wave = tid >> 6;
     for (int n = tid; n < N; n += 256) { sh.qe[n] = z_all[(size_t)r * LD + n]; sh.qf[n] = z_all[(size_t)r * LD + N + n]; }
     __syncthreads();
     float a_mx = -INFINITY, c_mx = -INFINITY;
@@ -327,7 +340,7 @@
     __syncthreads();
 }
 __device__ __forceinline__ void clip_sum2(float& a, float& c, float* red) {
-    const int lane = threadIdx.x & 63, wave = threadIdx.x >> 6;
+    const int lane = clip_tid() & 63, wave = clip_tid() >> 6;
     a = wave_sum(a); c = wave_sum(c);
     if (lane == 0) { red[wave] = a; red[4 + wave] = c; }
     __syncthreads();
@@ -336,7 +349,7 @@
     __syncthreads();
 }
 __device__ __forceinline__ void clip_max2(float& a, float& c, float* red) {
-    const int lane = threadIdx.x & 63, wave = threadIdx.x >> 6;
+    const int lane = clip_tid() & 63, wave = clip_tid() >> 6;
     a = wave_max(a); c = wave_max(c);
     if (lane == 0) { red[wave] = a; red[4 + wave] = c; }
     __syncthreads();
@@ -346,12 +359,9 @@
 }
 
 template <bool GROUPED>
-__global__ __launch_bounds__(256) void clip_lse_kernel(const float* __restrict__ z_all, const float* __restrict__ logit_scale,
-                                                       float* __restrict__ ws, int Bg, int N, const int* __restrict__ gid) {
-    extern __shared__ float sm[];
-    const ClipShared sh = clip_shared(sm, N, Bg);
-    const int r = blockIdx.x, tid = threadIdx.x;
-    const float s = __expf(logit_scale[0]);
+__device__ __forceinline__ void clip_lse_row(const float* __restrict__ z_all, float s, float* __restrict__ ws, int r, int Bg, int N,
+                                             const ClipShared& sh, const int* __restrict__ gid, bool write) {
+    const int tid = clip_tid();
     int gr = 0;
     if constexpr (GROUPED) gr = gid[r];
     float mxr, mxc;
@@ -381,7 +391,7 @@
         clip_sum2(qe, qf, sh.red);
         clip_sum2(qee, qef, sh.red);
     }
-    if (tid == 0) {
+    if (tid == 0 && write) {
         if constexpr (GROUPED) {
             const float lse_r = s * mxr + __logf(se), lse_c = s * mxc + __logf(sf);
             const float lsp_r = s * pmr + __logf(qe), lsp_c = s * pmc + __logf(qf);
@@ -406,6 +416,73 @@
     }
 }
 
+__device__ __forceinline__ void clip_scalars(const float* __restrict__ ws, float* __restrict__ scal, int B, int Bg, int row0) {
+    const int tid = threadIdx.x;
+    float acc[4] = {0.f, 0.f, 0.f, 0.f};
+    for (int r0 = 0; r0 < B; r0 += 64) {
+        float v[4];
+#pragma unroll
+        for (int q = 0; q < 4; ++q) v[q] = (r0 + tid < B) ? ws[(size_t)(2 + q) * Bg + row0 + r0 + tid] : 0.f;
+#pragma unroll
+        for (int q = 0; q < 4; ++q) acc[q] += wave_sum(v[q]);
+    }
+    if (tid < 4) scal[tid] = (tid == 0 ? acc[0] : tid == 1 ? acc[1] : tid == 2 ? acc[2] : acc[3]) * (1.f / (float)B);
+}
+
+template <bool GROUPED>
+__device__ __forceinline__ void clip_dz_row(const float* __restrict__ z_all, float s, const float* __restrict__ ws, int gi, int B,
+                                            int Bg, int N, const ClipShared& sh, const int* __restrict__ gid,
+                                            float* __restrict__ orow, int n_lo, int n_hi, bool on) {
+    const int tid = clip_tid(), LD = 2 * N;
+    const float invB = 1.f / (float)B;
+    if (on) {
+        const float lse_rg = ws[gi], lse_cg = ws[Bg + gi];
+        float lsp_rg = 0.f, lsp_cg = 0.f;
+        int gg = 0;
+        if constexpr (GROUPED) { lsp_rg = ws[6 * Bg + gi]; lsp_cg = ws[7 * Bg + gi]; gg = gid[gi]; }
+        const float k = 0.5f * invB * s;
+        for (int j = tid; j < Bg; j += 256) {
+            const float a = s * sh.cr[j], c = s * sh.cc[j];
+            float ga = __expf(a - lse_rg) + __expf(a - ws[Bg + j]);
+            float gc = __expf(c - ws[j]) + __expf(c - lse_cg);
+            if constexpr (GROUPED) {
+                if (gid[j] == gg) {
+                    ga -= __expf(a - lsp_rg) + __expf(a - ws[7 * Bg + j]);
+                    gc -= __expf(c - ws[6 * Bg + j]) + __expf(c - lsp_cg);
+                }
+            } else {
+                if (j == gi) { ga -= 2.f; gc -= 2.f; }
+            }
+            sh.cr[j] = k * ga; sh.cc[j] = k * gc;
+        }
+    }
+    __syncthreads();
+    if (!on) return;
+    for (int n = n_lo + tid; n < n_hi; n += 256) {
+        const bool first = n < N;
+        const float* g = first ? sh.cr : sh.cc;
+        const float* col = z_all + (first ? N + n : n - N);
+        float acc = 0.f;
+        int j = 0;
+        for (; j + 8 <= Bg; j += 8) {
+            float v[8];
+#pragma unroll
+            for (int q = 0; q < 8; ++q) v[q] = col[(size_t)(j + q) * LD];
+#pragma unroll
+            for (int q = 0; q < 8; ++q) acc += g[j + q] * v[q];
+        }
+        for (; j < Bg; ++j) acc += g[j] * col[(size_t)j * LD];
+        orow[n - n_lo] = acc;
+    }
+}
+
+template <bool GROUPED>
+__global__ __launch_bounds__(256) void clip_lse_kernel(const float* __restrict__ z_all, const float* __restrict__ logit_scale,
+                                                       float* __restrict__ ws, int Bg, int N, const int* __restrict__ gid) {
+    extern __shared__ float sm[];
+    clip_lse_row<GROUPED>(z_all, __expf(logit_scale[0]), ws, blockIdx.x, Bg, N, clip_shared(sm, N, Bg), gid, true);
+}
+
 template <bool GROUPED>
 __global__ __launch_bounds__(256) void clip_rows_kernel(const float* __restrict__ z_all, const float* __restrict__ logit_scale,
                                                         const float* __restrict__ ws, float* __restrict__ scal,
@@ -413,60 +490,63 @@
                                                         const int* __restrict__ gid) {
     extern __shared__ float sm[];
     const ClipShared sh = clip_shared(sm, N, Bg);
-    const int i = blockIdx.x, gi = row0 + i, tid = threadIdx.x, LD = 2 * N;
-    const float s = __expf(logit_scale[0]);
-    const float invB = 1.f / (float)B;
-    if (i == 0 && tid < 64) {
-        float acc[4] = {0.f, 0.f, 0.f, 0.f};
-        for (int r0 = 0; r0 < B; r0 += 64) {
-            float v[4];
-#pragma unroll
-            for (int q = 0; q < 4; ++q) v[q] = (r0 + tid < B) ? ws[(size_t)(2 + q) * Bg + row0 + r0 + tid] : 0.f;
-#pragma unroll
-            for (int q = 0; q < 4; ++q) acc[q] += wave_sum(v[q]);
-        }
-        if (tid < 4) scal[tid] = (tid == 0 ? acc[0] : tid == 1 ? acc[1] : tid == 2 ? acc[2] : acc[3]) * invB;
-    }
+    const int i = blockIdx.x, gi = row0 + i;
+    if (i == 0 && threadIdx.x < 64) clip_scalars(ws, scal, B, Bg, row0);
     if (!dz) return;
     float mxr, mxc;
     clip_cosines(z_all, gi, Bg, N, sh, mxr, mxc);
-    const float lse_rg = ws[gi], lse_cg = ws[Bg + gi];
-    float lsp_rg = 0.f, lsp_cg = 0.f;
-    int gg = 0;
-    if constexpr (GROUPED) { lsp_rg = ws[6 * Bg + gi]; lsp_cg = ws[7 * Bg + gi]; gg = gid[gi]; }
-    const float k = 0.5f * invB * s;
-    for (int j = tid; j < Bg; j += 256) {
-        const float a = s * sh.cr[j], c = s * sh.cc[j];
-        float ga = __expf(a - lse_rg) + __expf(a - ws[Bg + j]);
-        float gc = __expf(c - ws[j]) + __expf(c - lse_cg);
-        if constexpr (GROUPED) {
-            if (gid[j] == gg) {
-                ga -= __expf(a - lsp_rg) + __expf(a - ws[7 * Bg + j]);
-                gc -= __expf(c - ws[6 * Bg + j]) + __expf(c - lsp_cg);
-            }
-        } else {
-            if (j == gi) { ga -= 2.f; gc -= 2.f; }
-        }
-        sh.cr[j] = k * ga; sh.cc[j] = k * gc;
-    }
-    __syncthreads();
-    float* orow = dz + (size_t)i * LD;
-    for (int n = tid; n < 2 * N; n += 256) {
-        const bool first = n < N;
-        const float* g = first ? sh.cr : sh.cc;
-        const float* col = z_all + (first ? N + n : n - N);
-        float acc = 0.f;
-        int j = 0;
-        for (; j + 8 <= Bg; j += 8) {
-            float v[8];
-#pragma unroll
-            for (int q = 0; q < 8; ++q) v[q] = col[(size_t)(j + q) * LD];
-#pragma unroll
-            for (int q = 0; q < 8; ++q) acc += g[j + q] * v[q];
-        }
-        for (; j < Bg; ++j) acc += g[j] * col[(size_t)j * LD];
-        orow[n] = acc;
-    }
+    clip_dz_row<GROUPED>(z_all, __expf(logit_scale[0]), ws, gi, B, Bg, N, sh, gid, dz + (size_t)i * 2 * N, 0, 2 * N, true);
+}
+
+constexpr int FUSED_MAXB = 32;
+struct ClipFusedArgs {
+    const float* logit_scale; float* scal; float* dz; const int* gid;
+};
+__host__ __device__ constexpr int clip_fused_team_floats(int B, int N) { return 2 * N + 2 * B + 32; }
+__host__ __device__ constexpr int clip_fused_lds_floats(int B, int N) {
+    return B * 2 * N + 2 * B * B + 8 * B + B * N + 4 * clip_fused_team_floats(B, N) + B;
+}
+
+template <int NE, bool GROUPED>
+__global__ __launch_bounds__(1024) void clip_heads_bwd_fused_kernel(HeadsArgs a, ClipFusedArgs c) {
+    __shared__ float d1[HB_RC][HEAD_MAXN];
+    __shared__ float px[1024];
+    extern __shared__ __attribute__((aligned(16))) float fsm[];
+    const int j = blockIdx.x, m = blockIdx.y, tid = threadIdx.x, team = tid >> 8;
+    const int N = a.N, B = a.B, LD = 2 * N;
+    float* zs = fsm;
+    float* CR = zs + B * LD;
+    float* CC = CR + B * B;
+    float* ws = CC + B * B;
+    float* dzs = ws + 8 * B;
+    float* tm = dzs + B * N + team * clip_fused_team_floats(B, N);
+    int* gs = reinterpret_cast<int*>(dzs + B * N + 4 * clip_fused_team_floats(B, N));
+    for (int i = tid; i < B * LD / 4; i += 1024)
+        reinterpret_cast<float4*>(zs)[i] = reinterpret_cast<const float4*>(a.z)[i];
+    if constexpr (GROUPED)
+        for (int i = tid; i < B; i += 1024) gs[i] = c.gid[i];
+    const float s = __expf(c.logit_scale[0]);
+    __syncthreads();
+    const bool full = j == 0 && m == 0;
+    ClipShared sh;
+    sh.qe = tm; sh.qf = tm + N; sh.red = tm + 2 * N + 2 * B;
+    for (int r0 = 0; r0 < B; r0 += 4) {
+        const bool on = r0 + team < B;
+        const int r = on ? r0 + team : B - 1;
+        sh.cr = on ? CR + r * B : tm + 2 * N; sh.cc = on ? CC + r * B : tm + 2 * N + B;
+        clip_lse_row<GROUPED>(zs, s, ws, r, B, N, sh, gs, on);
+    }
+    __syncthreads();
+    if (full && tid < 64) clip_scalars(ws, c.scal, B, B, 0);
+    for (int r0 = 0; r0 < B; r0 += 4) {
+        const bool on = r0 + team < B;
+        const int r = on ? r0 + team : B - 1;
+        sh.cr = CR + r * B; sh.cc = CC + r * B;
+        clip_dz_row<GROUPED>(zs, s, ws, r, B, B, N, sh, gs, full ? c.dz + (size_t)r * LD : dzs + r * N,
+                             full ? 0 : m * N, full ? LD : (m + 1) * N, on);
+    }
+    __syncthreads();
+    proj_heads_bwd_block<NE>(a, full ? c.dz : dzs, full ? LD : N, full ? m * N : 0, j, m, gridDim.x, d1, px);
 }
 
 constexpr int SUMSQ_SLOTS = 1024;
@@ -1327,14 +1407,17 @@
     for (size_t i = (size_t)blockIdx.x * blockDim.x + threadIdx.x; i < n; i += (size_t)gridDim.x * blockDim.x) o[i] = a[i] * b[i];
 }
 
-__global__ __launch_bounds__(256) void pooled_head_fwd_kernel(const float* __restrict__ pooled, const mm_acc_t* __restrict__ pooled_acc,
-                                                             const float* __restrict__ W,
-                                                             const float* __restrict__ bias, float* __restrict__ out,
-                                                             bf16* __restrict__ z_pre, bf16* __restrict__ pooled_bf16,
-                                                             int D, int N, int act, uint32_t thresh, float inv_keep,
-                                                             uint32_t seed, const uint32_t* __restrict__ epoch) {
-    __shared__ float xs[1024];
-    const int b = blockIdx.x;
+struct PooledHeadFwdArgs {
+    const float* pooled; const mm_acc_t* pooled_acc; const float* W; const float* bias; float* out; bf16* z_pre; bf16* pooled_bf16;
+    int D, N, act; uint32_t thresh; float inv_keep; uint32_t seed; const uint32_t* epoch;
+};
+__device__ __forceinline__ void pooled_head_fwd_row(const PooledHeadFwdArgs& p, int b, float* xs, float* out_lds) {
+    const float* __restrict__ pooled = p.pooled; const mm_acc_t* __restrict__ pooled_acc = p.pooled_acc;
+    const float* __restrict__ W = p.W; const float* __restrict__ bias = p.bias; float* __restrict__ out = p.out;
+    bf16* __restrict__ z_pre = p.z_pre; bf16* __restrict__ pooled_bf16 = p.pooled_bf16;
+    const int D = p.D, N = p.N, act = p.act;
+    const uint32_t thresh = p.thresh; const float inv_keep = p.inv_keep; uint32_t seed = p.seed;
+    const uint32_t* __restrict__ epoch = p.epoch;
     for (int k = threadIdx.x; k < D; k += 256) {
         const float v = pooled ? pooled[(size_t)b * D + k] : acc_val<MM_ACC_GRAD>(pooled_acc[(size_t)b * D + k]);
         xs[k] = v;
@@ -1370,7 +1453,21 @@
         float v = apply_act(z, act);
         if (thresh) v *= dropout_scale(seed, (uint32_t)idx, thresh, inv_keep);
         out[idx] = v;
-    }
+        if (out_lds) out_lds[n] = v;
+    }
+}
+
+__global__ __launch_bounds__(256) void pooled_head_fwd_kernel(PooledHeadFwdArgs p) {
+    __shared__ float xs[1024];
+    pooled_head_fwd_row(p, blockIdx.x, xs, nullptr);
+}
+
+__global__ __launch_bounds__(256) void heads_fwd_fused_kernel(PooledHeadFwdArgs p, HeadsArgs a) {
+    __shared__ float xp[1024];
+    __shared__ float xs[HEAD_MAXK], v[HEAD_MAXN], red[4];
+    const int b = blockIdx.x, m = blockIdx.y;
+    if (m == 0) pooled_head_fwd_row(p, b, xp, xs);
+    proj_heads_fwd_row(a, b, m, m == 0, xs, v, red);
 }
 
 __global__ __launch_bounds__(256) void pooled_head_bwd_kernel(const float* __restrict__ dout, const bf16* __restrict__ z_pre,
@@ -1448,6 +1545,20 @@
 inline uint32_t thresh_h(float p) { return p > 0.f ? (uint32_t)((double)p * 4294967296.0) : 0u; }
 inline int grid_h(size_t n, int cap = 2048) { size_t g = (n + 255) / 256; return (int)(g < (size_t)cap ? (g ? g : 1) : cap); }
 
+template <bool GROUPED>
+static void clip_heads_bwd_fused_launch(const HeadsArgs& a, const ClipFusedArgs& c, size_t lds, hipStream_t st) {
+    auto go = [&](auto kern) {
+        (void)hipFuncSetAttribute(reinterpret_cast<const void*>(kern), hipFuncAttributeMaxDynamicSharedMemorySize, (int)lds);
+        hipLaunchKernelGGL(kern, dim3(a.B, 2), dim3(1024), lds, st, a, c);
+    };
+    switch (ceil_div(a.N, 64)) {
+        case 1: go(clip_heads_bwd_fused_kernel<1, GROUPED>); break;
+        case 2: go(clip_heads_bwd_fused_kernel<2, GROUPED>); break;
+        case 3: go(clip_heads_bwd_fused_kernel<3, GROUPED>); break;
+        default: go(clip_heads_bwd_fused_kernel<4, GROUPED>); break;
+    }
+}
+
 }
 
 extern "C" {
@@ -1495,6 +1606,18 @@
     return mm_check_launch("colstats");
 }
 
+static HeadsArgs heads_fwd_args(const float* x_e, const float* W_e, const float* b_e, const float* g_e, const float* be_e, int K_e,
+                                const float* x_f, const float* W_f, const float* b_f, const float* g_f, const float* be_f, int K_f,
+                                float* z1, float* hn, float* stat, float* z, float* nrm, int B, int N, float eps, float drop_p,
+                                uint32_t seed_e, uint32_t seed_f, const uint32_t* seed_epoch) {
+    HeadsArgs a{};
+    a.s[0].x = x_e; a.s[0].W = W_e; a.s[0].bias = b_e; a.s[0].gamma = g_e; a.s[0].beta = be_e; a.s[0].K = K_e; a.s[0].seed = seed_e;
+    a.s[1].x = x_f; a.s[1].W = W_f; a.s[1].bias = b_f; a.s[1].gamma = g_f; a.s[1].beta = be_f; a.s[1].K = K_f; a.s[1].seed = seed_f;
+    a.z1 = z1; a.hn = hn; a.stat = stat; a.z = z; a.nrm = nrm; a.B = B; a.N = N; a.eps = eps;
+    a.thresh = thresh_h(drop_p); a.inv_keep = drop_p > 0.f ? 1.f / (1.f - drop_p) : 1.f; a.epoch = seed_epoch;
+    return a;
+}
+
 int mm_proj_heads_fwd(const float* x_e, const float* W_e, const float* b_e, const float* g_e, const float* be_e, int K_e,
                       const float* x_f, const float* W_f, const float* b_f, const float* g_f, const float* be_f, int K_f,
                       float* z1, float* hn, float* stat, float* z, float* nrm, int B, int N, float eps, float drop_p,
@@ -1503,13 +1626,27 @@
     MM_REQUIRE((!z1 && !hn && !stat) || (z1 && hn && stat), "proj_heads_fwd: z1/hn/stat go together");
     MM_REQUIRE(B > 0 && N > 0 && N <= HEAD_MAXN && K_e > 0 && K_e <= HEAD_MAXK && K_f > 0 && K_f <= HEAD_MAXK,
                "proj_heads_fwd: B=%d N=%d K=%d/%d", B, N, K_e, K_f);
-    HeadsArgs a{};
-    a.s[0].x = x_e; a.s[0].W = W_e; a.s[0].bias = b_e; a.s[0].gamma = g_e; a.s[0].beta = be_e; a.s[0].K = K_e; a.s[0].seed = seed_e;
-    a.s[1].x = x_f; a.s[1].W = W_f; a.s[1].bias = b_f; a.s[1].gamma = g_f; a.s[1].beta = be_f; a.s[1].K = K_f; a.s[1].seed = seed_f;
-    a.z1 = z1; a.hn = hn; a.stat = stat; a.z = z; a.nrm = nrm; a.B = B; a.N = N; a.eps = eps;
-    a.thresh = thresh_h(drop_p); a.inv_keep = drop_p > 0.f ? 1.f / (1.f - drop_p) : 1.f; a.epoch = seed_epoch;
+    const HeadsArgs a = heads_fwd_args(x_e, W_e, b_e, g_e, be_e, K_e, x_f, W_f, b_f, g_f, be_f, K_f, z1, hn, stat, z, nrm, B, N, eps,
+                                       drop_p, seed_e, seed_f, seed_epoch);
     hipLaunchKernelGGL(proj_heads_fwd_kernel, dim3(B, 2), dim3(256), 0, st, a);
     return mm_check_launch("proj_heads_fwd");
+}
+
+static HeadsArgs heads_bwd_args(const float* dz, const float* z, const float* nrm, const float* hn, const float* z1,
+                                const float* stat, const float* x_e, const float* W_e, const float* g_e, int K_e,
+                                const float* x_f, const float* W_f, const float* g_f, int K_f, float* dx_e, float* dW_e,
+                                float* db_e, float* dg_e, float* dbe_e, float* dx_f, float* dW_f, float* db_f, float* dg_f,
+                                float* dbe_f, int B, int N, float drop_p, uint32_t seed_e, uint32_t seed_f,
+                                const uint32_t* seed_epoch) {
+    HeadsArgs a{};
+    a.s[0].x = x_e; a.s[0].W = W_e; a.s[0].gamma = g_e; a.s[0].K = K_e; a.s[0].seed = seed_e;
+    a.s[0].dx = dx_e; a.s[0].dW = dW_e; a.s[0].dbias = db_e; a.s[0].dgamma = dg_e; a.s[0].dbeta = dbe_e;
+    a.s[1].x = x_f; a.s[1].W = W_f; a.s[1].gamma = g_f; a.s[1].K = K_f; a.s[1].seed = seed_f;
+    a.s[1].dx = dx_f; a.s[1].dW = dW_f; a.s[1].dbias = db_f; a.s[1].dgamma = dg_f; a.s[1].dbeta = dbe_f;
+    a.z1 = const_cast<float*>(z1); a.hn = const_cast<float*>(hn); a.stat = const_cast<float*>(stat);
+    a.z = const_cast<float*>(z); a.nrm = const_cast<float*>(nrm); a.dz = dz; a.B = B; a.N = N;
+    a.thresh = thresh_h(drop_p); a.inv_keep = drop_p > 0.f ? 1.f / (1.f - drop_p) : 1.f; a.epoch = seed_epoch;
+    return a;
 }
 
 int mm_proj_heads_bwd(const float* dz, const float* z, const float* nrm, const float* hn, const float* z1,
@@ -1521,14 +1658,8 @@
     MM_REQUIRE(dz && z && nrm && hn && z1 && stat && x_e && W_e && g_e && x_f && W_f && g_f, "proj_heads_bwd: null");
     MM_REQUIRE(B > 0 && N > 0 && N <= HEAD_MAXN && K_e > 0 && K_e <= HEAD_MAXK && K_f > 0 && K_f <= HEAD_MAXK,
                "proj_heads_bwd: B=%d N=%d K=%d/%d", B, N, K_e, K_f);
-    HeadsArgs a{};
-    a.s[0].x = x_e; a.s[0].W = W_e; a.s[0].gamma = g_e; a.s[0].K = K_e; a.s[0].seed = seed_e;
-    a.s[0].dx = dx_e; a.s[0].dW = dW_e; a.s[0].dbias = db_e; a.s[0].dgamma = dg_e; a.s[0].dbeta = dbe_e;
-    a.s[1].x = x_f; a.s[1].W = W_f; a.s[1].gamma = g_f; a.s[1].K = K_f; a.s[1].seed = seed_f;
-    a.s[1].dx = dx_f; a.s[1].dW = dW_f; a.s[1].dbias = db_f; a.s[1].dgamma = dg_f; a.s[1].dbeta = dbe_f;
-    a.z1 = const_cast<float*>(z1); a.hn = const_cast<float*>(hn); a.stat = const_cast<float*>(stat);
-    a.z = const_cast<float*>(z); a.nrm = const_cast<float*>(nrm); a.dz = dz; a.B = B; a.N = N;
-    a.thresh = thresh_h(drop_p); a.inv_keep = drop_p > 0.f ? 1.f / (1.f - drop_p) : 1.f; a.epoch = seed_epoch;
+    const HeadsArgs a = heads_bwd_args(dz, z, nrm, hn, z1, stat, x_e, W_e, g_e, K_e, x_f, W_f, g_f, K_f, dx_e, dW_e, db_e, dg_e, dbe_e,
+                                       dx_f, dW_f, db_f, dg_f, dbe_f, B, N, drop_p, seed_e, seed_f, seed_epoch);
     switch (ceil_div(N, 64)) {
         case 1: hipLaunchKernelGGL(proj_heads_bwd_kernel<1>, dim3(B, 2), dim3(1024), 0, st, a); break;
         case 2: hipLaunchKernelGGL(proj_heads_bwd_kernel<2>, dim3(B, 2), dim3(1024), 0, st, a); break;
@@ -1582,6 +1713,65 @@
     return clip_loss_launch("clip_loss_own_rows_grouped", z_all, gid_all, logit_scale, scal4, dz_local, ws, B, Bg, N, row0, st);
 }
 
+static PooledHeadFwdArgs pooled_head_fwd_args(const float* pooled, const float* pooled_acc, const float* W, const float* bias,
+                                              float* out, void* z_pre_bf16, void* pooled_bf16, int D, int N, int act, float drop_p,
+                                              uint32_t seed, const uint32_t* seed_epoch) {
+    PooledHeadFwdArgs p{};
+    p.pooled = pooled; p.pooled_acc = reinterpret_cast<const mm_acc_t*>(pooled_acc); p.W = W; p.bias = bias; p.out = out;
+    p.z_pre = (bf16*)z_pre_bf16; p.pooled_bf16 = (bf16*)pooled_bf16; p.D = D; p.N = N; p.act = act;
+    p.thresh = drop_p > 0.f ? (uint32_t)((double)drop_p * 4294967296.0) : 0u;
+    p.inv_keep = drop_p > 0.f ? 1.f / (1.f - drop_p) : 1.f; p.seed = seed; p.epoch = seed_epoch;
+    return p;
+}
+
+int mm_heads_fwd_fused(const float* pooled, const float* pooled_acc, const float* W_p, const float* b_p, float* x_e, void* z_pre_bf16,
+                       void* pooled_bf16, int D, int act, float drop_p_p, uint32_t seed_p, const float* W_e, const float* b_e,
+                       const float* g_e, const float* be_e, int K_e, const float* x_f, const float* W_f, const float* b_f,
+                       const float* g_f, const float* be_f, int K_f, float* z1, float* hn, float* stat, float* z, float* nrm,
+                       int B, int N, float eps, float drop_p, uint32_t seed_e, uint32_t seed_f, const uint32_t* seed_epoch,
+                       hipStream_t st) {
+    MM_REQUIRE((pooled != nullptr) != (pooled_acc != nullptr) && W_p && x_e, "heads_fwd_fused: null (exactly one of pooled / pooled_acc)");
+    MM_REQUIRE(D > 0 && D <= 1024 && D % 16 == 0, "heads_fwd_fused: D=%d (multiple of 16, <= 1024)", D);
+    MM_REQUIRE(drop_p_p >= 0.f && drop_p_p < 1.f, "heads_fwd_fused: drop_p");
+    MM_REQUIRE(W_e && g_e && be_e && x_f && W_f && g_f && be_f && z && nrm, "heads_fwd_fused: null");
+    MM_REQUIRE((!z1 && !hn && !stat) || (z1 && hn && stat), "heads_fwd_fused: z1/hn/stat go together");
+    MM_REQUIRE(B > 0 && N > 0 && N <= HEAD_MAXN && K_e > 0 && K_e <= HEAD_MAXK && K_f > 0 && K_f <= HEAD_MAXK,
+               "heads_fwd_fused: B=%d N=%d K=%d/%d", B, N, K_e, K_f);
+    const PooledHeadFwdArgs p = pooled_head_fwd_args(pooled, pooled_acc, W_p, b_p, x_e, z_pre_bf16, pooled_bf16, D, K_e, act, drop_p_p,
+                                                     seed_p, seed_epoch);
+    const HeadsArgs a = heads_fwd_args(x_e, W_e, b_e, g_e, be_e, K_e, x_f, W_f, b_f, g_f, be_f, K_f, z1, hn, stat, z, nrm, B, N, eps,
+                                       drop_p, seed_e, seed_f, seed_epoch);
+    hipLaunchKernelGGL(heads_fwd_fused_kernel, dim3(B, 2), dim3(256), 0, st, p, a);
+    return mm_check_launch("heads_fwd_fused");
+}
+
+int mm_clip_heads_bwd_fused_ok(int B, int N, int* ok_host, hipStream_t) {
+    MM_REQUIRE(ok_host && B > 0 && N > 0, "clip_heads_bwd_fused_ok: bad args");
+    *ok_host = B <= FUSED_MAXB && N <= HEAD_MAXN && N % 4 == 0 &&
+               (size_t)clip_fused_lds_floats(B, N) * sizeof(float) + (HB_RC * HEAD_MAXN + 1024) * sizeof(float) <= 160 * 1024;
+    return 0;
+}
+
+int mm_clip_heads_bwd_fused(const float* z, const int* gid, const float* logit_scale, float* scal4, float* dz, const float* nrm,
+                            const float* hn, const float* z1, const float* stat, const float* x_e, const float* W_e,
+                            const float* g_e, int K_e, const float* x_f, const float* W_f, const float* g_f, int K_f,
+                            float* dx_e, float* dW_e, float* db_e, float* dg_e, float* dbe_e, float* dx_f, float* dW_f,
+                            float* db_f, float* dg_f, float* dbe_f, int B, int N, float drop_p, uint32_t seed_e,
+                            uint32_t seed_f, const uint32_t* seed_epoch, hipStream_t st) {
+    MM_REQUIRE(z && logit_scale && scal4 && dz && nrm && hn && z1 && stat && x_e && W_e && g_e && x_f && W_f && g_f,
+               "clip_heads_bwd_fused: null");
+    MM_REQUIRE(B > 0 && B <= FUSED_MAXB && N > 0 && N <= HEAD_MAXN && N % 4 == 0 && K_e > 0 && K_e <= HEAD_MAXK && K_f > 0 &&
+               K_f <= HEAD_MAXK, "clip_heads_bwd_fused: B=%d (<= %d) N=%d K=%d/%d", B, FUSED_MAXB, N, K_e, K_f);
+    const size_t lds = (size_t)clip_fused_lds_floats(B, N) * sizeof(float);
+    MM_REQUIRE(lds + (HB_RC * HEAD_MAXN + 1024) * sizeof(float) <= 160 * 1024, "clip_heads_bwd_fused: B=%d N=%d do not fit the LDS", B, N);
+    const HeadsArgs a = heads_bwd_args(dz, z, nrm, hn, z1, stat, x_e, W_e, g_e, K_e, x_f, W_f, g_f, K_f, dx_e, dW_e, db_e, dg_e, dbe_e,
+                                       dx_f, dW_f, db_f, dg_f, dbe_f, B, N, drop_p, seed_e, seed_f, seed_epoch);
+    ClipFusedArgs c{logit_scale, scal4, dz, gid};
+    if (gid) clip_heads_bwd_fused_launch<true>(a, c, lds, st);
+    else clip_heads_bwd_fused_launch<false>(a, c, lds, st);
+    return mm_check_launch("clip_heads_bwd_fused");
+}
+
 int mm_sumsq(const float* g, float* state, int64_t n, hipStream_t st) {
     MM_REQUIRE(g && state && n > 0, "sumsq: null");
     hipLaunchKernelGGL(sumsq_kernel, dim3(grid_h((size_t)n, 1024)), dim3(256), 0, st, g, state, (size_t)n);
@@ -1813,9 +2003,8 @@
     MM_REQUIRE((pooled != nullptr) != (pooled_acc != nullptr) && W && out && B > 0, "pooled_head_fwd: null (exactly one of pooled / pooled_acc)");
     MM_REQUIRE(D > 0 && D <= 1024 && D % 16 == 0 && N > 0, "pooled_head_fwd: D=%d (multiple of 16, <= 1024)", D);
     MM_REQUIRE(drop_p >= 0.f && drop_p < 1.f, "pooled_head_fwd: drop_p");
-    const uint32_t thresh = drop_p > 0.f ? (uint32_t)((double)drop_p * 4294967296.0) : 0u;
-    hipLaunchKernelGGL(pooled_head_fwd_kernel, dim3(B), dim3(256), 0, st, pooled, reinterpret_cast<const mm_acc_t*>(pooled_acc), W, bias, out, (bf16*)z_pre_bf16,
-                       (bf16*)pooled_bf16, D, N, act, thresh, drop_p > 0.f ? 1.f / (1.f - drop_p) : 1.f, seed, seed_epoch);
+    hipLaunchKernelGGL(pooled_head_fwd_kernel, dim3(B), dim3(256), 0, st,
+                       pooled_head_fwd_args(pooled, pooled_acc, W, bias, out, z_pre_bf16, pooled_bf16, D, N, act, drop_p, seed, seed_epoch));
     return mm_check_launch("pooled_head_fwd");
 }
 
diff --git a/multimodal_eeg_fmri_amd/ops.py b/multimodal_eeg_fmri_amd/ops.py
--- a/multimodal_eeg_fmri_amd/ops.py
+++ b/multimodal_eeg_fmri_amd/ops.py
@@ -299,13 +299,29 @@
     return clip_loss_ws_floats(B, Bg, grouped=True)
 
 
-def clip_loss_own_rows(z_all, gid_all, logit_scale1, scal, dz, B: int, row0: int):
+def heads_fused_level() -> int:
+    v = os.environ.get("MM_HEADS_FUSED", "1")
+    if v not in ("0", "1", "2"):
+        raise ValueError(f"MM_HEADS_FUSED must be 0, 1 or 2, got {v!r}")
+    return int(v)
+
+
+def clip_heads_bwd_fused_ok(B: int, N: int) -> bool:
+    return bool(_hip.host_int("mm_clip_heads_bwd_fused_ok", B, N))
+
+
+def clip_loss_own_rows(z_all, gid_all, logit_scale1, scal, dz, B: int, row0: int, heads=None):
     Bg, N2 = z_all.shape
+    if (heads is not None and dz is not None and Bg == B and row0 == 0 and heads["z"] is z_all and heads_fused_level() >= 2
+            and clip_heads_bwd_fused_ok(B, N2 // 2)):
+        heads["loss"] = (gid_all, logit_scale1, scal)
+        return True
     ws = _empty((clip_loss_ws_floats(B, Bg, gid_all is not None),), _F32, z_all)
     if gid_all is None:
         _hip.call("mm_clip_loss_own_rows", z_all, logit_scale1, scal, dz, ws, B, Bg, N2 // 2, row0)
     else:
         _hip.call("mm_clip_loss_own_rows_grouped", z_all, gid_all, logit_scale1, scal, dz, ws, B, Bg, N2 // 2, row0)
+    return False
 
 
 def group_ids(groups, n: int, device=None, who: str = "groups") -> Optional[torch.Tensor]:
@@ -578,7 +594,7 @@
 
 
 def pooled_head_fwd(x: torch.Tensor, lin, *, act="gelu", training=False, drop_p=0.0,
-                    need_dgrad=False, save=None, pooled_f32=None):
+                    need_dgrad=False, save=None, pooled_f32=None, defer=False):
     B, L, D = x.shape
     pooled_acc = pooled_f32 is not None
     save = training if save is None else save
@@ -592,9 +608,12 @@
         out = _empty((B, N), _F32, x)
         z = _empty((B, N), _BF, x) if save else None
         pooled = _empty((B, D), _BF, x) if save else None
-        _hip.call("mm_pooled_head_fwd", None if pooled_acc else pooled_f32, pooled_f32 if pooled_acc else None,
-                  lin.weight, lin.bias, out, z, pooled, B, D, N, ACT[act], float(p), int(seed), EP())
+        args = (None if pooled_acc else pooled_f32, pooled_f32 if pooled_acc else None, lin.weight, lin.bias, out, z, pooled)
         saved = dict(pooled=pooled, z=z, seed=seed, drop_p=p, B=B, L=L, D=D, lin=lin, act=act, fused=True) if save else None
+        if defer and save:
+            saved["pending"] = args
+        else:
+            _hip.call("mm_pooled_head_fwd", *args, B, D, N, ACT[act], float(p), int(seed), EP())
         return out, saved
     pooled = _empty((B, D), _BF, x)
     _hip.call("mm_meanpool_fwd", x, None, pooled, B, L, D)
@@ -612,7 +631,7 @@
     return pe[:L, 0, :].contiguous()
 
 
-def _encoder_tail_impl(m, h, training: bool, need_dgrad: bool, save: bool, prenorm=None, stages=None):
+def _encoder_tail_impl(m, h, training: bool, need_dgrad: bool, save: bool, prenorm=None, stages=None, defer_head=False):
     blocks = []
     B, L, D = h.shape
     nblk = len(m.transformer_layers)
@@ -628,11 +647,12 @@
         if stages is not None:
             stages[f"block{i}"] = h.clone()
     out, s = pooled_head_fwd(h, m.output_proj[2], training=training, drop_p=m.drop_p, need_dgrad=need_dgrad,
-                             save=save, pooled_f32=pooled)
+                             save=save, pooled_f32=pooled, defer=defer_head)
     return out, blocks, s, h
 
 
-def _erp_forward_impl(m, x: torch.Tensor, training: bool, need_dgrad: bool, save=None, xb=None, stages=None):
+def _erp_forward_impl(m, x: torch.Tensor, training: bool, need_dgrad: bool, save=None, xb=None, stages=None,
+                      defer_head=False):
     cl = m.conv_layers
     save = training if save is None else save
     p = m.drop_p if training else 0.0
@@ -661,7 +681,8 @@
             o4 = bn_fold_eval(cl[10], cl[9].bias)
             stages["conv3"] = igemm(saved_in[1], wf3, cl[9].kernel_size[0], cl[9].padding[0], cl[9].out_channels,
                                     scale=o4[0], shift=o4[1], act="gelu", out_f32=True, out_bf16=False)["f32"]
-    out, blocks, s, h = _encoder_tail_impl(m, r["f32"], training, need_dgrad, save, prenorm=r.get("prenorm"), stages=stages)
+    out, blocks, s, h = _encoder_tail_impl(m, r["f32"], training, need_dgrad, save, prenorm=r.get("prenorm"), stages=stages,
+                                           defer_head=defer_head)
     return out, dict(convs=saved, blocks=blocks, head=s, x_shape=tuple(x.shape), tokens=h)
 
 
@@ -891,7 +912,7 @@
     return a, dict(x=x, z1=z1, hn=hn, stat=stat, p=p, seed=seed, seq=seq)
 
 
-def contrastive_embed_impl(bridge, eeg: torch.Tensor, fmri: torch.Tensor, training: bool):
+def contrastive_embed_impl(bridge, eeg: torch.Tensor, fmri: torch.Tensor, training: bool, eeg_head=None):
     B = eeg.shape[0]
     N = bridge.bridge_dim
     xe, xf = eeg.float().contiguous(), fmri.float().contiguous()
@@ -904,9 +925,18 @@
     z1 = _empty((2, B, N), _F32, eeg)
     hn = _empty((2, B, N), _F32, eeg)
     stat = _empty((2, B, 2), _F32, eeg)
-    _hip.call("mm_proj_heads_fwd", xe, le.weight, le.bias, lne.weight, lne.bias, xe.shape[1],
-              xf, lf.weight, lf.bias, lnf.weight, lnf.bias, xf.shape[1],
-              z1, hn, stat, z, nrm, B, N, float(lne.eps), p, se, sf, EP())
+    pending = eeg_head.pop("pending", None) if eeg_head is not None else None
+    if pending is not None:
+        if pending[4] is not xe:
+            raise ValueError("contrastive_embed_impl: eeg_head does not belong to these EEG features")
+        _hip.call("mm_heads_fwd_fused", *pending, eeg_head["D"], ACT[eeg_head["act"]], float(eeg_head["drop_p"]),
+                  int(eeg_head["seed"]), le.weight, le.bias, lne.weight, lne.bias, xe.shape[1],
+                  xf, lf.weight, lf.bias, lnf.weight, lnf.bias, xf.shape[1],
+                  z1, hn, stat, z, nrm, B, N, float(lne.eps), p, se, sf, EP())
+    else:
+        _hip.call("mm_proj_heads_fwd", xe, le.weight, le.bias, lne.weight, lne.bias, xe.shape[1],
+                  xf, lf.weight, lf.bias, lnf.weight, lnf.bias, xf.shape[1],
+                  z1, hn, stat, z, nrm, B, N, float(lne.eps), p, se, sf, EP())
     return z, dict(xe=xe, xf=xf, z1=z1, hn=hn, stat=stat, z=z, nrm=nrm, B=B, N=N, p=p, seeds=(se, sf), bridge=bridge)
 
 
@@ -1599,7 +1629,7 @@
     return conv, bn, seqs
 
 
-def _power_forward_impl(m, xb: torch.Tensor, training: bool, need_dgrad: bool, save=None):
+def _power_forward_impl(m, xb: torch.Tensor, training: bool, need_dgrad: bool, save=None, defer_head=False):
     save = training if save is None else save
     conv, bn, seqs = _power_merged_train(m, need_dgrad)
     r, s0 = conv_bn_act(xb, conv, bn, training=training, need_dgrad=need_dgrad, save=save)
@@ -1614,7 +1644,7 @@
     r, s1 = conv_bn_act(r["bf16"], m.fusion[0], m.fusion[1], training=training, drop_p=p,
                         pe=pe_table(m.pos_encoder, T), pe_drop_p=(m.pos_encoder.dropout.p if training else 0.0),
                         want_f32=True, want_bf16=False, need_dgrad=True, save=save)
-    out, blocks, sh, h = _encoder_tail_impl(m, r["f32"], training, True, save)
+    out, blocks, sh, h = _encoder_tail_impl(m, r["f32"], training, True, save, defer_head=defer_head)
     return out, dict(convs=[s0, s1], blocks=blocks, head=sh, merged=(conv, bn, seqs), tokens=h)
 
 
```

After: 41400. 1.4% lower.
